# Skaipi/HNSWIndex.Net

Hardware: AMD Instinct MI355X
Metric: knn_queries_per_sec (higher is better)
Workload: dtype f32

## Files before the change

hnswindex.net_amd/bindings.py:

```python
import ctypes as ct
import os
from pathlib import Path
from typing import List, Optional, Tuple

import numpy as np
import numpy.typing as npt

_PKG = Path(__file__).resolve().parent
LIB_PATH = _PKG / "artifacts" / "native" / "linux-x64" / "HNSWIndex.Native.so"


def _load_lib():
    if os.environ.get("HNSW_MI355X_NO_TORCH", "0") != "1":
        try:
            import torch
        except Exception:
            pass
    override = os.environ.get("HNSW_MI355X_LIB")
    if override:
        return ct.CDLL(override)
    if not LIB_PATH.exists():
        raise FileNotFoundError(
            f"Native library missing {LIB_PATH}: run `python -c 'import __graft_entry__ as g; g.build()'` "
            "(hipcc --offload-arch=gfx950); there is no pure-Python or CPU fallback")
# ... 139 lines not shown


class LayerReach(ct.Structure):
    _fields_ = [(n, ct.c_int32) for n in ("layer_id", "nodes_count", "seeds", "reached", "max_hops")]

    def as_dict(self) -> dict:
        return {n: getattr(self, n) for n, _ in self._fields_}


_GRAPH_REACH_SUMMARY = ("nodes_count", "seeds", "reached", "max_hops")
lib.hnsw_mi355x_reachability.restype = ct.c_int
lib.hnsw_mi355x_reachability.argtypes = [ct.c_void_p, ct.POINTER(LayerReach), ct.c_int]
lib.hnsw_mi355x_unreachable_ids.restype = ct.c_int
lib.hnsw_mi355x_unreachable_ids.argtypes = [ct.c_void_p, ct.c_int, _I, ct.c_int]
lib.hnsw_mi355x_hop_counts.restype = ct.c_int
lib.hnsw_mi355x_hop_counts.argtypes = [ct.c_void_p, ct.c_int, _I, ct.c_int]
lib.hnswdev_graph_reach_layer.restype = ct.c_int
lib.hnswdev_graph_reach_layer.argtypes = [ct.c_void_p, ct.c_int, _U32, ct.c_longlong, _U32, ct.c_longlong, _U32, _I, ct.POINTER(ct.c_uint64)]
lib.hnswdev_graph_reach.restype = ct.c_int
lib.hnswdev_graph_reach.argtypes = [ct.c_void_p, ct.c_int, _U32, ct.c_longlong, ct.c_int, ct.POINTER(LayerReach), ct.c_int, _U32, _I]


class LayerRepair(ct.Structure):
    _fields_ = [(n, ct.c_int32) for n in ("layer_id", "unreachable_before", "linked", "evicted", "rounds", "unreachable_after")]

    def as_dict(self) -> dict:
        return {n: getattr(self, n) for n, _ in self._fields_}


lib.hnsw_mi355x_repair_reachability.restype = ct.c_int
lib.hnsw_mi355x_repair_reachability.argtypes = [ct.c_void_p, ct.c_int, ct.c_int, ct.POINTER(LayerRepair), ct.c_int]
lib.hnswdev_graph_repair_propose.restype = ct.c_int
lib.hnswdev_graph_repair_propose.argtypes = [ct.c_void_p, ct.c_int, _U32, ct.c_longlong, _U32, ct.c_longlong, ct.c_int, ct.c_int, _I, _I, _I, _I, ct.c_int]
lib.hnsw_mi355x_range_query_filtered.restype = ct.c_int
lib.hnsw_mi355x_range_query_filtered.argtypes = [ct.c_void_p, _F, ct.c_int, ct.c_int, ct.c_float, _U32, ct.c_longlong, ct.POINTER(ct.c_void_p),
                                                 ct.POINTER(ct.c_void_p), ct.POINTER(ct.c_int)]
lib.hnsw_mi355x_active_ids.restype = ct.c_int
lib.hnsw_mi355x_knn_query_at_layer.restype = ct.c_int
lib.hnsw_mi355x_knn_query_at_layer.argtypes = [ct.c_void_p, _F, ct.c_int, ct.c_int, ct.c_int, ct.c_int, _U32, ct.c_longlong, _I, _F]
lib.hnsw_mi355x_range_query_at_layer.restype = ct.c_int
lib.hnsw_mi355x_range_query_at_layer.argtypes = [ct.c_void_p, _F, ct.c_int, ct.c_int, ct.c_float, ct.c_int, _U32, ct.c_longlong, ct.POINTER(ct.c_void_p),
                                                 ct.POINTER(ct.c_void_p), ct.POINTER(ct.c_int)]
lib.hnsw_mi355x_multilayer_knn_query.restype = ct.c_int
lib.hnsw_mi355x_multilayer_knn_query.argtypes = [ct.c_void_p, _F, ct.c_int, ct.c_int, ct.c_int, ct.c_int, ct.c_int, ct.c_int, _I, _F]
lib.hnsw_mi355x_active_ids.argtypes = [ct.c_void_p, _I, ct.c_int]
lib.hnsw_mi355x_node_max_layer.restype = ct.c_int
lib.hnsw_mi355x_node_max_layer.argtypes = [ct.c_void_p, ct.c_int]
lib.hnsw_mi355x_get_out_edges.restype = ct.c_int
lib.hnsw_mi355x_get_out_edges.argtypes = [ct.c_void_p, ct.c_int, ct.c_int, _I, ct.c_int]
lib.hnsw_mi355x_export_levels.restype = ct.c_int
lib.hnsw_mi355x_export_levels.argtypes = [ct.c_void_p, _I, ct.c_int]
lib.hnsw_mi355x_export_edges.restype = ct.c_int
lib.hnsw_mi355x_export_edges.argtypes = [ct.c_void_p, ct.c_int, _I, _I, ct.c_int, ct.c_int]
lib.hnsw_mi355x_dim.restype = ct.c_int
lib.hnsw_mi355x_dim.argtypes = [ct.c_void_p]
lib.hnsw_mi355x_serialize.restype = ct.c_int
lib.hnsw_mi355x_serialize.argtypes = [ct.c_void_p, ct.c_char_p]
lib.hnsw_mi355x_deserialize.restype = ct.c_void_p
lib.hnsw_mi355x_deserialize.argtypes = [ct.c_char_p, ct.c_char_p]
lib.hnsw_mi355x_graph_hash.restype = ct.c_uint64
lib.hnsw_mi355x_graph_hash.argtypes = [ct.c_void_p]
lib.hnsw_mi355x_get_stats.restype = ct.c_int
lib.hnsw_mi355x_get_stats.argtypes = [ct.c_void_p, ct.POINTER(DeviceStats)]
lib.hnsw_mi355x_set_profiling.restype = ct.c_int
lib.hnsw_mi355x_set_profiling.argtypes = [ct.c_void_p, ct.c_int]
lib.hnsw_mi355x_index_set_insert_batch.restype = ct.c_int
lib.hnsw_mi355x_index_set_insert_batch.argtypes = [ct.c_void_p, ct.c_int]
lib.hnsw_mi355x_index_insert_batch.restype = ct.c_int
lib.hnsw_mi355x_index_insert_batch.argtypes = [ct.c_void_p]
lib.hnsw_mi355x_host_parallelism.restype = ct.c_int
lib.hnsw_mi355x_host_parallelism.argtypes = []
lib.hnsw_mi355x_device_count.restype = ct.c_int
lib.hnsw_mi355x_device_count.argtypes = [ct.c_void_p]
lib.hnsw_mi355x_get_stats_at.restype = ct.c_int
lib.hnsw_mi355x_get_stats_at.argtypes = [ct.c_void_p, ct.c_int, ct.POINTER(DeviceStats)]
lib.hnsw_mi355x_build_id.restype = ct.c_char_p
lib.hnsw_mi355x_build_id.argtypes = []
lib.hnsw_mi355x_exact_window_stats.restype = ct.c_int
lib.hnsw_mi355x_exact_window_stats.argtypes = [ct.c_void_p, ct.POINTER(ct.c_uint64)]
lib.hnsw_mi355x_row_prefilter_stats.restype = ct.c_int
lib.hnsw_mi355x_row_prefilter_stats.argtypes = [ct.c_void_p, ct.POINTER(ct.c_uint64)]
lib.hnsw_mi355x_row_prefilter_form_stats.restype = ct.c_int
lib.hnsw_mi355x_row_prefilter_form_stats.argtypes = [ct.c_void_p, ct.POINTER(ct.c_uint64)]
lib.hnsw_mi355x_row_prefilter_peek.restype = ct.c_int
lib.hnsw_mi355x_row_prefilter_peek.argtypes = [ct.c_void_p, ct.c_int, ct.c_int, ct.POINTER(ct.c_uint64), ct.POINTER(ct.c_float)]

lib.hnsw_mi355x_import_nodes.argtypes = [ct.c_void_p, _F, ct.c_int, ct.c_int, _I, ct.c_int]
lib.hnsw_mi355x_import_edges.argtypes = [ct.c_void_p, ct.c_int, _I, _I, ct.c_int]
lib.hnswdev_device_count.restype = ct.c_int
lib.hnswdev_create.restype = ct.c_int
lib.hnswdev_create.argtypes = [ct.c_int, ct.c_int, ct.c_int, ct.c_longlong, ct.POINTER(ct.c_void_p)]
lib.hnswdev_destroy.argtypes = [ct.c_void_p]
lib.hnswdev_reserve.argtypes = [ct.c_void_p, ct.c_longlong]
lib.hnswdev_upload_rows.argtypes = [ct.c_void_p, ct.c_int, ct.c_int, _F]
lib.hnswdev_download_rows.argtypes = [ct.c_void_p, ct.c_int, ct.c_int, _F]
lib.hnswdev_dist_query_batch.argtypes = [ct.c_void_p, _F, ct.c_int, _I, _I, _F]
lib.hnswdev_dist_pair_batch.argtypes = [ct.c_void_p, _I, _I, ct.c_int, _F]
lib.hnswdev_graph_begin.argtypes = [ct.c_void_p, ct.c_int, ct.c_int, _I]
lib.hnswdev_graph_set_layer.argtypes = [ct.c_void_p, ct.c_int, _I, _I, ct.c_int]
lib.hnswdev_graph_commit.argtypes = [ct.c_void_p]
lib.hnswdev_knn_search.argtypes = [ct.c_void_p, _F, ct.c_int, ct.c_int, ct.c_int, ct.c_int, _I, _F, _I]
lib.hnswdev_knn_search_filtered.restype = ct.c_int
lib.hnswdev_knn_search_filtered.argtypes = [ct.c_void_p, _F, ct.c_int, ct.c_int, ct.c_int, ct.c_int, _U32, ct.c_longlong, _I, _F, _I]
lib.hnswdev_range_search.restype = ct.c_int
lib.hnswdev_range_search.argtypes = [ct.c_void_p, _F, ct.c_int, ct.c_int, ct.c_float, _I, _I]
lib.hnswdev_exact_knn.restype = ct.c_int
lib.hnswdev_exact_knn.argtypes = [ct.c_void_p, _F, ct.c_int, ct.c_longlong, ct.c_int, _U32, ct.c_longlong, _I, _F]
lib.hnswdev_range_search_filtered.restype = ct.c_int
lib.hnswdev_range_search_filtered.argtypes = [ct.c_void_p, _F, ct.c_int, ct.c_int, ct.c_float, _U32, ct.c_longlong, _I, _I]
lib.hnswdev_exact_range.restype = ct.c_int
lib.hnswdev_exact_range.argtypes = [ct.c_void_p, _F, ct.c_int, ct.c_longlong, ct.c_float, _U32, ct.c_longlong, _I]
lib.hnswdev_exact_range_results.restype = ct.c_int
lib.hnswdev_exact_range_results.argtypes = [ct.c_void_p, _I, _F]
lib.hnswdev_exact_range_grouped.restype = ct.c_int
lib.hnswdev_exact_range_grouped.argtypes = [ct.c_void_p, _F, ct.c_int, ct.c_longlong, ct.c_float, _I, ct.c_longlong, _I, ct.c_int, _I]
lib.hnswdev_exact_knn_grouped.restype = ct.c_int
lib.hnswdev_exact_knn_grouped.argtypes = [ct.c_void_p, _F, ct.c_int, ct.c_longlong, ct.c_int, _I, ct.c_longlong, _I, ct.c_int, _I, _F]
lib.hnswdev_exact_knn_collapsed.restype = ct.c_int
lib.hnswdev_exact_knn_collapsed.argtypes = [ct.c_void_p, _F, ct.c_int, ct.c_longlong, ct.c_int, _I, ct.c_longlong, ct.c_int, _U32, ct.c_longlong, _I, _F]
lib.hnswdev_exact_grouped_list_ms.restype = ct.c_int
lib.hnswdev_exact_grouped_list_ms.argtypes = [ct.c_void_p, ct.POINTER(ct.c_double)]
lib.hnswdev_knn_search_tagged.restype = ct.c_int
lib.hnswdev_knn_search_tagged.argtypes = [ct.c_void_p, _F, ct.c_int, ct.c_int, ct.c_int, ct.c_int, ct.c_int, _U32, ct.c_longlong, _U32, ct.c_int, _I, _F, _I]
lib.hnswdev_exact_knn_tagged.restype = ct.c_int
lib.hnswdev_exact_knn_tagged.argtypes = [ct.c_void_p, _F, ct.c_int, ct.c_longlong, ct.c_int, _U32, ct.c_longlong, _U32, ct.c_int, _I, _F]
lib.hnswdev_gather_rows.restype = ct.c_int
lib.hnswdev_gather_rows.argtypes = [ct.c_void_p, _I, ct.c_int, _F]
lib.hnswdev_knn_search_by_id.restype = ct.c_int
lib.hnswdev_knn_search_by_id.argtypes = [ct.c_void_p, _I, ct.c_int, ct.c_int, ct.c_int, ct.c_int, ct.c_int, _I, _F, _I]
lib.hnswdev_exact_knn_by_id.restype = ct.c_int
lib.hnswdev_exact_knn_by_id.argtypes = [ct.c_void_p, _I, ct.c_int, ct.c_longlong, ct.c_int, _U32, ct.c_longlong, _I, _F]
lib.hnswdev_exact_range_by_id.restype = ct.c_int
lib.hnswdev_exact_range_by_id.argtypes = [ct.c_void_p, _I, ct.c_int, ct.c_longlong, ct.c_float, _U32, ct.c_longlong, _I]
lib.hnswdev_exact_range_groups.restype = ct.c_int
lib.hnswdev_exact_range_groups.argtypes = [ct.c_void_p, ct.c_longlong, ct.c_float, _U32, ct.c_longlong, _I, ct.POINTER(ct.c_uint64)]
lib.hnswdev_tag_list_ms.restype = ct.c_int
lib.hnswdev_tag_list_ms.argtypes = [ct.c_void_p, ct.POINTER(ct.c_double)]
lib.hnswdev_knn_search_grouped.restype = ct.c_int
lib.hnswdev_knn_search_grouped.argtypes = [ct.c_void_p, _F, ct.c_int, ct.c_int, ct.c_int, ct.c_int, ct.c_int, _I, ct.c_longlong, _I, ct.c_int, _I, _F, _I]
lib.hnswdev_range_search_grouped.restype = ct.c_int
lib.hnswdev_range_search_grouped.argtypes = [ct.c_void_p, _F, ct.c_int, ct.c_int, ct.c_float, ct.c_int, _I, ct.c_longlong, _I, ct.c_int, _I, _I]
lib.hnswdev_range_search_tagged.restype = ct.c_int
lib.hnswdev_range_search_tagged.argtypes = [ct.c_void_p, _F, ct.c_int, ct.c_int, ct.c_float, ct.c_int, _U32, ct.c_longlong, _U32, ct.c_int, _I, _I]
lib.hnswdev_exact_range_tagged.restype = ct.c_int
lib.hnswdev_exact_range_tagged.argtypes = [ct.c_void_p, _F, ct.c_int, ct.c_longlong, ct.c_float, _U32, ct.c_longlong, _U32, ct.c_int, _I]
lib.hnswdev_range_results.restype = ct.c_int
lib.hnswdev_range_results.argtypes = [ct.c_void_p, _I, _F]
lib.hnswdev_knn_search_at_layer.restype = ct.c_int
lib.hnswdev_knn_search_at_layer.argtypes = [ct.c_void_p, _F, ct.c_int, ct.c_int, ct.c_int, ct.c_int, ct.c_int, _U32, ct.c_longlong, _I, _F, _I]
lib.hnswdev_range_search_at_layer.restype = ct.c_int
lib.hnswdev_range_search_at_layer.argtypes = [ct.c_void_p, _F, ct.c_int, ct.c_int, ct.c_float, ct.c_int, _U32, ct.c_longlong, _I, _I]
lib.hnswdev_multilayer_search.restype = ct.c_int
lib.hnswdev_multilayer_search.argtypes = [ct.c_void_p, _F, ct.c_int, ct.c_int, ct.c_int, ct.c_int, ct.c_int, ct.c_int, _I, _F, _I]
lib.hnswdev_sync.argtypes = [ct.c_void_p]
lib.hnswdev_set_profiling.argtypes = [ct.c_void_p, ct.c_int]
lib.hnswdev_get_stats.argtypes = [ct.c_void_p, ct.POINTER(DeviceStats)]
lib.hnswdev_reset_stats.argtypes = [ct.c_void_p]
lib.hnswdev_last_error.argtypes = [ct.c_char_p, ct.c_int]
lib.hnswdev_ctx_last_error.argtypes = [ct.c_void_p, ct.c_char_p, ct.c_int]
lib.hnswdev_set_queries.argtypes = [ct.c_void_p, _F, ct.c_int]
lib.hnswdev_step_buffers.argtypes = [ct.c_void_p, ct.c_int, ct.c_int, ct.c_int, ct.POINTER(_I), ct.POINTER(_F)]
lib.hnswdev_step_submit.argtypes = [ct.c_void_p, ct.c_int, ct.c_int]
lib.hnswdev_step_wait.argtypes = [ct.c_void_p, ct.c_int]
lib.hnswdev_test_sqrt_rn.argtypes = [ct.c_int, ct.POINTER(ct.c_double), ct.POINTER(ct.c_double), ct.c_int]

COUNTER_BLOCKS = {
# ... 218 lines not shown

    @staticmethod
    def _check(status):
        if status < 0:
            raise RuntimeError(last_error())

    def set_collection_size(self, init_size: int):
        self._check(lib.hnsw_set_collection_size(init_size))

    def set_max_edges(self, max_conn: int):
        self._check(lib.hnsw_set_max_edges(max_conn))

    def set_max_candidates(self, max_candidates: int):
        self._check(lib.hnsw_set_max_candidates(max_candidates))

    def set_remove_max_candidates(self, rem_max_candidates: int):
        self._check(lib.hnsw_set_remove_max_candidates(rem_max_candidates))

    def set_distribution_rate(self, dist_rate: float):
        self._check(lib.hnsw_set_distribution_rate(dist_rate))

    def set_random_seed(self, random_seed: int):
        self._check(lib.hnsw_set_random_seed(random_seed))

    def set_min_nn(self, min_nn: int):
        self._check(lib.hnsw_set_min_nn(min_nn))

    def set_allow_removals(self, allow_removals: bool):
        self._check(lib.hnsw_set_allow_removals(allow_removals))

    def set_device(self, device: int):
        self._check(lib.hnsw_mi355x_set_device(device))

    def set_devices(self, n: int):
        self._check(lib.hnsw_mi355x_set_devices(n))

    def stats_at(self, context: int):
        st = DeviceStats()
        if not self._h or lib.hnsw_mi355x_get_stats_at(self._h, context, ct.byref(st)) != 0:
            raise RuntimeError(last_error() or "no such device context")
        return st.as_dict()

    def set_insert_batch(self, max_batch: int):
        self._check(lib.hnsw_mi355x_set_insert_batch(max_batch))

    def set_insert_batch_live(self, max_batch: int):
        if not self._h:
            return self.set_insert_batch(max_batch)
        self._check(lib.hnsw_mi355x_index_set_insert_batch(self._h, max_batch))

    @property
    def insert_batch_cap(self) -> int:
        return int(lib.hnsw_mi355x_index_insert_batch(self._h)) if self._h else host_parallelism()

    def exact_window_stats(self):
        out = (ct.c_uint64 * 4)()
        if not self._h or lib.hnsw_mi355x_exact_window_stats(self._h, out) != 0:
            return {"rounds": 0, "searches": 0, "alone": 0, "linked": 0}
        return {"rounds": int(out[0]), "searches": int(out[1]), "alone": int(out[2]), "linked": int(out[3])}

    def row_prefilter_stats(self):
        out = (ct.c_uint64 * 4)()
        if not self._h or lib.hnsw_mi355x_row_prefilter_stats(self._h, out) != 0:
            return {"launches": 0, "rows_on_shadow": 0, "rows_reread": 0, "rows_packed": 0}
        return {"launches": int(out[0]), "rows_on_shadow": int(out[1]), "rows_reread": int(out[2]), "rows_packed": int(out[3])}

    def row_prefilter_form_stats(self):
        out = (ct.c_uint64 * 2)()
        if not self._h or lib.hnsw_mi355x_row_prefilter_form_stats(self._h, out) != 0:
            return {"runtime_dim": 0, "fixed_dim": 0}
        return {"runtime_dim": int(out[0]), "fixed_dim": int(out[1])}

    def row_prefilter_peek(self, first_id: int = 0, count: int = 0):
        out = (ct.c_uint64 * 2)()
        rows = np.zeros((max(int(count), 0), self.dim), dtype=np.float32)
        if not self._h:
            if count > 0:
                raise RuntimeError("row_prefilter_peek: the index has no shadow rows")
            return {"packed": 0, "e_bits": 0, "e": np.float32(0), "rows": rows}
        self._check(lib.hnsw_mi355x_row_prefilter_peek(self._h, int(first_id), int(count), out, rows.ctypes.data_as(ct.POINTER(ct.c_float))))
        bits = int(out[1]) & 0xffffffff
        return {"packed": int(out[0]), "e_bits": bits, "e": np.array([bits], dtype=np.uint32).view(np.float32)[0], "rows": rows}

    def set_remove_batch(self, max_batch: int):
        self._check(lib.hnsw_mi355x_set_remove_batch(max_batch))

    def set_search_slots(self, slots: int):
        self._check(lib.hnsw_mi355x_set_search_slots(slots))

    def set_host_threads(self, threads: int):
        self._check(lib.hnsw_mi355x_set_host_threads(threads))

    def set_device_traversal(self, enabled: bool):
        self._check(lib.hnsw_mi355x_set_device_traversal(int(enabled)))

    def add(self, vecs: npt.ArrayLike) -> npt.NDArray[np.int32]:
        if not self._initialized:
            self._initialize()
        a = _as_2d_f32(vecs, self.dim)
        n, d = a.shape
        out_ids = np.empty(n, dtype=np.int32)
        rc = lib.hnsw_add(self._h, a.ctypes.data_as(_F), int(n), int(d), out_ids.ctypes.data_as(_I))
        if rc < 0:
            raise RuntimeError(last_error())
        return out_ids[:rc].copy()

    def remove(self, ids: npt.ArrayLike) -> None:
        arr = np.asarray(ids, dtype=np.int32).ravel()
        if arr.size == 0:
            return
        result = lib.hnsw_remove(self._h, arr.ctypes.data_as(_I), int(arr.size))
        if result < 0:
            raise RuntimeError(last_error())

    def knn_query(self, queries: npt.ArrayLike, k: int, allowed=None, layer: int = 0) -> Tuple[npt.NDArray[np.int32], npt.NDArray[np.float32]]:
        q = _as_2d_f32(queries, self.dim)
        n = int(q.shape[0])
        ids = np.empty((n, k), dtype=np.int32)
        dists = np.empty((n, k), dtype=np.float32)
        if layer != 0:
            ids.fill(-1)
            dists.fill(np.nan)
            words, nbits = allow_bits(allowed) if allowed is not None else (None, 0)
            words, wp = _words_arg(words) if allowed is not None else (None, None)
            status = lib.hnsw_mi355x_knn_query_at_layer(self._h, q.ctypes.data_as(_F), n, self.dim, k, int(layer), wp, nbits, ids.ctypes.data_as(_I),
                                                        dists.ctypes.data_as(_F))
            if status < 0:
                raise RuntimeError(last_error())
            return ids, dists
        if allowed is not None:
            words, nbits = allow_bits(allowed)
            words, wp = _words_arg(words)
            status = lib.hnsw_mi355x_knn_query_filtered(self._h, q.ctypes.data_as(_F), n, self.dim, k, wp, nbits, ids.ctypes.data_as(_I),
                                                        dists.ctypes.data_as(_F))
            if status < 0:
                raise RuntimeError(last_error())
            return ids, dists
        status = lib.hnsw_knn_query(self._h, q.ctypes.data_as(_F), n, self.dim, k, ids.ctypes.data_as(_I),
                                    dists.ctypes.data_as(_F))
        if status < 0:
            raise RuntimeError(last_error())
        return ids, dists

    def exact_knn_query(self, queries: npt.ArrayLike, k: int, allowed=None) -> Tuple[npt.NDArray[np.int32], npt.NDArray[np.float32]]:
        q = _as_2d_f32(queries, self.dim)
        n = int(q.shape[0])
        ids = np.full((n, max(k, 0)), -1, dtype=np.int32)
        dists = np.full((n, max(k, 0)), np.nan, dtype=np.float32)
        words, nbits = allow_bits(allowed) if allowed is not None else (None, 0)
        words, wp = _words_arg(words) if allowed is not None else (None, None)
        status = lib.hnsw_mi355x_exact_knn_query(self._h, q.ctypes.data_as(_F), n, self.dim, k, wp, nbits, ids.ctypes.data_as(_I),
                                                 dists.ctypes.data_as(_F))
        if status < 0:
            raise RuntimeError(last_error())
        return ids, dists

    def exact_knn_query_grouped(self, queries: npt.ArrayLike, k: int, row_group, query_group,
                                n_groups=None) -> Tuple[npt.NDArray[np.int32], npt.NDArray[np.float32]]:
        q = _as_2d_f32(queries, self.dim)
        n = int(q.shape[0])
        rg, qg, ng = _group_args(row_group, query_group, n_groups, n)
        ids = np.full((n, max(k, 0)), -1, dtype=np.int32)
        dists = np.full((n, max(k, 0)), np.nan, dtype=np.float32)
        status = lib.hnsw_mi355x_exact_knn_query_grouped(self._h, q.ctypes.data_as(_F), n, self.dim, k, rg.ctypes.data_as(_I), rg.shape[0],
                                                         qg.ctypes.data_as(_I), ng, ids.ctypes.data_as(_I), dists.ctypes.data_as(_F))
        if status < 0:
# ... 949 lines not shown
```

hnswindex.net_amd/csrc/device_backend.h:

```cpp
#pragma once
#include <cstddef>
#include <algorithm>
#include <atomic>
#include <cstdint>
#include <functional>
#include <memory>
#include <mutex>
#include <string>
#include <unordered_map>
#include <vector>
#include <thread>

#include "../../include/hnsw_mi355x.h"
#include "counter_blocks.h"
#include "dev_buf.h"

namespace hnsw {

#define HNSW_FOR_EACH_METRIC(X)      \
    X(M_SQ, sq, "sq_euclid")         \
    X(M_COS, cos, "cosine")          \
    X(M_UCOS, ucos, "ucosine")       \
    X(M_I8, i8, "sq_euclid_i8")      \
    X(M_SQH, sqh, "sq_euclid_f16")   \
// ... 210 lines not shown
    long long resident_queries() const { return n_queries_; }
    bool dist_query_batch(const float *queries, int nq, const int *offsets, const int *ids, float *out);
    bool dist_pair_batch(const int *a, const int *b, int n, float *out);

    bool graph_begin(int n, int max_edges, const int *levels);
    bool graph_set_layer(int layer, const int *counts, const int *edges, int stride);
    bool graph_commit();
    bool knn_search(const float *queries, int nq, int entry_point, int k_beam, int k_out, int *out_ids, float *out_d, int *out_flag, int layer = 0);
    bool knn_search_filtered(const float *queries, int nq, int entry_point, int k_beam, int k_out, const uint32_t *allow_bits, long long nbits,
                             int *out_ids, float *out_d, int *out_flag, int layer = 0);
    bool knn_search_grouped(const float *queries, int nq, int entry_point, int k_beam, int k_out, const int *row_group, long long n_row_group,
                            const int *query_group, int n_groups, int *out_ids, float *out_d, int *out_flag, int layer = 0);
    bool knn_search_tagged(const float *queries, int nq, int entry_point, int k_beam, int k_out, const uint32_t *row_tags, long long n_row_tags,
                           const uint32_t *query_tags, int match, int *out_ids, float *out_d, int *out_flag, int layer = 0);
    int multilayer_search_abi(const float *queries, int nq, int entry_point, int k, int max_layer, int min_layer, int layers_cap, int *out_ids,
                              float *out_d, int *out_flag);
    struct RangeResults {
        std::vector<unsigned long long> off;
        std::vector<int> cnt, flag, entry;
        std::vector<int> state;
        SearchHit *found = nullptr;
        size_t found_n = 0;
    };
    bool range_batch(const SearchJob *jobs, int njobs, float range, RangeResults *res, const RangeFilter &f);
    bool tag_candidates(const uint32_t *row_tags, long long n, const std::vector<uint32_t> &masks, int match, std::vector<int> &cnt);
    bool range_search(const float *queries, int nq, int entry_point, float range, int *out_counts, int *out_flags);
    bool range_search_filtered(const float *queries, int nq, int entry_point, float range, const uint32_t *allow_bits, long long nbits,
                               int *out_counts, int *out_flags, int layer = 0);
    bool range_search_grouped(const float *queries, int nq, int entry_point, float range, const int *row_group, long long n_row_group,
                              const int *query_group, int n_groups, int *out_counts, int *out_flags, int layer = 0);
    bool range_search_tagged(const float *queries, int nq, int entry_point, float range, const uint32_t *row_tags, long long n_row_tags,
                             const uint32_t *query_tags, int match, int *out_counts, int *out_flags, int layer = 0);
    bool range_results(int *out_ids, float *out_d);
    bool exact_knn(const float *queries, int nq, long long n_rows, int k, const uint32_t *allow_bits, long long nbits, int *out_ids, float *out_d);
    bool exact_knn_collapsed(const float *queries, int nq, long long n_rows, int k, const int *row_group, long long n_row_group, int per_group,
                             const uint32_t *allow_bits, long long nbits, int *out_ids, float *out_d);
    bool search_collapsed(int nq, int entry, int entry_layer, int ef, int beam, int k, const int *row_group, long long n_row_group, int per_group,
                          const uint32_t *allow_bits, long long nbits, int *out_ids, float *out_d, int *out_flag, int search_layer = 0);
    bool gather_rows(const int *ids, int n, float *out);
    bool set_queries_by_id(const int *ids, int nq);
    bool search_self(int nq, int entry, int entry_layer, int k, int k_out, int *out_ids, float *out_d, int *out_flag, int search_layer = 0);
    bool knn_search_by_id(const int *ids, int nq, int entry_point, int k_beam, int k_out, int *out_ids, float *out_d, int *out_flag, int layer = 0);
    bool exact_knn_by_id(const int *ids, int nq, long long n_rows, int k, const uint32_t *allow_bits, long long nbits, int *out_ids, float *out_d);
    bool exact_range(const float *queries, int nq, long long n_rows, float range, const uint32_t *allow_bits, long long nbits, int *out_counts);
    bool exact_range_results(int *out_ids, float *out_d);
    size_t exact_range_total() const { return xr_ids_.size(); }
    bool exact_range_by_id(const int *ids, int nq, long long n_rows, float range, const uint32_t *allow_bits, long long nbits, int *out_counts);
    bool exact_range_groups(long long n_rows, float range, const uint32_t *allow_bits, long long nbits, int *out_labels, uint64_t *out_info);
    bool exact_knn_grouped(const float *queries, int nq, long long n_rows, int k, const int *row_group, long long n_row_group, const int *query_group,
                           int n_groups, int *out_ids, float *out_d);
    bool exact_knn_tagged(const float *queries, int nq, long long n_rows, int k, const uint32_t *row_tags, long long n_row_tags, const uint32_t *query_tags,
                          int match, int *out_ids, float *out_d);
    double tag_list_ms() const { return xt_list_ms_; }
    bool exact_range_grouped(const float *queries, int nq, long long n_rows, float range, const int *row_group, long long n_row_group,
                             const int *query_group, int n_groups, int *out_counts);
    bool exact_range_tagged(const float *queries, int nq, long long n_rows, float range, const uint32_t *row_tags, long long n_row_tags,
                            const uint32_t *query_tags, int match, int *out_counts);
    double exact_grouped_list_ms() const { return xg_list_ms_; }
    bool graph_info(int layer, const uint32_t *live_bits, long long nbits, bool with_in_edges, hnsw_mi355x_layer_info *out);
    bool graph_components(int layer, const uint32_t *live_bits, long long nbits, int *out_count);
    bool graph_info_layer(const char *who, int layer);
    bool graph_reach_layer(int layer, const uint32_t *live_bits, long long nbits, const uint32_t *seed_bits, long long seed_nbits,
                           uint32_t *out_reached_bits, int *out_hops, uint64_t out_summary[4]);
    int graph_reach(int entry_point, int top, const uint32_t *live_bits, long long nbits, int min_layer, hnsw_mi355x_layer_reach *out_layers, int cap,
                    uint32_t *out_reached_bits, int *out_hops);
    bool graph_reach_top(const char *who, int entry_point, int *top);

    bool graph_repair_round(int layer, const uint32_t *live_bits, long long nbits, int seed_mode, int entry_point, const uint32_t *seed_bits, long long seed_nbits,
                            int which, int cands, int max_edges, bool propose, GraphRepairRound *out);
    bool graph_repair_patch(const int *recs, int nrows, int row_stride);
    int graph_repair_propose(int layer, const uint32_t *live_bits, long long nbits, const uint32_t *seed_bits, long long seed_nbits, int cands, int max_edges,
                             int *out_n, int *out_ids, int *out_cands, int *out_codes, int cap);

    void set_profiling(bool on) { profiling_ = on; }


    void set_shadows_allowed(bool on) { shadows_allowed_ = on; }
    void get_stats(hnswdev_stats *out);
    void reset_stats();
    void counters(CounterBlock b, uint64_t *out) const { std::copy_n(counters_[(int)b], kCounterSlots[(int)b], out); }
    void row_prefilter_stats(uint64_t out[4]);
    void row_prefilter_form_stats(uint64_t out[2]);
    bool row_prefilter_peek(long long first_id, int count, uint64_t out[2], float *rows);

    std::mutex &mutex() { return mu_; }
    void set_error(const std::string &msg) { std::lock_guard<std::mutex> lk(err_mu_); err_ = msg; }
    std::string error() { std::lock_guard<std::mutex> lk(err_mu_); return err_; }

private:
    Device() = default;
    std::mutex mu_, err_mu_;
    std::string err_;
    bool bind();
    bool abi_entry(const char *who, int entry_point, int *top, bool args_ok = true);
    bool abi_begin(const char *who, const float *queries, int nq, int entry_point, int layer, int *top, bool args_ok = true);
    int device_ = 0, dim_ = 0, metric_ = 0;
    int pitch_ = 0;
    int row_pitch_ = 0;
    DevBuf<float> q_stage_;
    long long capacity_ = 0;
    long long n_rows_hw_ = 0;
    DevBuf<float> d_rows_;
    DevBuf<double> d_row_sn_;
    struct RowPrefilter {
        std::mutex mu;
        DevBuf<float> rows;
        DevBuf<unsigned long long> words;
        long long row_cap = 0, packed = 0;
        bool lost = false;
        bool no_memory = false;
        uint64_t launches = 0, on_shadow = 0, reread = 0, rows_packed = 0;
        uint64_t form_launches[2] = {0, 0};
    };
    std::shared_ptr<RowPrefilter> pf_;
    void rows_written(long long first_id);
    bool row_prefilter_ready();
    DevBuf<float> d_queries_;
    DevBuf<double> d_q_sn_;
    long long q_capacity() const { return (long long)(d_queries_.cap() / (size_t)pitch_); }
    long long n_queries_ = 0;
    DevBuf<int> g_adj0_, g_level_, g_pool_;
    DevBuf<int64_t> g_upper_;
    long long g_n_ = 0;
    long long g_cap_n() const { return (long long)g_tested0_.cap(); }
    long long g_pool_cap() const { return (long long)g_testedU_.cap(); }
    bool graph_room(long long n, long long node_cap, int stride0, long long pool_len);
    DevBuf<int> g_tested0_, g_testedU_;
    int g_stride0_ = 0, g_strideU_ = 0;
    DevBuf<unsigned> s_visited_;
    DevBuf<int> s_jobctr_;
    DevBuf<int> lp_slot_[3];
    DevBuf<int> lp_grp_[6];
    DevBuf<int> lp_counters_;
    int last_insert_jobs_ = 0, last_insert_upper_ = 0, last_insert_stride_ = 0;
    int fetch_njobs_ = 0, fetch_nupper_ = 0;
    DevBuf<int> s_vistab_;
    int s_vistab_each_ = 0;
    DevBuf<int> s_fvistab_;
    int s_fvistab_each_ = 0;
    bool visited_scratch(int k, int min_cap, bool allow_hash, VisitedScratch *out, bool filtered = false);
    bool plan_traversal(bool insert, int k, bool two_heap, size_t lds, TraversalLaunch *out, bool filtered = false);
    template <class Upload, class Launch>
    bool run_resident(size_t row, long long chunk, size_t extra, bool hashed, int nq, int *out_ids, float *out_d, int *out_flag, Upload &&upload,
                      Launch &&launch);
    template <class OwnRules> bool predicate_call_ok(const PredicateCall &c, OwnRules &&own_rules);
    template <class Of> auto plan_predicate_search(const PredicateCall &c, Of of);
    template <class K, class Upload, class JobsOf, class Predicate>
    bool run_predicate_search(const PredicateCall &c, const PredicatePlan<K> &p, size_t extra, Upload &&upload, JobsOf &&jobs_of, Predicate &&predicate);
    uint64_t count_search_overflows(const PredicateCall &c);
    bool count_launch(const LaunchFamily *family, unsigned long long evals, bool hashed, bool timed, void *t0, void *t1);
    int num_cu_ = 256;
    int max_slots() const { return num_cu_ * max_waves_per_cu(); }
    static int max_waves_per_cu();
    DevBuf<SearchJob> s_jobs_;
    DevBuf<SearchHit> s_hits_;
    DevBuf<int> s_cnt_, s_flag_;
    DevBuf<unsigned long long> s_evals_;
    DevBuf<int> s_sel_, s_lcnt_, s_selU_, s_cntU_, s_iflag_;
    PinBuf<char> h_res_;
    DevBuf<int> s_rl_;
    DevBuf<int> s_order_;
    DevBuf<int> s_rlog_;
    struct QueryTail { const float *src = nullptr; long long first = 0, n = 0; } tail_;
    PinBuf<int> h_ready_;
    int *d_ready_ = nullptr;
    DevStream copy_stream_;
    bool upload_tail();
    DevBuf<int> s_dry_;
    DevBuf<int> s_wdry_;
    DevBuf<int> s_win_;
    DevBuf<SearchHit> s_spill_;
    DevBuf<SearchHit> s_fspill_;
    DevBuf<unsigned> s_allow_;
    DevBuf<int> s_glabel_;
    DevBuf<int> s_gquery_;
    DevBuf<unsigned> s_ttags_;
    DevBuf<unsigned> s_tmask_;
    DevBuf<int> s_tcnt_;
    DevBuf<int> s_tquery_;
    double xt_list_ms_ = 0.0;
    bool tag_counts(const unsigned *row_tags, long long n, const std::vector<uint32_t> &masks, int match, std::vector<int> &cnt);
    DevBuf<int> s_self_;
    DevBuf<int> x_self_;
    bool q_by_id_ = false;
    bool query_room(int nq);
    bool upload_ids(const int *ids, int n, DevBuf<int> &d_ids);
    bool gather_launch(const int *d_ids, long long n, float *out);
    bool gather_queries(const int *ids, int n, DevBuf<int> &d_ids, float *d_q, double *d_qsn);
    DevBuf<int> x_ids_;
    DevBuf<long long> x_boff_;
    DevBuf<unsigned long long> x_lists_;
    DevBuf<int> x_out_;
    DevBuf<unsigned long long> x_evals_;
    DevBuf<float> x_queries_;
    DevBuf<double> x_q_sn_;
    bool exact_queries(const char *who, const float *queries, int nq, const float **d_q, const double **d_qsn);
    bool exact_id_list(const uint32_t *allow_bits, long long n_allow, long long *m);
    bool exact_knn_rounds(const float *d_q, const double *d_qsn, int nq, const int *d_idlist, long long m, int k, int *out_ids, float *out_d, int *d_keep_ids,
                          const int *d_self = nullptr, const ExactCollapseArgs *collapse = nullptr);
// ... 119 lines not shown
```

hnswindex.net_amd/csrc/device_backend.hip:

```cpp

#include <hip/hip_runtime.h>

#include <algorithm>
#include <cmath>
#include <cstdio>
#include <cstdlib>
#include <cstring>
#include <limits>
#include <map>
#include <mutex>
#include <type_traits>
#include <vector>

#include "device_backend.h"
#include "diag.h"
#define HNSW_HOST_TU
#include "device_kernels.h"
#include "dk_exact.h"
#include "dk_graph_info.h"
#include "dk_graph_reach.h"
#include "dk_graph_repair.h"
#include "dk_tag_lists.h"
#include "range_replay.h"

// ... 322 lines not shown
    const int pitch = f16_row_words(dim);
    for (size_t r = 0; r < n; ++r) {
        const float *x = src + r * (size_t)dim;
        unsigned *rec = dst + r * (size_t)pitch;
        for (int w = 0; w < pitch; ++w) {
            const int i0 = ((w >> 3) << 4) | (w & 7), i1 = i0 + 8;
            unsigned b0 = 0u, b1 = 0u;
            if (i0 < dim) { memcpy(&b0, x + i0, 4); b0 = f32_to_f16_bits(b0); }
            if (i1 < dim) { memcpy(&b1, x + i1, 4); b1 = f32_to_f16_bits(b1); }
            rec[w] = b0 | (b1 << 16);
        }
    }
}

bool Device::upload_rows_begin(int first_id, int n, const float *rows)
{
    if (n <= 0) return true;
    if (metric_ == M_I8 || bg_.active.load()) { set_dev_error("upload_rows_begin: not available (int8 rows, or an upload already in flight)"); return false; }
    if (first_id < 0 || (long long)first_id + n > capacity_ || !rows) { set_dev_error("upload_rows: range outside capacity"); return false; }
    if (!bind()) return false;
    rows_written(first_id);
    const size_t row_bytes = (size_t)dim_ * sizeof(float);
    const size_t chunk_rows = std::max<size_t>(1, (8u << 20) / row_bytes);
    if (!bg_.stream.create(false) || !bg_.ev[0].create(false) || !bg_.ev[1].create(false)) return false;
    const size_t pin_need = chunk_rows * std::max(row_bytes, (size_t)row_pitch_ * sizeof(float));
    if (!bg_.pin[0].grow(pin_need) || !bg_.pin[1].grow(pin_need)) return false;
    bg_.resident.store(first_id);
    bg_.failed.store(false);
    bg_.active.store(true);
    n_rows_hw_ = std::max(n_rows_hw_, (long long)first_id + n);
    const bool f16 = metric_f16(metric_);
    bg_.th = std::thread([this, first_id, n, rows, row_bytes, chunk_rows, f16] {
        auto fail = [&](const char *what, hipError_t e) { bg_.err = std::string(what) + ": " + hipGetErrorString(e); bg_.failed.store(true); };
        hipError_t e = hipSetDevice(device_);
        if (e != hipSuccess) { fail("hipSetDevice", e); return; }
        hipStream_t st = S(bg_.stream);
        size_t pending_rows[2] = {0, 0};
        bool in_flight[2] = {false, false};
        int b = 0;
        long long landed = first_id;
        for (size_t r0 = 0; r0 < (size_t)n; r0 += chunk_rows, b ^= 1) {
            const size_t nr = std::min(chunk_rows, (size_t)n - r0);
            if (in_flight[b]) {
                if ((e = hipEventSynchronize(E(bg_.ev[b]))) != hipSuccess) { fail("hipEventSynchronize", e); return; }
                landed += (long long)pending_rows[b];
                bg_.resident.store(landed, std::memory_order_release);
                in_flight[b] = false;
            }
            if (f16) pack_f16_rows_host(reinterpret_cast<unsigned *>(bg_.pin[b].get()), rows + r0 * dim_, nr, dim_);
            else memcpy(bg_.pin[b], rows + r0 * dim_, nr * row_bytes);
            if ((e = hipMemcpyAsync(d_rows_ + ((size_t)first_id + r0) * row_pitch_, bg_.pin[b], f16 ? nr * (size_t)row_pitch_ * sizeof(float) : nr * row_bytes, hipMemcpyHostToDevice, st)) != hipSuccess) { fail("hipMemcpyAsync", e); return; }
            if (metric_ == M_COS) {
                const int blocks = (int)(((long long)nr * 8 + 255) / 256);
                hipLaunchKernelGGL(row_sqrtnorm_kernel, dim3(blocks), dim3(256), 0, st, d_rows_, pitch_, (long long)first_id + (long long)r0, (int)nr, d_row_sn_);
            }
            if ((e = hipEventRecord(E(bg_.ev[b]), st)) != hipSuccess) { fail("hipEventRecord", e); return; }
            pending_rows[b] = nr;
            in_flight[b] = true;
        }
        for (int k = 0; k < 2; ++k, b ^= 1)
            if (in_flight[b]) {
                if ((e = hipEventSynchronize(E(bg_.ev[b]))) != hipSuccess) { fail("hipEventSynchronize", e); return; }
                landed += (long long)pending_rows[b];
                bg_.resident.store(landed, std::memory_order_release);
            }
    });
    return true;
}

bool Device::upload_rows_wait(long long upto)
{
    if (!bg_.active.load()) return true;
    if (upto >= 0) {
        while (bg_.resident.load(std::memory_order_acquire) < upto && !bg_.failed.load()) std::this_thread::yield();
        if (!bg_.failed.load()) return true;
    }
    if (bg_.th.joinable()) bg_.th.join();
    bg_.active.store(false);
    if (bg_.failed.load()) { set_dev_error("background row upload failed: " + bg_.err); return false; }
    return true;
}

static int row_prefilter_mode() { return diag("row_prefilter", 1); }

void Device::rows_written(long long first_id)
{
    if (!pf_) return;
    std::lock_guard<std::mutex> lk(pf_->mu);
    pf_->packed = std::min(pf_->packed, std::max(0ll, first_id));
    pf_->lost = false;
}

bool Device::row_prefilter_ready()
{
    const int mode = row_prefilter_mode();
    if (!pf_ || metric_ != M_SQ || mode == 0 || bg_.active.load() || n_rows_hw_ <= 0) return false;
    RowPrefilter &P = *pf_;
    std::lock_guard<std::mutex> lk(P.mu);
    if (P.no_memory || (P.lost && mode != 2)) return false;
    hipStream_t st = S(stream_);
    const size_t words = (size_t)f16_row_words(dim_);
    if (P.row_cap < capacity_ || !P.rows) {
        const std::string before = get_dev_error();
        const bool first = !P.words;
        if (!P.rows.grow((size_t)capacity_ * words) || !P.words.grow(4)) {
            (void)P.rows.reset();
            P.row_cap = P.packed = 0;
            P.no_memory = true;
            (void)hipGetLastError();
            set_dev_error(before);
            return false;
        }
        P.row_cap = capacity_;
        P.packed = 0;
        if (first) HIP_OK(hipMemsetAsync(P.words, 0, 4 * sizeof(unsigned long long), st));
    }
    const long long n = n_rows_hw_;
    if (P.packed < n) {
        if (P.packed == 0) HIP_OK(hipMemsetAsync(P.words, 0, sizeof(unsigned long long), st));
        const long long more = n - P.packed;
        hipLaunchKernelGGL(pack_shadow_rows_kernel, dim3((unsigned)((more + 3) / 4)), dim3(256), 0, st, d_rows_.get(), dim_, P.packed, more, P.rows.get(),
                           reinterpret_cast<unsigned *>(P.words.get()));
        HIP_OK(hipGetLastError());
        HIP_OK(hipStreamSynchronize(st));
        P.rows_packed += (uint64_t)more;
        P.packed = n;
    }
    return true;
}

void Device::row_prefilter_stats(uint64_t out[4])
{
    out[0] = out[1] = out[2] = out[3] = 0;
    if (!pf_) return;
    std::lock_guard<std::mutex> lk(pf_->mu);
    out[0] = pf_->launches; out[1] = pf_->on_shadow; out[2] = pf_->reread; out[3] = pf_->rows_packed;
}

void Device::row_prefilter_form_stats(uint64_t out[2])
{
    out[0] = out[1] = 0;
    if (!pf_) return;
    std::lock_guard<std::mutex> lk(pf_->mu);
    out[0] = pf_->form_launches[0]; out[1] = pf_->form_launches[1];
}

bool Device::row_prefilter_peek(long long first_id, int count, uint64_t out[2], float *rows)
{
    out[0] = out[1] = 0;
    if (!pf_ || !pf_->rows || !pf_->words) {
        if (count > 0) set_dev_error("row_prefilter_peek: the index has no shadow rows");
        return count <= 0;
    }
    if (!bind()) return false;
    RowPrefilter &P = *pf_;
    std::lock_guard<std::mutex> lk(P.mu);
    unsigned long long e_word = 0;
    HIP_OK(hipMemcpy(&e_word, P.words.get(), sizeof(e_word), hipMemcpyDeviceToHost));
    out[0] = (uint64_t)P.packed;
    out[1] = (uint64_t)(e_word & 0xffffffffull);
    if (count <= 0) return true;
    if (first_id < 0 || first_id + count > P.packed || !rows) {
        set_dev_error("row_prefilter_peek: range outside the packed shadow rows");
        return false;
    }
    const size_t words = (size_t)f16_row_words(dim_), total = (size_t)count * words;
    const unsigned *src = reinterpret_cast<const unsigned *>(P.rows.get()) + (size_t)first_id * words;
    unsigned buf[2048];
    for (size_t w0 = 0; w0 < total; w0 += 2048) {
        const size_t nw = std::min<size_t>(2048, total - w0);
        HIP_OK(hipMemcpy(buf, src + w0, nw * sizeof(unsigned), hipMemcpyDeviceToHost));
        for (size_t j = 0; j < nw; ++j) {
            const size_t r = (w0 + j) / words;
            const int w = (int)((w0 + j) % words), i0 = ((w >> 3) << 4) | (w & 7), i1 = i0 + 8;
            if (i0 < dim_) rows[r * (size_t)dim_ + i0] = half_lo(buf[j]);
            if (i1 < dim_) rows[r * (size_t)dim_ + i1] = half_hi(buf[j]);
        }
    }
    return true;
}

bool Device::download_rows(int first_id, int n, float *rows)
{
    if (n <= 0) return true;
    if (first_id < 0 || (long long)first_id + n > capacity_ || !rows) {
        set_dev_error("download_rows: range outside capacity");
        return false;
    }
    if (!bind()) return false;
    if (metric_ == M_I8) {
        if (!q_stage_.grow((size_t)n * (size_t)dim_)) return false;
        hipLaunchKernelGGL(dequantize_rows_kernel, dim3((unsigned)(((long long)n * dim_ + 255) / 256)), dim3(256), 0, S(stream_), d_rows_, pitch_,
                           (long long)first_id, n, dim_, q_stage_);
        HIP_OK(hipGetLastError());
        HIP_OK(hipMemcpyAsync(rows, q_stage_, (size_t)n * dim_ * sizeof(float), hipMemcpyDeviceToHost, S(stream_)));
    } else if (metric_f16(metric_)) {
        const size_t chunk_rows = std::max<size_t>(1, (64u << 20) / ((size_t)dim_ * sizeof(float)));
        if (!q_stage_.grow(std::min<size_t>((size_t)n, chunk_rows) * (size_t)dim_)) return false;
        for (size_t r0 = 0; r0 < (size_t)n; r0 += chunk_rows) {
            const size_t nr = std::min(chunk_rows, (size_t)n - r0);
            hipLaunchKernelGGL(unpack_f16_rows_kernel, dim3((unsigned)((nr * (size_t)dim_ + 255) / 256)), dim3(256), 0, S(stream_), d_rows_,
                               (long long)first_id + (long long)r0, (int)nr, dim_, q_stage_);
            HIP_OK(hipGetLastError());
            HIP_OK(hipMemcpyAsync(rows + r0 * (size_t)dim_, q_stage_, nr * (size_t)dim_ * sizeof(float), hipMemcpyDeviceToHost, S(stream_)));
            HIP_OK(hipStreamSynchronize(S(stream_)));
        }
    } else {
        HIP_OK(hipMemcpyAsync(rows, d_rows_ + (size_t)first_id * pitch_, (size_t)n * dim_ * sizeof(float), hipMemcpyDeviceToHost, S(stream_)));
    }
    HIP_OK(hipStreamSynchronize(S(stream_)));
    return true;
}

bool Device::staged_upload(float *dst, const float *src, size_t bytes)
{
    constexpr int T = 4;
    constexpr size_t kChunk = 2u << 20;
    for (int i = 0; i < 2 * T; ++i) {
        if (!up_pin_[i].grow(kChunk) || !up_ev_[i].create(false)) return false;
// ... 462 lines not shown
    const int c = diag("spill_cap", -1);
    return c < 0 ? kSpillCap : std::min(kSpillCap, c);
}
constexpr int kFilterSpillCap = 32768;
static int filter_spill_cap()
{
    const int c = diag("spill_cap", -1);
    return c < 0 ? kFilterSpillCap : std::min(kFilterSpillCap, c);
}
constexpr int kFilterVisCap = 1 << 17;


static bool shadow_mode()
{
    return diag("shadow", 1) != 0;
}
static int overlap_mode()
{
    return diag("overlap", 1);
}
static bool lean_mode() { return diag("lean", 1) != 0; }
static int novis_mode()
{
    return diag("novis", 2);
}
static constexpr size_t kTeamLds = ((sizeof(TeamMail) + 15) & ~(size_t)15) + 16;
static int lat_mode()
{
    return diag("lat", 1);
}

static bool mfma_heuristic()
{
    return diag("mfma", 1) != 0;
}

struct VisitedScratch {
    long long words = 0;
    size_t bytes_per_job = 0;
    int *tab = nullptr;
    int tab_cap = 0;
};

bool Device::visited_scratch(int k, int min_cap, bool allow_hash, VisitedScratch *v, bool filtered)
{
    *v = VisitedScratch{};
    v->words = ((g_n_ + 31) / 32 + 3) & ~3LL;
    v->bytes_per_job = sizeof(unsigned) * (size_t)v->words;
    if (!allow_hash) return true;
    const int e = diag("vis_hash", -1);
    const bool want = e >= 0 ? e != 0 : v->bytes_per_job > (512u << 10);
    if (!want) return true;
    int cap = 16384;
    while (cap < 64 * k && cap < (1 << 22)) cap <<= 1;
    if (const int c = diag("vis_hash_cap", 0)) { cap = 64; while (cap < c && cap < (1 << 22)) cap <<= 1; }
    while (cap < min_cap) cap <<= 1;
    const size_t need = (size_t)max_slots() * (size_t)cap;
    DevBuf<int> &tab = filtered ? s_fvistab_ : s_vistab_;
    int &tab_each = filtered ? s_fvistab_each_ : s_vistab_each_;
    if (need > tab.cap() || cap != tab_each) {
        HIP_OK(hipStreamSynchronize(S(stream_)));
        if (!tab.reset() || !tab.grow(need)) return false;
        HIP_OK(hipMemsetAsync(tab, 0xff, sizeof(int) * need, S(stream_)));
        tab_each = cap;
    }
    v->tab = tab;
    v->tab_cap = cap;
    v->words = 0;
    v->bytes_per_job = 16;
    return true;
}

struct TraversalLaunch {
    int metric, max_slots, num_cu;
    size_t lds;
    int ns;
    bool exact_only;
    VisitedScratch vis;
    bool novis;
    bool lat_ok;
    bool filtered;
    bool prefilter;
    bool pf_fixed;
    int form;
    int slots, grid;
    unsigned block;
    size_t lds_total;
    int flags;
};

bool Device::plan_traversal(bool insert, int k, bool two_heap, size_t lds, TraversalLaunch *t, bool filtered)
{
    const int ns = g_n_ < kSortedTopMaxNodes && !two_heap && !filtered ? sorted_top_sets(k) : 0;
    t->metric = metric_;
    t->max_slots = max_slots();
    t->num_cu = num_cu_;
    t->lds = lds;
    t->filtered = filtered;
    t->prefilter = false;
    t->pf_fixed = pitch_ == kPfFixedDim && diag("pf_fixed_dim", 1) != 0;
    t->exact_only = ns == 0;
    t->ns = t->exact_only ? 2 : ns;
    if (!visited_scratch(k, filtered ? kFilterVisCap : 512, t->ns != 8, &t->vis, filtered)) return false;
    if (filtered) {
        t->novis = false;
        t->lat_ok = false;
        return true;
    }
    const int novis = novis_mode();
    t->novis = (!insert || diag("novis_insert", 1) != 0) && g_stride0_ - 2 <= 64 && overlap_mode() != 0 && (size_t)pitch_ * sizeof(float) <= 1024 &&
               (novis == 2 || (novis == 1 && t->vis.tab != nullptr));
    t->lat_ok = !t->exact_only && g_stride0_ - 2 <= 64 && lds + kTeamLds <= 64 * 1024;
    return true;
}

template <bool Insert, int M, int NS, bool H>
static auto traversal_form(int form)
{
    if constexpr (Insert)
        return form == kFormLat ? &graph_insert_search_kernel<M, NS, H, kFormLat> : &graph_insert_search_kernel<M, NS, H, kFormPlain>;
    else if constexpr (NS <= 4)
        return form == kFormLat ? &graph_search_kernel<M, NS, H, kFormLat>
               : form == kFormLean ? &graph_search_kernel<M, NS, H, kFormLean>
               : form == kFormLeanPF ? &graph_search_kernel<M, NS, H, kFormLeanPF>
               : form == kFormLeanPFFixed ? &graph_search_kernel<M, NS, H, kFormLeanPFFixed> : &graph_search_kernel<M, NS, H, kFormPlain>;
    else
        return form == kFormLat ? &graph_search_kernel<M, NS, H, kFormLat> : &graph_search_kernel<M, NS, H, kFormPlain>;
}
template <bool Insert>
static auto traversal_kernel(const TraversalLaunch &t, int form)
{
    const bool hashed = t.vis.tab != nullptr;
    decltype(traversal_form<Insert, M_SQ, 2, false>(0)) kernel = nullptr;
    with_metric(t.metric, [&](auto m) {
        if (t.ns == 2) kernel = hashed ? traversal_form<Insert, m, 2, true>(form) : traversal_form<Insert, m, 2, false>(form);
        else if (t.ns == 4) kernel = hashed ? traversal_form<Insert, m, 4, true>(form) : traversal_form<Insert, m, 4, false>(form);
        else kernel = traversal_form<Insert, m, 8, false>(form);
    });
    return kernel;
}

template <class Of>
static auto persistent_kernel(int metric, bool hashed, Of of)
{
    decltype(of(std::integral_constant<int, M_SQ>{}, std::false_type{})) kernel = nullptr;
    with_metric(metric, [&](auto m) { kernel = hashed ? of(m, std::true_type{}) : of(m, std::false_type{}); });
    return kernel;
}
template <class K>
static void place_persistent(K kernel, TraversalLaunch &t, int nj)
{
    t.form = kFormPlain;
    t.slots = std::min(t.max_slots, resident_blocks(kernel, t.lds, t.num_cu));
    t.grid = std::min(nj, t.slots);
    t.block = 64;
    t.lds_total = t.lds;
    t.flags = 0;
}

template <bool Insert>
static auto place_traversal(TraversalLaunch &t, int nj)
{
    const bool hashed = t.vis.tab != nullptr;
    const int lat = lat_mode();
    t.form = kFormPlain;
    if (t.lat_ok && lat != 0) {
        const int slots = std::min(t.max_slots, resident_blocks(traversal_kernel<Insert>(t, kFormLat), t.lds + kTeamLds, t.num_cu, 128));
        if (slots > 0 && (lat == 2 || nj <= slots)) { t.form = kFormLat; t.slots = slots; }
    }
    if (!Insert && t.form == kFormPlain && t.novis && !t.exact_only && lean_mode() && t.ns <= 4) t.form = !t.prefilter ? kFormLean : t.pf_fixed ? kFormLeanPFFixed : kFormLeanPF;
    const auto kernel = traversal_kernel<Insert>(t, t.form);
    if (t.form != kFormLat) t.slots = std::min(t.max_slots, resident_blocks(kernel, t.lds, t.num_cu));
    t.grid = std::min(nj, t.slots);
    t.block = t.form == kFormLat ? 128 : 64;
    t.lds_total = t.lds + (t.form == kFormLat ? kTeamLds : 0);
    const int overlap = overlap_mode();
    t.flags = (t.exact_only ? 0x200 : 0) | (t.novis ? 9 : overlap == 2 || (overlap == 1 && (nj <= t.slots || hashed)) ? 1 : 0);
    return kernel;
}

bool Device::ensure_search_scratch(long long chunk, long long slots, int k, size_t vis_bytes_per_job)
{
    const size_t vis_words = vis_bytes_per_job * (size_t)slots / sizeof(unsigned);
    if (vis_words > s_visited_.cap()) {
        if (!s_visited_.grow(vis_words)) return false;
        HIP_OK(hipMemsetAsync(s_visited_, 0, sizeof(unsigned) * vis_words, S(stream_)));
    }
    const size_t jobs_cap = s_flag_.cap();
    if (!s_jobctr_.grow(4 + std::max<size_t>((size_t)chunk, jobs_cap))) return false;
    if ((size_t)chunk > jobs_cap) {
        uj_len_ = 0;
        if (!reset_all(s_jobs_, s_cnt_, s_flag_)) return false;
        if (!s_jobs_.grow((size_t)chunk) || !s_cnt_.grow((size_t)chunk) || !s_flag_.grow((size_t)chunk)) return false;
    }
    if (k > 0 && !s_hits_.grow((size_t)chunk * k + ((size_t)chunk + 1) / 2)) return false;
    if (!s_spill_.grow((size_t)slots * kSpillCap + 8)) return false;
    if (!s_evals_.grow(1)) return false;
    return ev0_.create(true) && ev1_.create(true) && ev2_.create(false);
}

static bool jobs_valid(const SearchJob *jobs, int njobs, long long g_n, long long n_queries, long long n_rows)
{
    for (int i = 0; i < njobs; ++i) {
        const SearchJob &j = jobs[i];
        bool ok = j.entry >= 0 && j.entry < g_n && j.search_layer >= 0 && j.entry_layer >= j.search_layer &&
                  (j.qref >= 0 ? j.qref < n_queries : (~j.qref) < n_rows);
        if (!ok) return false;
    }
    return true;
}

bool Device::insert_search_batch(const SearchJob *jobs, int njobs, int k, int max_edges0, int n_upper, InsertResults *res, WindowExtras *win)
{
    if (njobs <= 0) return true;
    const bool windowed = win != nullptr;
    const int read_log_cap = windowed ? win->read_log_cap : 0;
    if (windowed && (read_log_cap < 8 || njobs > (1 << 16) || (n_upper > 0 && !win->upper_owner))) { set_dev_error("insert_search_batch: bad window request"); return false; }
    if (!jobs || !res || k < 1 || n_upper < 0 || max_edges0 < 2) { set_dev_error("insert_search_batch: bad argument"); return false; }
    if (g_n_ <= 0) { set_dev_error("insert_search_batch: no graph uploaded"); return false; }
    for (int i = 0; i < njobs; ++i) {
        const SearchJob &j = jobs[i];
        if (j.qref >= 0) { set_dev_error("insert_search_batch: qref must name a stored row"); return false; }
        if (j.search_layer > 0 && (j.aux < 0 || j.aux + j.search_layer > n_upper)) { set_dev_error("insert_search_batch: upper-layer slot out of range"); return false; }
        if (j.stop_layer < 0 || j.stop_layer > j.search_layer || (!windowed && j.stop_layer != 0)) { set_dev_error("insert_search_batch: bad stop layer"); return false; }
    }
    if (!jobs_valid(jobs, njobs, g_n_, n_queries_, n_rows_hw_)) { set_dev_error("insert_search_batch: job outside the uploaded graph / rows"); return false; }
    const int cand_cap = cand_lds_cap(k, pitch_, true, nbcap());
    const size_t lds = search_lds_bytes(k, cand_cap, pitch_, true, nbcap());
    if (lds > 64 * 1024) { set_dev_error("insert_search_batch: beam width / dimension exceed the LDS budget"); return false; }
    const size_t lds_link = windowed ? link_lds_or_error("insert_search_batch", pitch_, nbcap()) : 0;
    if (windowed && !lds_link) return false;
    if (!bind()) return false;
    hipStream_t st = S(stream_);
    const int sel_stride = max_edges0;
    const long long chunk = std::min<long long>(njobs, 1 << 20);
    TraversalLaunch tl;
    if (!plan_traversal(true, k, false, lds, &tl)) return false;
    if (!ensure_search_scratch(chunk, max_slots(), 0, tl.vis.bytes_per_job)) return false;
    const size_t nU = (size_t)std::max(n_upper, 1);
    if (!s_sel_.grow((size_t)njobs * sel_stride) || !s_lcnt_.grow((size_t)njobs) || !s_selU_.grow(nU * sel_stride) || !s_cntU_.grow(nU) || !s_iflag_.grow((size_t)njobs))
        return false;
    if (windowed && !s_rlog_.grow((size_t)njobs * (size_t)read_log_cap)) return false;
    const size_t b_sel0 = 4u * (size_t)njobs * sel_stride, b_cnt0 = 4u * (size_t)njobs, b_selU = 4u * nU * sel_stride, b_cntU = 4u * nU, b_flag = 4u * (size_t)njobs;
    const size_t b_log = windowed ? 4u * (size_t)njobs * (size_t)read_log_cap : 0;
    const size_t b_dry = windowed ? b_sel0 + b_selU : 0;
    const size_t b_drop = windowed ? 3u * b_sel0 : 0;
    const size_t b_rep = windowed ? b_flag : 0;
    if (windowed && !s_wdry_.grow(nU)) return false;
    const size_t need = b_sel0 + b_cnt0 + b_selU + b_cntU + b_flag + 16 + b_log + b_dry + b_drop + b_rep;
    if (windowed && !s_win_.grow((need - b_rep + 3) / 4u + 64)) return false;
    if (!h_res_.grow(need, need + need / 2)) return false;
    char *hb = h_res_;
    int *h_sel0 = reinterpret_cast<int *>(hb), *h_cnt0 = reinterpret_cast<int *>(hb + b_sel0);
// ... 348 lines not shown
{
    if (set < 0 || set > 1 || !lset_[set].busy) { set_dev_error("link_batch_finish: nothing in flight"); return false; }
    LinkSet &ls = lset_[set];
    if (!bind()) return false;
    HIP_OK(hipEventSynchronize(E(ls.ev_done)));
    ls.busy = false;
    if (out_lists) *out_lists = ls.h_out;
    if (ls.ngroups > 0 && !count_launch(&kLinkFamily, *ls.h_ev, false, ls.timed, ls.ev_start, ls.ev_stop)) return false;
    return true;
}


void *Device::pinned_stage(size_t bytes)
{
    return h_stage_.grow(bytes, std::max<size_t>(bytes, 1u << 20)) ? h_stage_.get() : nullptr;
}

bool Device::search_batch(const SearchJob *jobs, int njobs, int k, int k_out, int *out_ids, float *out_d, int *out_flag, bool keep_repeat_flag,
                          bool two_heap)
{
    if (njobs <= 0) return true;
    if (!jobs) { set_dev_error("search_batch: bad argument"); return false; }
    return search_batch_impl(jobs, njobs, k, k_out, out_ids, out_d, out_flag, keep_repeat_flag, two_heap, -1, -1);
}

bool Device::search_queries(int nq, int entry, int entry_layer, int k, int k_out, int *out_ids, float *out_d, int *out_flag)
{
    if (nq <= 0) return true;
    if (nq > (1 << 20)) {
        std::vector<SearchJob> jobs((size_t)nq);
        for (int i = 0; i < nq; ++i) jobs[(size_t)i] = SearchJob{i, entry, entry_layer, 0, -1, 0};
        return search_batch(jobs.data(), nq, k, k_out, out_ids, out_d, out_flag);
    }
    return search_batch_impl(nullptr, nq, k, k_out, out_ids, out_d, out_flag, false, false, entry, entry_layer);
}

bool Device::search_batch_impl(const SearchJob *jobs, int njobs, int k, int k_out, int *out_ids, float *out_d, int *out_flag, bool keep_repeat_flag,
                               bool two_heap, int u_entry, int u_layer)
{
    if (!out_ids || !out_d || !out_flag || k < 1 || k_out < 1) { set_dev_error("search_batch: bad argument"); return false; }
    if (g_n_ <= 0) { set_dev_error("search_batch: no graph uploaded"); return false; }
    if (jobs ? !jobs_valid(jobs, njobs, g_n_, n_queries_, n_rows_hw_) : !(u_entry >= 0 && u_entry < g_n_ && u_layer >= 0 && njobs <= n_queries_)) {
        set_dev_error("search_batch: job outside the uploaded graph / rows / queries");
        return false;
    }
    const int cand_cap = cand_lds_cap(k, pitch_, false, nbcap());
    const size_t lds = search_lds_bytes(k, cand_cap, pitch_, false, nbcap());
    if (lds > 64 * 1024) { set_dev_error("search_batch: beam width / dimension exceed the LDS budget"); return false; }
    if (!bind()) return false;
    hipStream_t st = S(stream_);
    const long long chunk = std::min<long long>(njobs, 1 << 20);
    TraversalLaunch tl;
    if (!plan_traversal(false, k, two_heap, lds, &tl)) return false;
    if (!ensure_search_scratch(chunk, max_slots(), k_out, tl.vis.bytes_per_job)) return false;
    const size_t b_jobs = sizeof(SearchJob) * (size_t)chunk, b_res = 4u * (size_t)chunk * k_out;
    const size_t off_pf = (16 + b_jobs + 2 * b_res + 4u * (size_t)chunk + 7) & ~(size_t)7;
    char *hs = static_cast<char *>(pinned_stage(off_pf + 16));
    if (!hs) return false;
    unsigned long long *h_ev = reinterpret_cast<unsigned long long *>(hs), *h_pf = reinterpret_cast<unsigned long long *>(hs + off_pf);
    SearchJob *h_jobs = reinterpret_cast<SearchJob *>(hs + 16);
    int *h_ids = reinterpret_cast<int *>(hs + 16 + b_jobs);
    float *h_d = reinterpret_cast<float *>(hs + 16 + b_jobs + b_res);
    int *h_flag = reinterpret_cast<int *>(hs + 16 + b_jobs + 2 * b_res);
    int *d_ids = reinterpret_cast<int *>(s_hits_.get());
    float *d_d = reinterpret_cast<float *>(s_hits_.get()) + (size_t)chunk * k_out;
    const bool compact = !row_collapse_ && njobs == chunk && 2 * b_res + 4u * (size_t)chunk <= (size_t)1 << 20;
    const size_t w_out = row_collapse_ ? (size_t)row_collapse_->k : (size_t)k_out;
    int *d_flag = compact ? reinterpret_cast<int *>(d_d + (size_t)chunk * k_out) : s_flag_;
    unsigned long long *d_ev = compact ? reinterpret_cast<unsigned long long *>(s_jobctr_.get() + 2) : s_evals_;
    const int *gate = tail_.n > 0 ? d_ready_ : nullptr;
    struct TailGuard { Device *d; ~TailGuard() { if (d->tail_.n > 0) d->n_queries_ = 0; d->tail_.n = 0; } } tail_guard{this};
    for (long long off = 0; off < njobs; off += chunk) {
        const int nj = (int)std::min<long long>(chunk, njobs - off);
        if (jobs) {
            memcpy(h_jobs, jobs + off, sizeof(SearchJob) * (size_t)nj);
            HIP_OK(hipMemcpyAsync(s_jobs_, h_jobs, sizeof(SearchJob) * (size_t)nj, hipMemcpyHostToDevice, st));
            uj_len_ = 0;
        } else if (!(uj_len_ >= nj && uj_entry_ == u_entry && uj_layer_ == u_layer)) {
            for (int i = 0; i < nj; ++i) h_jobs[i] = SearchJob{i, u_entry, u_layer, 0, -1, 0};
            HIP_OK(hipMemcpyAsync(s_jobs_, h_jobs, sizeof(SearchJob) * (size_t)nj, hipMemcpyHostToDevice, st));
            uj_len_ = nj; uj_entry_ = u_entry; uj_layer_ = u_layer;
        }
        auto kernel = place_traversal<false>(tl, nj);
        if (tl.form == kFormLean && row_prefilter_ready()) {
            tl.prefilter = true;
            kernel = place_traversal<false>(tl, nj);
        }
        const bool prefiltered = form_is_pf(tl.form);
        HIP_OK(hipMemsetAsync(s_jobctr_, 0, sizeof(int) * (4 + (size_t)nj), st));
        if (!compact) HIP_OK(hipMemsetAsync(s_evals_, 0, sizeof(unsigned long long), st));
        const bool timed = profiling_;
        if (timed) HIP_OK(hipEventRecord(E(ev0_), st));
        hipLaunchKernelGGL(kernel, dim3(tl.grid), dim3(tl.block), tl.lds_total, st, d_rows_, d_row_sn_, d_queries_, d_q_sn_, pitch_, g_adj0_, g_stride0_,
                           g_upper_, g_pool_, g_strideU_, s_jobs_, k, cand_cap, reinterpret_cast<ND *>(s_spill_.get()), spill_cap_for_tests(), s_visited_,
                           tl.vis.words, tl.vis.tab, tl.vis.tab_cap, k_out, d_ids, d_d, s_cnt_, d_flag, d_ev, nbcap(), nj, s_jobctr_,
                           tl.flags | (shadow_mode() && shadows_allowed_ ? 0x100 : 0), gate, prefiltered ? pf_->rows.get() : (const float *)nullptr,
                           prefiltered ? pf_->words.get() : (unsigned long long *)nullptr);
        if (tl.form == kFormLat) stats_.lat_launches++;
        if (form_is_lean(tl.form)) stats_.lean_launches++;
        HIP_OK(hipGetLastError());
        if (timed) HIP_OK(hipEventRecord(E(ev1_), st));
        if (prefiltered) HIP_OK(hipMemcpyAsync(h_pf, pf_->words.get() + 1, 2 * sizeof(unsigned long long), hipMemcpyDeviceToHost, st));
        if (tail_.n > 0 && !upload_tail()) return false;
        if (compact) {
            HIP_OK(hipMemcpyAsync(h_ids, d_ids, 2 * b_res + sizeof(int) * (size_t)nj, hipMemcpyDeviceToHost, st));
            HIP_OK(hipMemcpyAsync(h_ev, d_ev, sizeof(unsigned long long), hipMemcpyDeviceToHost, st));
            HIP_OK(hipStreamSynchronize(st));
            memcpy(out_ids + (size_t)off * k_out, h_ids, 4u * (size_t)nj * k_out);
        } else if (row_collapse_) {
            if (!collapse_and_fetch(d_ids, d_d, nj, (size_t)k_out, h_ids, h_d)) return false;
            HIP_OK(hipMemcpyAsync(h_flag, s_flag_, sizeof(int) * (size_t)nj, hipMemcpyDeviceToHost, st));
            HIP_OK(hipMemcpyAsync(h_ev, s_evals_, sizeof(unsigned long long), hipMemcpyDeviceToHost, st));
            HIP_OK(hipStreamSynchronize(st));
            memcpy(out_ids + (size_t)off * w_out, h_ids, 4u * (size_t)nj * w_out);
        } else {
        HIP_OK(hipMemcpyAsync(h_ids, d_ids, 4u * (size_t)nj * k_out, hipMemcpyDeviceToHost, st));
        HIP_OK(hipEventRecord(E(ev2_), st));
        HIP_OK(hipMemcpyAsync(h_d, d_d, 4u * (size_t)nj * k_out, hipMemcpyDeviceToHost, st));
        HIP_OK(hipMemcpyAsync(h_flag, s_flag_, sizeof(int) * (size_t)nj, hipMemcpyDeviceToHost, st));
        HIP_OK(hipMemcpyAsync(h_ev, s_evals_, sizeof(unsigned long long), hipMemcpyDeviceToHost, st));
        HIP_OK(hipEventSynchronize(E(ev2_)));
        memcpy(out_ids + (size_t)off * k_out, h_ids, 4u * (size_t)nj * k_out);
        HIP_OK(hipStreamSynchronize(st));
        }
        memcpy(out_d + (size_t)off * w_out, h_d, 4u * (size_t)nj * w_out);
        for (int i = 0; i < nj; ++i) {
            if (h_flag[i] == 2) { stats_.search_repeats++; if (!keep_repeat_flag) h_flag[i] = 0; }
            else if (h_flag[i] == 4) { stats_.tie_windows++; h_flag[i] = 0; }
        }
        memcpy(out_flag + off, h_flag, sizeof(int) * (size_t)nj);
        if (prefiltered) {
            std::lock_guard<std::mutex> lk(pf_->mu);
            const uint64_t d_shadow = h_pf[0] > pf_->on_shadow ? h_pf[0] - pf_->on_shadow : 0, d_reread = h_pf[1] > pf_->reread ? h_pf[1] - pf_->reread : 0;
            pf_->launches++;
            pf_->form_launches[tl.form == kFormLeanPFFixed]++;
            pf_->on_shadow += d_shadow;
            pf_->reread += d_reread;
            if (2 * d_reread > d_shadow && row_prefilter_mode() != 2) pf_->lost = true;
        }
        tl.prefilter = false;
        if (!count_launch(nullptr, *h_ev, tl.vis.tab != nullptr, timed, ev0_, ev1_)) return false;
    }
    for (int i = 0; i < njobs; ++i) stats_.search_overflows += (uint64_t)(out_flag[i] == 1);
    return true;
}

bool Device::collapse_and_fetch(int *d_ids, float *d_d, int nj, size_t width, int *h_ids, float *h_d)
{
    hipStream_t st = S(stream_);
    const RowCollapse &rc = *row_collapse_;
    const size_t lds = 12 * width + 4 * (size_t)rc.k, w = (size_t)rc.k;
    if (lds > 64 * 1024) { set_dev_error("search_collapsed: the beam exceeds the LDS budget of the collapse"); return false; }
    hipLaunchKernelGGL(collapse_rows_kernel, dim3((unsigned)nj), dim3(64), lds, st, d_ids, d_d, (int)width, rc.k, rc.d_labels, rc.n_labels, rc.per_group);
    HIP_OK(hipGetLastError());
    HIP_OK(hipMemcpy2DAsync(h_ids, 4 * w, d_ids, 4 * width, 4 * w, (size_t)nj, hipMemcpyDeviceToHost, st));
    HIP_OK(hipMemcpy2DAsync(h_d, 4 * w, d_d, 4 * width, 4 * w, (size_t)nj, hipMemcpyDeviceToHost, st));
    return true;
}

template <class Upload, class Launch>
bool Device::run_resident(size_t row, long long chunk, size_t extra, bool hashed, int nq, int *out_ids, float *out_d, int *out_flag, Upload &&upload,
                          Launch &&launch)
{
    hipStream_t st = S(stream_);
    const size_t b_res = 4u * (size_t)chunk * row;
    char *hs = static_cast<char *>(pinned_stage(16 + 2 * b_res + 4u * (size_t)chunk + extra));
    if (!hs) return false;
    unsigned long long *h_ev = reinterpret_cast<unsigned long long *>(hs);
    int *h_ids = reinterpret_cast<int *>(hs + 16);
    float *h_d = reinterpret_cast<float *>(hs + 16 + b_res);
    int *h_flag = reinterpret_cast<int *>(hs + 16 + 2 * b_res);
    if (!upload(hs + 16 + 2 * b_res + 4u * (size_t)chunk)) return false;
    int *d_ids = reinterpret_cast<int *>(s_hits_.get());
    float *d_d = reinterpret_cast<float *>(s_hits_.get()) + (size_t)chunk * row;
    for (long long off = 0; off < nq; off += chunk) {
        const int nj = (int)std::min<long long>(chunk, nq - off);
        HIP_OK(hipMemsetAsync(s_jobctr_, 0, sizeof(int) * 4, st));
        HIP_OK(hipMemsetAsync(s_evals_, 0, sizeof(unsigned long long), st));
        const bool timed = profiling_;
        if (timed) HIP_OK(hipEventRecord(E(ev0_), st));
        launch(off, nj, d_ids, d_d);
        HIP_OK(hipGetLastError());
        if (timed) HIP_OK(hipEventRecord(E(ev1_), st));
        const size_t w = row_collapse_ ? (size_t)row_collapse_->k : row;
        if (row_collapse_) { if (!collapse_and_fetch(d_ids, d_d, nj, row, h_ids, h_d)) return false; }
        else {
            HIP_OK(hipMemcpyAsync(h_ids, d_ids, 4u * (size_t)nj * row, hipMemcpyDeviceToHost, st));
            HIP_OK(hipMemcpyAsync(h_d, d_d, 4u * (size_t)nj * row, hipMemcpyDeviceToHost, st));
        }
        HIP_OK(hipMemcpyAsync(h_flag, s_flag_, sizeof(int) * (size_t)nj, hipMemcpyDeviceToHost, st));
        HIP_OK(hipMemcpyAsync(h_ev, s_evals_, sizeof(unsigned long long), hipMemcpyDeviceToHost, st));
        HIP_OK(hipStreamSynchronize(st));
        memcpy(out_ids + (size_t)off * w, h_ids, 4u * (size_t)nj * w);
        memcpy(out_d + (size_t)off * w, h_d, 4u * (size_t)nj * w);
        memcpy(out_flag + off, h_flag, sizeof(int) * (size_t)nj);
        if (!count_launch(nullptr, *h_ev, hashed, timed, ev0_, ev1_)) return false;
    }
    return true;
}

struct PredicateCall {
    std::string who;
    int nq, entry, entry_layer, search_layer, k, k_out;
    int *out_ids;
    float *out_d;
    int *out_flag;
};
template <class K>
struct PredicatePlan {
    bool ok;
    K kernel;
    TraversalLaunch tl;
    int cand_cap, fspill;
    long long chunk;
};

template <class OwnRules>
bool Device::predicate_call_ok(const PredicateCall &c, OwnRules &&own_rules)
{
    const std::string &who = c.who;
    if (!c.out_ids || !c.out_d || !c.out_flag || c.k < 1 || c.k_out < 1) { set_dev_error(who + ": bad argument"); return false; }
    if (const std::string why = own_rules(); !why.empty()) { set_dev_error(why); return false; }
    if (g_n_ <= 0) { set_dev_error(who + ": no graph uploaded"); return false; }
// ... 2955 lines not shown
```

hnswindex.net_amd/csrc/device_kernels.h:

```cpp
#pragma once
#include "dk_base.h"
#include "dk_metric.h"
#include "dk_heaps.h"
#include "dk_measure.h"
#include "dk_search_common.h"
#include "dk_sorted_top.h"
#include "dk_team.h"
#include "dk_pool_top.h"
#include "dk_traverse_exact.h"
#include "dk_heuristic.h"
#include "dk_search_kernels.h"
#include "dk_range_finish.h"
#include "dk_insert_kernels.h"
#include "dk_link.h"
#include "dk_misc_kernels.h"

namespace hnsw {

#define HNSW_FOR_EACH_TRAVERSAL(X, M) \
    X(M, 2, false, kFormPlain) X(M, 4, false, kFormPlain) X(M, 8, false, kFormPlain) \
    X(M, 2, true, kFormPlain) X(M, 4, true, kFormPlain)
#define HNSW_FOR_EACH_TRAVERSAL_LAT(X, M) \
    X(M, 2, false, kFormLat) X(M, 4, false, kFormLat) X(M, 8, false, kFormLat) \
    X(M, 2, true, kFormLat) X(M, 4, true, kFormLat)
#define HNSW_FOR_EACH_TRAVERSAL_LEAN(X, M) \
    X(M, 2, false, kFormLean) X(M, 4, false, kFormLean) X(M, 2, true, kFormLean) X(M, 4, true, kFormLean) \
    X(M, 2, false, kFormLeanPF) X(M, 4, false, kFormLeanPF) X(M, 2, true, kFormLeanPF) X(M, 4, true, kFormLeanPF) \
    X(M, 2, false, kFormLeanPFFixed) X(M, 4, false, kFormLeanPFFixed) X(M, 2, true, kFormLeanPFFixed) X(M, 4, true, kFormLeanPFFixed)

#define HNSW_FOR_EACH_KIND(X, ...) \
    X(insert, __VA_ARGS__) X(insert_lat, __VA_ARGS__) X(search, __VA_ARGS__) X(search_lat, __VA_ARGS__) X(search_lean, __VA_ARGS__) \
    X(filtered, __VA_ARGS__) X(multilayer, __VA_ARGS__)
#define HNSW_UNIT_insert(DO, M) HNSW_FOR_EACH_TRAVERSAL(HNSW_##DO##_INSERT, M)
#define HNSW_UNIT_insert_lat(DO, M) HNSW_FOR_EACH_TRAVERSAL_LAT(HNSW_##DO##_INSERT, M)
#define HNSW_UNIT_search(DO, M) HNSW_FOR_EACH_TRAVERSAL(HNSW_##DO##_SEARCH, M)
#define HNSW_UNIT_search_lat(DO, M) HNSW_FOR_EACH_TRAVERSAL_LAT(HNSW_##DO##_SEARCH, M)
#define HNSW_UNIT_search_lean(DO, M) HNSW_FOR_EACH_TRAVERSAL_LEAN(HNSW_##DO##_SEARCH, M)
#define HNSW_UNIT_filtered(DO, M) HNSW_FOR_EACH_FILTERED(HNSW_##DO##_FILTERED, M) HNSW_FOR_EACH_FILTERED(HNSW_##DO##_GROUPED, M) HNSW_FOR_EACH_FILTERED(HNSW_##DO##_TAGGED, M) HNSW_FOR_EACH_FILTERED(HNSW_##DO##_SELF, M)
#define HNSW_UNIT_multilayer(DO, M) HNSW_FOR_EACH_MULTILAYER(HNSW_##DO##_MULTILAYER, M)

}
```

hnswindex.net_amd/csrc/dk_base.h:

```cpp
#pragma once
#include <hip/hip_runtime.h>

#include <cstddef>
#include <cstdint>

#include "device_backend.h"

#ifdef EXP_LAT_REGS
#define HNSW_WAVES(x) 1
#else
#define HNSW_WAVES(x) (x)
#endif

#ifndef HNSW_I8_WAVES
#define HNSW_I8_WAVES 5
#endif

#ifndef HNSW_PF_WAVES
#define HNSW_PF_WAVES 3
#endif
#ifndef HNSW_PF_FIXED_WAVES
#define HNSW_PF_FIXED_WAVES 4
#endif

namespace hnsw {

__device__ __forceinline__ void wave_sync()
{
    __builtin_amdgcn_fence(__ATOMIC_SEQ_CST, "workgroup");
    __builtin_amdgcn_s_waitcnt(0);
    __builtin_amdgcn_wave_barrier();
    __builtin_amdgcn_fence(__ATOMIC_SEQ_CST, "workgroup");
}

__device__ __forceinline__ void wave_lds_sync()
{
    __builtin_amdgcn_fence(__ATOMIC_RELEASE, "wavefront");
    __builtin_amdgcn_wave_barrier();
    __builtin_amdgcn_fence(__ATOMIC_ACQUIRE, "wavefront");
}
constexpr int kFormPlain = 0, kFormLat = 1, kFormLean = 2, kFormLeanPF = 3, kFormLeanPFFixed = 4;
constexpr int kPfFixedDim = 128;
constexpr __host__ __device__ bool form_is_pf(int f) { return f == kFormLeanPF || f == kFormLeanPFFixed; }
constexpr __host__ __device__ bool form_is_lean(int f) { return f == kFormLean || form_is_pf(f); }

template <class T>
__device__ __forceinline__ T kernarg_load(unsigned byte_offset)
{
    typedef const char __attribute__((address_space(4))) *cptr;
    typedef const volatile T __attribute__((address_space(4))) *tptr;
    return *(tptr)((cptr)__builtin_amdgcn_kernarg_segment_ptr() + byte_offset);
}

constexpr __host__ __device__ bool metric_f16(int m) { return m == M_SQH || m == M_UCOSH; }
constexpr __host__ __device__ bool metric_is_sq(int m) { return m == M_SQ || m == M_SQH; }
constexpr __host__ __device__ bool metric_is_ucos(int m) { return m == M_UCOS || m == M_UCOSH; }
constexpr __host__ __device__ int metric_arith(int m) { return m == M_SQH ? (int)M_SQ : m == M_UCOSH ? (int)M_UCOS : m; }
constexpr __host__ __device__ int f16_row_words(int dim) { return ((dim + 15) >> 4) << 3; }
template <int METRIC>
__host__ __device__ __forceinline__ int row_words(int dim)
{
    if constexpr (metric_f16(METRIC)) return f16_row_words(dim);
    else return dim;
}
template <int METRIC>
__device__ __forceinline__ const float *row_at(const float *__restrict__ rows, size_t id, int dim)
{
    if constexpr (metric_f16(METRIC)) return rows + id * (size_t)f16_row_words(dim);
    else return rows + id * dim;
}
__host__ __device__ __forceinline__ float half_lo(unsigned w) { return (float)__builtin_bit_cast(_Float16, (unsigned short)(w & 0xffffu)); }
__host__ __device__ __forceinline__ float half_hi(unsigned w) { return (float)__builtin_bit_cast(_Float16, (unsigned short)(w >> 16)); }
template <int METRIC>
__device__ __forceinline__ float row_elem(const float *__restrict__ rec, int i)
{
    if constexpr (metric_f16(METRIC)) {
        const unsigned w = reinterpret_cast<const unsigned *>(rec)[((i >> 4) << 3) | (i & 7)];
        return (i & 8) ? half_hi(w) : half_lo(w);
    } else return rec[i];
}
__host__ __device__ inline unsigned short f32_to_f16_bits(unsigned x)
{
    const unsigned sign = (x >> 16) & 0x8000u, a = x & 0x7fffffffu;
    if (a >= 0x7f800000u) return (unsigned short)(sign | (a > 0x7f800000u ? 0x7e00u | ((a >> 13) & 0x3ffu) : 0x7c00u));
    if (a >= 0x477ff000u) return (unsigned short)(sign | 0x7c00u);
    if (a >= 0x38800000u) {
        const unsigned r = a - 0x38000000u;
        return (unsigned short)(sign | ((r + 0xfffu + ((r >> 13) & 1u)) >> 13));
    }
    if (a < 0x33000000u) return (unsigned short)sign;
    const unsigned e = a >> 23, m = (a & 0x7fffffu) | 0x800000u;
    const unsigned sh = 126u - e;
    const unsigned q = m >> sh, rem = m & ((1u << sh) - 1u), halfway = 1u << (sh - 1u);
    return (unsigned short)(sign | (q + ((rem > halfway || (rem == halfway && (q & 1u))) ? 1u : 0u)));
}

}
```

hnswindex.net_amd/csrc/dk_misc_kernels.h:

```cpp
#pragma once
#include "dk_metric.h"

namespace hnsw {

template <int METRIC>
__global__ void __launch_bounds__(256)
pair_distance_kernel(const float *__restrict__ rows, const double *__restrict__ row_sn, int dim,
                     const int *__restrict__ a_ids, const int *__restrict__ b_ids, float *__restrict__ out, int n,
                     long long n_rows, int *__restrict__ guard)
{
    const int g = (blockIdx.x * 256 + threadIdx.x) >> 3;
    const int j = threadIdx.x & 7;
    const bool act = g < n;
    int a = a_ids[act ? g : 0], b = b_ids[act ? g : 0];
    const bool bad = (unsigned long long)(long long)a >= (unsigned long long)n_rows || (unsigned long long)(long long)b >= (unsigned long long)n_rows;
    if (bad) { a = 0; b = 0; }
    double sa = 0.0, sb = 0.0;
    if (METRIC == M_COS) { sa = row_sn[a]; sb = row_sn[b]; }
    float r = group_metric<METRIC>(row_at<METRIC>(rows, (size_t)a, dim), row_at<METRIC>(rows, (size_t)b, dim), dim, j, sa, sb);
    if (act && j == 0) {
        out[g] = bad ? __uint_as_float(0x7fc00000u) : r;
        if (bad) atomicOr(guard, 1);
    }
}
// ... 28 lines not shown
    for (int o = 32; o > 0; o >>= 1) m = fmaxf(m, __shfl_xor(m, o, 64));
    const float scale = m / 127.0f;
    int sumsq = 0;
    const int nwords = pitch - 2;
    for (int w = lane; w < nwords; w += 64) {
        unsigned packed = 0u;
#pragma unroll
        for (int t = 0; t < 4; ++t) {
            const int i = 4 * w + t;
            int q = 0;
            if (i < dim && scale > 0.0f) {
                const float v = __builtin_rintf(x[i] / scale);
                q = (int)fminf(fmaxf(v, -127.0f), 127.0f);
            }
            sumsq += q * q;
            packed |= (unsigned)(q & 0xff) << (8 * t);
        }
        rec[w] = (int)packed;
    }
#pragma unroll
    for (int o = 32; o > 0; o >>= 1) sumsq += __shfl_xor(sumsq, o, 64);
    if (lane == 0) { rec[pitch - 2] = __float_as_int(scale); rec[pitch - 1] = sumsq; }
}
__global__ void __launch_bounds__(256)
dequantize_rows_kernel(const float *__restrict__ recs, int pitch, long long first, int n, int dim, float *__restrict__ out)
{
    const long long t = (long long)blockIdx.x * 256 + threadIdx.x;
    if (t >= (long long)n * dim) return;
    const int r = (int)(t / dim), i = (int)(t % dim);
    const int *rec = reinterpret_cast<const int *>(recs + (size_t)(first + r) * pitch);
    const int q = (int)(signed char)((rec[i >> 2] >> (8 * (i & 3))) & 0xff);
    out[t] = (float)q * __int_as_float(rec[pitch - 2]);
}
#endif
#ifdef HNSW_HOST_TU
__global__ void __launch_bounds__(256)
pack_f16_rows_kernel(const float *__restrict__ src, int dim, int n, float *__restrict__ dst, long long first)
{
    const int pitch = f16_row_words(dim);
    const long long t = (long long)blockIdx.x * 256 + threadIdx.x;
    if (t >= (long long)n * pitch) return;
    const int r = (int)(t / pitch), w = (int)(t % pitch);
    const int i0 = ((w >> 3) << 4) | (w & 7), i1 = i0 + 8;
    const float *x = src + (size_t)r * dim;
    const unsigned lo = i0 < dim ? f32_to_f16_bits(__float_as_uint(x[i0])) : 0u, hi = i1 < dim ? f32_to_f16_bits(__float_as_uint(x[i1])) : 0u;
    reinterpret_cast<unsigned *>(dst)[(size_t)(first + r) * pitch + w] = lo | (hi << 16);
}
__global__ void __launch_bounds__(256)
pack_shadow_rows_kernel(const float *__restrict__ src, int dim, long long first, long long n, float *__restrict__ dst, unsigned *__restrict__ e_bits)
{
    const int pitch = f16_row_words(dim), lane = threadIdx.x & 63;
    const long long r = (long long)blockIdx.x * 4 + (threadIdx.x >> 6);
    if (r >= n) return;
    const float *x = src + (size_t)(first + r) * dim;
    unsigned *rec = reinterpret_cast<unsigned *>(dst) + (size_t)(first + r) * pitch;
    double ss = 0.0;
    bool finite = true;
    for (int w = lane; w < pitch; w += 64) {
        const int i0 = ((w >> 3) << 4) | (w & 7), i1 = i0 + 8;
        const float x0 = i0 < dim ? x[i0] : 0.0f, x1 = i1 < dim ? x[i1] : 0.0f;
        const unsigned word = (unsigned)f32_to_f16_bits(__float_as_uint(x0)) | ((unsigned)f32_to_f16_bits(__float_as_uint(x1)) << 16);
        rec[w] = word;
        const float h0 = half_lo(word), h1 = half_hi(word);
        finite = finite && (h0 - h0 == 0.0f) && (h1 - h1 == 0.0f) && (x0 - x0 == 0.0f) && (x1 - x1 == 0.0f);
        const double d0 = (double)x0 - (double)h0, d1 = (double)x1 - (double)h1;
        ss += d0 * d0 + d1 * d1;
    }
#pragma unroll
    for (int o = 32; o > 0; o >>= 1) ss += __shfl_xor(ss, o, 64);
    const bool all_finite = __ballot(!finite) == 0ull;
    if (lane == 0) {
        unsigned bits = 0x7f800000u;
        if (all_finite && ss < 1e300) {
            const double e = sqrt(ss);
            float f = (float)e;
            if ((double)f < e) f = __uint_as_float(__float_as_uint(f) + 1u);
            f = f * 1.00000095367431640625f + 1e-37f;
            bits = __float_as_uint(f);
        }
        atomicMax(e_bits, bits);
    }
}
__global__ void __launch_bounds__(256)
unpack_f16_rows_kernel(const float *__restrict__ recs, long long first, int n, int dim, float *__restrict__ out)
{
    const long long t = (long long)blockIdx.x * 256 + threadIdx.x;
    if (t >= (long long)n * dim) return;
    const int r = (int)(t / dim), i = (int)(t % dim);
    out[t] = row_elem<M_SQH>(recs + (size_t)(first + r) * f16_row_words(dim), i);
}
#endif
#ifdef HNSW_HOST_TU
constexpr int kGatherBlock = 256;
__global__ void __launch_bounds__(kGatherBlock)
gather_rows_kernel(const float *__restrict__ rows, int pitch, long long n_rows, int kind, const int *__restrict__ ids, long long n_ids, int dim,
                           float *__restrict__ out)
{
    const long long total = n_ids * dim, step = (long long)gridDim.x * kGatherBlock;
    for (long long t = (long long)blockIdx.x * kGatherBlock + threadIdx.x; t < total; t += step) {
        const long long i = t / dim;
        const int e = (int)(t - i * dim);
        const long long id = ids[i];
        float x = 0.0f;
        if ((unsigned long long)id < (unsigned long long)n_rows) {
            const float *rec = rows + (size_t)id * pitch;
            if (kind == 1) x = row_elem<M_SQH>(rec, e);
            else if (kind == 2) {
                const int *r = reinterpret_cast<const int *>(rec);
                x = (float)(int)(signed char)((r[e >> 2] >> (8 * (e & 3))) & 0xff) * __int_as_float(r[pitch - 2]);
            } else x = rec[e];
        }
        out[t] = x;
    }
}
#endif
#ifdef HNSW_HOST_TU
__global__ void __launch_bounds__(64) collapse_rows_kernel(int *__restrict__ ids, float *__restrict__ d, int width, int k, const int *__restrict__ labels,
                                                           long long n_labels, int m)
{
    extern __shared__ int collapse_lds[];
    int *r_id = collapse_lds, *r_lab = r_id + width, *kept_lab = r_lab + width;
    float *r_d = reinterpret_cast<float *>(kept_lab + k);
    const int lane = threadIdx.x;
    int *row_ids = ids + (size_t)blockIdx.x * width;
    float *row_d = d + (size_t)blockIdx.x * width;
    for (int i = lane; i < width; i += 64) {
        const int id = row_ids[i];
        const bool real = id >= 0 && id < n_labels;
        r_id[i] = real ? id : -1;
        r_d[i] = row_d[i];
        r_lab[i] = real ? labels[id] : 0;
    }
    wave_lds_sync();
    int kept = 0;
    for (int e = 0; e < width && kept < k; ++e) {
        const int id = r_id[e], g = r_lab[e];
        int same = 0;
        for (int base = 0; base < kept; base += 64) same += __popcll(__ballot(base + lane < kept && kept_lab[base + lane] == g));
        const bool keep = id >= 0 && same < m;
        if (keep && lane == 0) { row_ids[kept] = id; row_d[kept] = r_d[e]; kept_lab[kept] = g; }
        wave_lds_sync();
        kept += keep ? 1 : 0;
    }
    for (int i = kept + lane; i < k; i += 64) { row_ids[i] = -1; row_d[i] = __uint_as_float(0x7fc00000u); }
}
#endif
#ifdef HNSW_HOST_TU
__global__ void sqrt_rn_kernel(const double *in, double *out, int n)
{
    int i = blockIdx.x * blockDim.x + threadIdx.x;
    if (i < n) out[i] = sqrt_rn(in[i]);
}
#endif

}
```

hnswindex.net_amd/csrc/dk_search_kernels.h:

```cpp
#pragma once
#include "dk_sorted_top.h"
#include "dk_pool_top.h"
#include "dk_traverse_exact.h"

namespace hnsw {

constexpr int kJobAnswered = 1, kJobTied = 2, kJobShadowed = 4;

struct SearchKernArgs {
    const float *rows; const double *row_sn; const float *queries; const double *q_sn; int dim; const int *adj0; int stride0;
    const int64_t *upper; const int *pool; int strideU; const SearchJob *jobs; int k, cand_cap; ND *spill; int spill_cap;
    unsigned *visited; long long vis_words; int *vis_tab; int vis_tab_cap, k_out; int *out_ids; float *out_d; int *out_cnt, *out_flag;
    unsigned long long *eval_counter; int nbcap, njobs; int *job_counter; int overlap; const int *ready;
    const float *pf_rows; unsigned long long *pf_words;
};
static_assert(offsetof(SearchKernArgs, jobs) == 80 && offsetof(SearchKernArgs, out_ids) == 144 && offsetof(SearchKernArgs, ready) == 208 &&
              offsetof(SearchKernArgs, pf_rows) == 216 && offsetof(SearchKernArgs, pf_words) == 224 && sizeof(SearchKernArgs) == 232,
              "SearchKernArgs must mirror graph_search_kernel's parameter list (the explicit arguments start the kernarg segment, each at its natural alignment)");
#define HNSW_KA(field) kernarg_load<decltype(SearchKernArgs::field)>((unsigned)offsetof(SearchKernArgs, field))

struct ChainEntry { int node, layer; };
template <bool CHAIN = false>
__device__ __forceinline__ void take_stable(const SearchLds &L, int lane, int top_n, int k_out, int *__restrict__ out_ids, float *__restrict__ out_d, int row,
                                            ChainEntry *next = nullptr, int per = 0)
// ... 18 lines not shown
        }
#pragma unroll
        for (int off = 32; off > 0; off >>= 1) {
            unsigned long long o = __shfl_xor(best, off, 64);
            best = o < best ? o : best;
        }
        if constexpr (CHAIN) {
            const bool have = best != ~0ull;
            const int wi = have ? (int)(best & 0xffffffffu) : 0;
            if (have && (wi & 63) == lane) used |= 1ull << (wi >> 6);
            ND w{-1, __uint_as_float(0x7fc00000u)};
            if (have) w = L.top[wi];
            if (r == 0) {
                if (have) { next->node = __builtin_amdgcn_readfirstlane(w.id); next->layer = row - 1; }
            } else if (lane == 0) {
                out_ids[(size_t)row * per + (r - 1)] = w.id;
                out_d[(size_t)row * per + (r - 1)] = w.dist;
            }
        } else {
            if (best == ~0ull) {
                if (lane == 0) { out_ids[(size_t)row * k_out + r] = -1; out_d[(size_t)row * k_out + r] = __uint_as_float(0x7fc00000u); }
                continue;
            }
            const int wi = (int)(best & 0xffffffffu);
            if ((wi & 63) == lane) used |= 1ull << (wi >> 6);
            if (lane == 0) { ND w = L.top[wi]; out_ids[(size_t)row * k_out + r] = w.id; out_d[(size_t)row * k_out + r] = w.dist; }
        }
    }
}

template <int METRIC, int NS, bool HASHED, int FORM = kFormPlain>
__device__ __forceinline__ void search_job(const float *__restrict__ rows, const double *__restrict__ row_sn, const float *__restrict__ queries,
                    const double *__restrict__ q_sn, int dim, const int *__restrict__ adj0, int stride0,
                    const int64_t *__restrict__ upper, const int *__restrict__ pool, int strideU,
                    const SearchJob *__restrict__ jobs, int k, int cand_cap, ND *__restrict__ spill,
                    int spill_cap, VisitedSet<HASHED> &V, int k_out, int *__restrict__ out_ids,
                    float *__restrict__ out_d, int *__restrict__ out_cnt, int *__restrict__ out_flag,
                    unsigned long long *__restrict__ eval_counter, int nbcap, unsigned char *smem, int job, int overlap,
                    int *__restrict__ job_word = nullptr, bool shadow = false, TeamPort *port = nullptr, bool *v_untouched = nullptr)
{
    constexpr bool LAT = FORM == kFormLat, LEAN = form_is_lean(FORM), PF = form_is_pf(FORM);
    if constexpr (LEAN) {
        cand_cap = HNSW_KA(cand_cap); nbcap = HNSW_KA(nbcap); jobs = HNSW_KA(jobs); queries = HNSW_KA(queries); q_sn = HNSW_KA(q_sn);
    }
    const SearchLds L = carve_lds(smem, k, cand_cap, dim, nbcap);
    const int lane = threadIdx.x & 63;
    if (v_untouched) *v_untouched = false;
    const SearchJob jb = jobs[job];
    const GraphView G{adj0, stride0, upper, pool, strideU};

    const float *q;
    double sb = 0.0;
    if (jb.qref >= 0) {
        q = queries + (size_t)jb.qref * dim;
        if (METRIC == M_COS) sb = q_sn[jb.qref];
    } else {
        q = row_at<METRIC>(rows, (size_t)(~jb.qref), dim);
        if (METRIC == M_COS) sb = row_sn[~jb.qref];
    }
    if constexpr (metric_f16(METRIC)) {
        if (jb.qref >= 0) for (int i = lane; i < dim; i += 64) L.qs[i] = q[i];
        else for (int i = lane; i < dim; i += 64) L.qs[i] = row_elem<METRIC>(q, i);
    } else
    for (int i = lane; i < dim; i += 64) L.qs[i] = q[i];
    if constexpr (LAT) { if (lane == 0) port->m->sb = sb; }
    unsigned long long evals = 0;
    int top_n = 0;
    bool repeated = shadow;
    ReadLog RL{nullptr, 0, 0};
    auto claim_answer = [&]() -> bool {
        if (!job_word) return true;
        int old = 0;
        if (lane == 0) old = atomicOr(job_word, kJobAnswered);
        return (__builtin_amdgcn_readfirstlane(old) & kJobAnswered) == 0;
    };
    if constexpr (NS > 0) {
        if (jb.aux != -2 && !shadow && !(overlap & 0x200)) {
        bool tie = false;
        bool window = false;
        bool ok1;
        if constexpr (LAT) ok1 = traverse_pool<METRIC, NS, HASHED>(rows, row_sn, dim, sb, G, jb, k, k_out + 1, V, L, lane, top_n, tie, evals, RL, nullptr, &window, port);
        else if constexpr (PF) {
            unsigned long long *const words = HNSW_KA(pf_words);
            RowPrefilterIo pf{HNSW_KA(pf_rows), __uint_as_float(*reinterpret_cast<const unsigned *>(words)), row_prefilter_c(dim), 0u, 0u};
            ok1 = traverse_sorted<METRIC, NS, HASHED, true, true>(rows, row_sn, dim, sb, G, jb, k, k_out + 1, V, L, lane, top_n, tie, evals, overlap, RL, nullptr, &window, &pf);
            if (lane == 0) { atomicAdd(words + 1, (unsigned long long)pf.n_shadow); atomicAdd(words + 2, (unsigned long long)pf.n_reread); }
        }
        else ok1 = traverse_sorted<METRIC, NS, HASHED, LEAN>(rows, row_sn, dim, sb, G, jb, k, k_out + 1, V, L, lane, top_n, tie, evals, overlap, RL, nullptr, &window);
        if (!(ok1 && tie)) {
            if (v_untouched) *v_untouched = LEAN || (!LAT && (overlap & 8) != 0);
            if (!claim_answer()) return;
            if constexpr (LEAN) {
                k_out = HNSW_KA(k_out); out_ids = HNSW_KA(out_ids); out_d = HNSW_KA(out_d); out_cnt = HNSW_KA(out_cnt); out_flag = HNSW_KA(out_flag);
                eval_counter = HNSW_KA(eval_counter);
            }
            for (int r = lane; r < k_out; r += 64) {
                const bool have = r < top_n;
                out_ids[(size_t)job * k_out + r] = have ? L.top[r].id : -1;
                out_d[(size_t)job * k_out + r] = have ? L.top[r].dist : __uint_as_float(0x7fc00000u);
            }
            if (lane == 0) {
                out_cnt[job] = ok1 ? top_n : 0;
                out_flag[job] = ok1 ? (window ? 4 : 0) : 1;
                atomicAdd(eval_counter, evals);
            }
            return;
        }
        if (job_word) {
            int old = 0;
            if (lane == 0) old = atomicOr(job_word, kJobTied);
            if (__builtin_amdgcn_readfirstlane(old) & (kJobShadowed | kJobAnswered)) return;
        }
        if constexpr (!LEAN) V.clear(lane);
        evals = 0;
        top_n = 0;
        repeated = true;
        }
    }
    bool aborted = false;
    bool ok;
    if constexpr (LEAN) {
        cand_cap = HNSW_KA(cand_cap);
        const int spill_cap_ = HNSW_KA(spill_cap);
        const long long vis_words = HNSW_KA(vis_words);
        int *const vis_tab = HNSW_KA(vis_tab);
        const int vis_tab_cap = HNSW_KA(vis_tab_cap);
        VisitedSet<HASHED> VE{HNSW_KA(visited) + (size_t)blockIdx.x * (size_t)vis_words, vis_words,
                              vis_tab ? vis_tab + (size_t)blockIdx.x * (size_t)vis_tab_cap : nullptr, (unsigned)(vis_tab_cap - 1), 0, vis_tab_cap / 4 * 3};
        ok = traverse<METRIC, HASHED>(rows, row_sn, dim, sb, G, jb, k, cand_cap, HNSW_KA(spill) + (size_t)blockIdx.x * spill_cap_, spill_cap_, VE, L, lane, top_n, evals, RL,
                                      shadow ? job_word : nullptr, &aborted, true);
        VE.clear(lane);
        if (v_untouched) *v_untouched = true;
        if (!aborted) {
            k_out = HNSW_KA(k_out); out_ids = HNSW_KA(out_ids); out_d = HNSW_KA(out_d); out_cnt = HNSW_KA(out_cnt); out_flag = HNSW_KA(out_flag);
            eval_counter = HNSW_KA(eval_counter);
        }
    } else
    ok = traverse<METRIC, HASHED>(rows, row_sn, dim, sb, G, jb, k, cand_cap, spill, spill_cap, V, L, lane, top_n, evals, RL,
                                             shadow ? job_word : nullptr, &aborted, LAT || (overlap & 1) != 0 || repeated);
    if (aborted || !claim_answer()) return;
    if (jb.aux == -2) {
        wave_sync();
        for (int r = lane; r < k_out; r += 64) {
            const bool have = ok && r < top_n;
            out_ids[(size_t)job * k_out + r] = have ? L.top[r].id : -1;
            out_d[(size_t)job * k_out + r] = have ? L.top[r].dist : __uint_as_float(0x7fc00000u);
        }
        if (lane == 0) {
            out_cnt[job] = ok ? top_n : 0;
            out_flag[job] = ok ? 0 : 1;
            atomicAdd(eval_counter, evals);
        }
        return;
    }
    take_stable(L, lane, top_n, k_out, out_ids, out_d, job);
    if (lane == 0) {
        out_cnt[job] = ok ? top_n : 0;
        out_flag[job] = ok ? (repeated ? 2 : 0) : 1;
        atomicAdd(eval_counter, evals);
    }
}

template <int METRIC, int NS, bool HASHED, int FORM = kFormPlain>
__global__ void __launch_bounds__(FORM == kFormLat ? 128 : 64) __attribute__((amdgpu_waves_per_eu(HNSW_WAVES(FORM == kFormLat ? (NS <= 4 ? 2 : 1) : FORM == kFormLeanPF ? HNSW_PF_WAVES : FORM == kFormLeanPFFixed ? HNSW_PF_FIXED_WAVES : METRIC == M_I8 ? (NS <= 2 ? HNSW_I8_WAVES : 4) : (NS <= 4 ? 3 : 2)))))
graph_search_kernel(const float *__restrict__ rows, const double *__restrict__ row_sn, const float *__restrict__ queries,
                    const double *__restrict__ q_sn, int dim, const int *__restrict__ adj0, int stride0,
                    const int64_t *__restrict__ upper, const int *__restrict__ pool, int strideU,
                    const SearchJob *__restrict__ jobs, int k, int cand_cap, ND *__restrict__ spill,
                    int spill_cap, unsigned *__restrict__ visited, long long vis_words, int *__restrict__ vis_tab, int vis_tab_cap, int k_out,
                    int *__restrict__ out_ids, float *__restrict__ out_d, int *__restrict__ out_cnt, int *__restrict__ out_flag,
                    unsigned long long *__restrict__ eval_counter, int nbcap, int njobs, int *__restrict__ job_counter, int overlap,
                    const int *__restrict__ ready, const float *__restrict__ pf_rows, unsigned long long *__restrict__ pf_words)
{
    constexpr bool LAT = FORM == kFormLat, LEAN = form_is_lean(FORM);
    if constexpr (form_is_pf(FORM) && METRIC != M_SQ) return;
    else {
    if constexpr (FORM == kFormLeanPFFixed) dim = kPfFixedDim;
    extern __shared__ __attribute__((aligned(16))) unsigned char smem[];
    const int lane = threadIdx.x & 63;
    VisitedSet<HASHED> V{LEAN ? nullptr : visited + (size_t)blockIdx.x * (size_t)vis_words, LEAN ? 0 : vis_words,
                 !LEAN && vis_tab ? vis_tab + (size_t)blockIdx.x * (size_t)vis_tab_cap : nullptr, LEAN ? 0u : (unsigned)(vis_tab_cap - 1), 0, LEAN ? 0 : vis_tab_cap / 4 * 3};
    ND *my_spill = LEAN ? nullptr : spill + (size_t)blockIdx.x * spill_cap;

    TeamPort port{nullptr, 0, 0};
    if constexpr (LAT) {
        TeamMail *mail = reinterpret_cast<TeamMail *>(smem + ((search_lds_bytes(k, cand_cap, dim, false, nbcap) + 15) & ~(size_t)15));
        if (threadIdx.x == 0) { mail->req_seq = 0; mail->rsp_seq = 0; mail->hint_node = -1; }
        __syncthreads();
        if (threadIdx.x >= 64) {
            const GraphView G{adj0, stride0, upper, pool, strideU};
            const SearchLds L = carve_lds(smem, k, cand_cap, dim, nbcap);
            memory_wave<METRIC, HASHED>(rows, row_sn, dim, G, V, L.qs, mail, lane);
            return;
        }
        port.m = mail;
    }
    bool shadows = (overlap & 0x100) != 0 && NS > 0 && !(overlap & 0x200);
    int *job_words = job_counter + 4;
    int known_ready = 0;
    bool v_clean = false;
    for (;;) {
        if constexpr (LEAN) {
            job_counter = HNSW_KA(job_counter); njobs = HNSW_KA(njobs); ready = HNSW_KA(ready); jobs = HNSW_KA(jobs); overlap = HNSW_KA(overlap);
            out_cnt = HNSW_KA(out_cnt); out_flag = HNSW_KA(out_flag);
            job_words = job_counter + 4;
            shadows = (overlap & 0x100) != 0 && !(overlap & 0x200);
        }
        int job = 0;
        bool shadow = false;
        if (lane == 0) job = atomicAdd(job_counter, 1);
        job = __builtin_amdgcn_readfirstlane(job);
        if (job >= njobs) {
            if (!shadows) break;
            int t = 0;
            if (lane == 0) t = atomicAdd(job_counter + 1, 1);
            t = __builtin_amdgcn_readfirstlane(t);
            if (t >= njobs || t >= (int)gridDim.x) break;
            job = njobs - 1 - t;
            if (ready) {
                const int need = __builtin_amdgcn_readfirstlane(jobs[job].qref);
                if (need >= known_ready) {
                    int r = 0;
                    if (lane == 0) r = __hip_atomic_load(ready, __ATOMIC_RELAXED, __HIP_MEMORY_SCOPE_SYSTEM);
                    known_ready = __builtin_amdgcn_readfirstlane(r);
                    __builtin_amdgcn_fence(__ATOMIC_ACQUIRE, "agent");
                    if (need >= known_ready) continue;
                }
            }
            int old = 0;
            if (lane == 0) old = atomicOr(job_words + job, kJobShadowed);
            old = __builtin_amdgcn_readfirstlane(old);
            if (old & (kJobAnswered | kJobTied)) continue;
            shadow = true;
        } else if (ready) {
            const int need = __builtin_amdgcn_readfirstlane(jobs[job].qref);
            if (need >= known_ready) {
                for (int spin = 0; spin < 512; ++spin) {
                    int r = 0;
                    if (lane == 0) r = __hip_atomic_load(ready, __ATOMIC_RELAXED, __HIP_MEMORY_SCOPE_SYSTEM);
                    known_ready = __builtin_amdgcn_readfirstlane(r);
                    if (need < known_ready) break;
                    for (int z = 0; z < 48; ++z) __builtin_amdgcn_s_sleep(127);
                }
                __builtin_amdgcn_fence(__ATOMIC_ACQUIRE, "agent");
                if (need >= known_ready) {
                    int old = 0;
                    if (shadows && lane == 0) {
                        old = atomicOr(job_words + job, kJobTied);
                        if (!(old & (kJobShadowed | kJobAnswered))) old = atomicOr(job_words + job, kJobAnswered) & kJobAnswered;
                    }
                    old = __builtin_amdgcn_readfirstlane(old);
                    if (old == 0 && lane == 0) {
                        out_cnt[job] = 0;
                        out_flag[job] = 1;
                    }
                    continue;
                }
            }
        }
        search_job<METRIC, NS, HASHED, FORM>(rows, row_sn, queries, q_sn, dim, adj0, stride0, upper, pool, strideU, jobs, k, cand_cap, my_spill, spill_cap,
// ... 343 lines not shown
```

hnswindex.net_amd/csrc/dk_sorted_top.h:

```cpp
#pragma once
#include "dk_search_common.h"

namespace hnsw {

__device__ __forceinline__ int dpp_wave_shr1(int carry_in, int v)
{
    return __builtin_amdgcn_update_dpp(carry_in, v, 0x138 , 0xf, 0xf, false);
}
template <int NS>
struct SortedTop {
    unsigned key[NS];
    int id[NS];
    __device__ __forceinline__ HEnt at(int p) const
    {
        HEnt e{__builtin_amdgcn_readlane(id[0], p & 63), (unsigned)__builtin_amdgcn_readlane((int)key[0], p & 63)};
#pragma unroll
        for (int t = 1; t < NS; ++t) {
            const int wi = __builtin_amdgcn_readlane(id[t], p & 63);
            const unsigned wk = (unsigned)__builtin_amdgcn_readlane((int)key[t], p & 63);
            if ((p >> 6) == t) { e.id = wi; e.key = wk; }
        }
        return e;
    }
    __device__ __forceinline__ unsigned key_at(int p) const
// ... 78 lines not shown
            if (lane == src) rank_old = r;
            rank_new += (xk < my_key || (xk == my_key && src > lane)) ? 1 : 0;
        }
        wave_lds_sync();
#pragma unroll
        for (int t = 0; t < NS; ++t) {
            const int p = lane + 64 * t;
            if (p < count && p + shift[t] <= k) lds[p + shift[t]] = make_uint2((unsigned)id[t], key[t]);
        }
        if ((pass >> lane) & 1ull) {
            const int np = rank_old + rank_new;
            if (np <= k) lds[np] = make_uint2((unsigned)my_id, my_key);
        }
        wave_lds_sync();
        const int total = count + (int)__popcll(pass);
        count = min(k, total);
#pragma unroll
        for (int t = 0; t < NS; ++t) {
            const int p = lane + 64 * t;
            if (p < count) { const uint2 e = lds[p]; id[t] = (int)e.x; key[t] = e.y; }
        }
        last_key = lds[count - 1].y;
        boundary_tie = total > k && lds[k].y == last_key;
        dropped_expanded = boundary_tie && (int)lds[k].x < 0;
        wave_lds_sync();
    }
    __device__ __forceinline__ bool contains_id(int node, int count, int lane) const
    {
        unsigned long long m = 0ull;
#pragma unroll
        for (int t = 0; t < NS; ++t) {
            if (64 * t >= count) break;
            m |= __ballot(lane + 64 * t < count && (id[t] & 0x3fffffff) == node);
        }
        return m != 0ull;
    }
    __device__ __forceinline__ bool any_open_key(unsigned k0, int count, int lane) const
    {
        bool o = false;
#pragma unroll
        for (int t = 0; t < NS; ++t) o |= lane + 64 * t < count && key[t] == k0 && id[t] >= 0;
        return __ballot(o) != 0ull;
    }
    __device__ __forceinline__ int first_flagged(int count, int lane, int bit) const
    {
#pragma unroll
        for (int t = 0; t < NS; ++t) {
            if (64 * t >= count) break;
            const unsigned long long m = __ballot(lane + 64 * t < count && (id[t] & bit) != 0);
            if (m) return 64 * t + (int)__builtin_ctzll(m);
        }
        return count;
    }
    __device__ __forceinline__ int count_key(unsigned k0, int count, int lane) const
    {
        int c = 0;
#pragma unroll
        for (int t = 0; t < NS; ++t) {
            if (64 * t >= count) break;
            c += (int)__popcll(__ballot(lane + 64 * t < count && key[t] == k0));
        }
        return c;
    }
    __device__ __forceinline__ bool adjacent_equal(int upto, int lane) const
    {
        bool eq = false;
#pragma unroll
        for (int t = 0; t < NS; ++t) {
            if (64 * t >= upto) break;
            int ck = 0;
            if (t > 0) ck = __builtin_amdgcn_readlane((int)key[t - 1], 63);
            const unsigned prev = (unsigned)dpp_wave_shr1(ck, (int)key[t]);
            const int p = lane + 64 * t;
            eq |= p >= 1 && p < upto && key[t] == prev;
        }
        return __ballot(eq) != 0ull;
    }
};

struct RowPrefilterIo {
    const float *rows;
    float e, c;
    unsigned n_shadow, n_reread;
};
__device__ __forceinline__ float row_prefilter_c(int dim) { return 1.0f + 1.5f * (1.001f * (float)((dim >> 3) + 16) * 5.9604644775390625e-8f); }
__device__ __forceinline__ float row_prefilter_threshold(float far, float e, float c)
{
    const float s = __builtin_sqrtf(fmaxf(far, 1e-30f) * c) + e;
    const float t = s * c;
    return t * t * 1.000003814697265625f;
}
__device__ __forceinline__ void measure_shadow(const float *shadow, int dim, const float *qs, const int *nbuf, float *dbuf, int m, int lane)
{
    for (int p0 = 0; p0 < m; p0 += 32) {
        const int left = m - p0;
        if (left > 24) measure_pass_h<M_SQH, 4>(shadow, dim, qs, nbuf, dbuf, p0, m, lane);
        else if (left > 16) measure_pass_h<M_SQH, 3>(shadow, dim, qs, nbuf, dbuf, p0, m, lane);
        else if (left > 8) measure_pass_h<M_SQH, 2>(shadow, dim, qs, nbuf, dbuf, p0, m, lane);
        else measure_pass_h<M_SQH, 1>(shadow, dim, qs, nbuf, dbuf, p0, m, lane);
    }
}

template <int METRIC, int NS, bool HASHED, bool LEAN = false, bool PF = false>
__device__ __forceinline__ bool traverse_sorted(const float *__restrict__ rows, const double *__restrict__ row_sn, int dim, double sb,
                                                const GraphView &G, const SearchJob jb, int k, int ordered_prefix, VisitedSet<HASHED> &V,
                                                const SearchLds &L, int lane, int &top_n_out, bool &tie_out, unsigned long long &evals,
                                                int oflags, ReadLog &RL, bool *order_tie_out = nullptr, bool *window_out = nullptr,
                                                RowPrefilterIo *pf = nullptr)
{
    int *nbuf = L.nbuf;
    float *dbuf = L.dbuf;
    const float *qs = L.qs;
    PH_DECL();
    int best;
    float cur;
    descend<METRIC>(rows, row_sn, dim, sb, G, jb, L, lane, best, cur, evals, RL);
    const int layer = jb.search_layer;
    RL.layer(layer, lane);
    SortedTop<NS> T;
#pragma unroll
    for (int t = 0; t < NS; ++t) { T.key[t] = 0u; T.id[t] = 0; }
    int top_n = 0;
    bool unsafe = key_unsafe(cur);
    bool tie = false, hash_full = false;
    T.insert(f2key(cur), best, top_n, k, lane);
    const bool novis = LEAN || (oflags & 8) != 0;
    if (!novis) {
        if (lane == 0) (void)V.first_visit(best);
        V.seen += 1;
    }
    unsigned far_key = f2key(cur);
    int pre_id = -1, pre_a = 0, pre_b = 0;
    const int lstride = layer == 0 ? G.stride0 : G.strideU;
    PH(0);
    constexpr int kDoubt = 0x40000000, kIdMask = 0x3fffffff;
    const bool ids_matter_everywhere = order_tie_out != nullptr;
    bool doubt_hard = false;
    unsigned nxt_key = 0xffffffffu;
    unsigned grp_key = 0u;
    int grp_cnt = 0;
    while (!unsafe && !tie) {
        const int pos = T.first_open(top_n, lane);
        if (pos < 0) break;
        const HEnt c = T.at(pos);
        if (c.id & kDoubt) { tie = true; break; }
        if (grp_cnt > 0 && c.key > grp_key) {
            if (T.count_key(grp_key, top_n, lane) != grp_cnt) { tie = true; break; }
            grp_cnt = 0;
            if (window_out) *window_out = true;
        }
        T.mark(pos, lane);
        RL.put(c.id & kIdMask, lane, top_n >= k && grp_cnt == 0 ? far_key : 0xffffffffu);
        PH(1);
        int n, nb_a = 0, nb_b = 0;
        if (c.id == pre_id) {
            n = __builtin_amdgcn_readlane(pre_a, 0);
            nb_a = __shfl(pre_a, (lane + 1) & 63, 64);
            const int w64 = __builtin_amdgcn_readlane(pre_b, 0);
            if (lane == 63) nb_a = w64;
            nb_b = __shfl(pre_b, (lane + 1) & 63, 64);
        } else {
            const int *l = G.list(c.id, layer);
            n = __builtin_amdgcn_readfirstlane(l[0]);
            if (lane < n) nb_a = l[1 + lane];
            if (lane + 64 < n) nb_b = l[65 + lane];
        }
        PH_COUNT(6, c.id == pre_id);
        PH_COUNT(7, 1);
        int m = 0;
        wave_sync();
        PH(2);
        bool have = false;
        float lane_d = 0.0f;
        int lane_id = 0;
        if (LEAN && n > 64) { hash_full = true; break; }
        const bool overlapped = LEAN || ((oflags & 1) != 0 && n <= 64);
        if (overlapped) {
            const bool in = lane < n;
            if (in) nbuf[lane] = nb_a;
            wave_sync();
            unsigned old = 0u;
            const unsigned bit = 1u << (nb_a & 31);
            unsigned hpos = 0u;
            if constexpr (HASHED) {
                hpos = ((unsigned)nb_a * 2654435761u) & V.tab_mask;
                if (in && !novis) old = (unsigned)atomicCAS(&V.tab[hpos], -1, nb_a);
            } else if (in && !novis) old = atomicOr(&V.bits[nb_a >> 5], bit);
            pre_id = -1;
            {
                const int nxt = T.first_open(top_n, lane);
                nxt_key = 0xffffffffu;
                if (nxt >= 0) {
                    const HEnt e = T.at(nxt);
                    nxt_key = e.key;
                    if (e.key == c.key) {
                        if (grp_cnt == 0) { grp_key = c.key; grp_cnt = T.count_key(c.key, top_n, lane); }
                        else if (c.key != grp_key) tie = true;
                    }
                    pre_id = e.id & kIdMask;
                    const int *pl = G.list(pre_id, layer);
                    pre_a = lane < lstride ? pl[lane] : 0;
                    pre_b = lane + 64 < lstride ? pl[lane + 64] : 0;
                }
            }
            PHX(0);
            bool pf_keep = false;
            int pf_pos = 0;
            if constexpr (PF) {
                if (n > 0) {
                    measure_shadow(pf->rows, dim, qs, nbuf, dbuf, n, lane);
                    wave_sync();
                    const float dh = in ? dbuf[lane] : 0.0f;
                    const float thr = top_n >= k ? row_prefilter_threshold(key2f(far_key), pf->e, pf->c) : __uint_as_float(0x7f800000u);
                    pf_keep = in && !(dh > thr);
                    const unsigned long long km = __ballot(pf_keep);
                    pf_pos = __builtin_amdgcn_mbcnt_hi((unsigned)(km >> 32), __builtin_amdgcn_mbcnt_lo((unsigned)km, 0));
                    const int kn = (int)__popcll(km);
                    if (pf_keep) nbuf[pf_pos] = nb_a;
                    wave_sync();
                    if (kn > 0) measure_all<METRIC>(rows, row_sn, dim, qs, sb, nbuf, dbuf, kn, lane);
                    pf->n_shadow += (unsigned)n;
                    pf->n_reread += (unsigned)kn;
                }
            } else
            if (n > 0) measure_all<METRIC>(rows, row_sn, dim, qs, sb, nbuf, dbuf, n, lane);
            wave_sync();
            PHX(1);
            if constexpr (PF) lane_d = pf_keep ? dbuf[pf_pos] : __uint_as_float(0x7f800000u);
            else
            lane_d = in ? dbuf[lane] : 0.0f;
            lane_id = nb_a;
            if (novis) {
                {
                    have = in;
                    const unsigned kq = f2key(lane_d);
                    unsigned long long look = __ballot(in && (top_n < k || kq <= far_key));
                    PHX_COUNT(3, __popcll(look));
                    unsigned long long listed = 0ull;
                    for (unsigned long long mm = look; mm; mm &= mm - 1) {
                        const int sl = (int)__builtin_ctzll(mm);
                        if (T.contains_id(__builtin_amdgcn_readlane(nb_a, sl), top_n, lane)) listed |= 1ull << sl;
                    }
                    if ((listed >> lane) & 1ull) have = false;
                }
            } else if constexpr (HASHED) {
                {
                have = in && (int)old == -1;
                if (in && (int)old != -1 && (int)old != nb_a) {
                    for (unsigned probes = 0; probes <= V.tab_mask; ++probes) {
                        hpos = (hpos + 1) & V.tab_mask;
                        const int o2 = atomicCAS(&V.tab[hpos], -1, nb_a);
                        if (o2 == -1) { have = true; break; }
                        if (o2 == nb_a) break;
                    }
                }
                }
            } else have = in && (old & bit) == 0u;
            const unsigned long long mask = __ballot(have);
            m = __popcll(mask);
            if (!novis) {
                V.seen += m;
                if (V.crowded()) { hash_full = true; break; }
            }
            PHX(2);
            PHX_COUNT(4, m);
            if (m == 0) continue;
            evals += (unsigned long long)m;
        } else {
        if (novis) { hash_full = true; break; }
        for (int base = 0; base < n; base += 64) {
            const int i = base + lane;
            bool fresh = false;
            const int nb = base == 0 ? nb_a : nb_b;
            if (i < n) fresh = V.first_visit(nb);
            const unsigned long long mask = __ballot(fresh);
            const int posn = __builtin_amdgcn_mbcnt_hi((unsigned)(mask >> 32), __builtin_amdgcn_mbcnt_lo((unsigned)mask, 0));
            if (fresh) nbuf[m + posn] = nb;
            m += __popcll(mask);
        }
        PH(3);
        pre_id = -1;
        {
            const int nxt = T.first_open(top_n, lane);
            nxt_key = 0xffffffffu;
            if (nxt >= 0) {
                const HEnt e = T.at(nxt);
                nxt_key = e.key;
                if (e.key == c.key) {
                    if (grp_cnt == 0) { grp_key = c.key; grp_cnt = T.count_key(c.key, top_n, lane); }
                    else if (c.key != grp_key) tie = true;
                }
                pre_id = e.id & kIdMask;
                const int *pl = G.list(pre_id, layer);
                pre_a = lane < lstride ? pl[lane] : 0;
                pre_b = lane + 64 < lstride ? pl[lane + 64] : 0;
            }
// ... 104 lines not shown
```

hnswindex.net_amd/csrc/exports.cpp:

```cpp
#include <algorithm>
#include <thread>
#include <atomic>
#include <chrono>
#include <cstddef>
#include <cstdio>
#include <cstdlib>
#include <cstring>
#include <mutex>
#include <shared_mutex>
#include <string>
#include <vector>

#include "../../include/hnsw_mi355x.h"
#include "hnsw_index.h"
#include "diag.h"
#include "range_replay.h"
#include "snapshot_io.h"

using hnsw::HnswIndex;
using hnsw::Params;

namespace {
std::mutex g_mu;
std::string g_last_error;
// ... 603 lines not shown
{
    std::lock_guard<std::mutex> lk(g_mu);
    g_pending.distribution_rate = (double)dist_rate;
    return 0;
}

#ifndef HNSW_MI355X_BUILD_ID_STR
#define HNSW_MI355X_BUILD_ID_STR "unidentified"
#endif
extern "C" __attribute__((visibility("default"), used)) const char hnsw_mi355x_build_id_tag[] = "HNSW_MI355X_BUILD_ID=" HNSW_MI355X_BUILD_ID_STR;
API const char *hnsw_mi355x_build_id(void) { return hnsw_mi355x_build_id_tag + sizeof("HNSW_MI355X_BUILD_ID=") - 1; }

API int hnsw_mi355x_count(void *h)
{
    if (!h) return 0;
    LOCK_INDEX(h);
    return static_cast<HnswIndex *>(h)->count();
}
API int hnsw_mi355x_set_queries(void *h, const float *queries, int count, int dim)
{
    if (!h || !queries || count <= 0 || dim <= 0) return -1;
    LOCK_INDEX(h);
    std::string err;
    if (static_cast<HnswIndex *>(h)->set_resident_queries(queries, count, dim, err) < 0) { set_error(err); return -1; }
    return 0;
}
API int hnsw_mi355x_resident_count(void *h)
{
    if (!h) return 0;
    LOCK_INDEX(h);
    return static_cast<HnswIndex *>(h)->resident_count();
}
API int hnsw_mi355x_knn_query_resident(void *h, int k, int *out_ids, float *out_dists)
{
    if (!h || !out_ids || !out_dists) return -1;
    LOCK_INDEX(h);
    std::string err;
    if (static_cast<HnswIndex *>(h)->knn_query_resident(k, out_ids, out_dists, err) < 0) { set_error(err); return -1; }
    return 0;
}
API int hnsw_mi355x_index_set_insert_batch(void *h, int max_batch)
{
    if (!h || max_batch == -1) { set_error("insert batch must be >= 1, 0 (the host's hardware threads), or -W with W >= 2"); return -1; }
    LOCK_INDEX(h);
    static_cast<HnswIndex *>(h)->set_insert_batch(max_batch);
    return 0;
}
API int hnsw_mi355x_host_parallelism(void) { return HnswIndex::host_parallelism(); }
API int hnsw_mi355x_index_insert_batch(void *h)
{
    if (!h) return 0;
    LOCK_INDEX(h);
    return static_cast<HnswIndex *>(h)->insert_batch_cap();
}
API int hnsw_mi355x_exact_window_stats(void *h, uint64_t out[4])
{
    if (!h || !out) return -1;
    LOCK_INDEX(h);
    static_cast<HnswIndex *>(h)->exact_window_stats(out);
    return 0;
}
API int hnsw_mi355x_row_prefilter_stats(void *h, uint64_t out[4])
{
    if (!h || !out) return -1;
    LOCK_INDEX(h);
    static_cast<HnswIndex *>(h)->row_prefilter_stats(out);
    return 0;
}
API int hnsw_mi355x_row_prefilter_form_stats(void *h, uint64_t out[2])
{
    if (!h || !out) return -1;
    LOCK_INDEX(h);
    static_cast<HnswIndex *>(h)->row_prefilter_form_stats(out);
    return 0;
}
API int hnsw_mi355x_row_prefilter_peek(void *h, int first_id, int count, uint64_t out[2], float *rows)
{
    if (!h || !out) return -1;
    LOCK_INDEX(h);
    std::string err;
    if (!static_cast<HnswIndex *>(h)->row_prefilter_peek(first_id, count, out, rows, err)) { set_error(err); return -1; }
    return 0;
}
API int hnsw_mi355x_get_info(void *h, hnsw_mi355x_layer_info *out, int cap)
{
    if (!h) return 0;
    if (cap < 0 || (cap > 0 && !out)) { set_error("System.ArgumentNullException: hnsw_mi355x_get_info"); return -1; }
    std::string err;
    LOCK_INDEX(h);
    const int n = static_cast<HnswIndex *>(h)->get_info(out, cap, err);
    if (n < 0) set_error(err);
    return n;
}
API int hnsw_mi355x_connected_component_counts(void *h, int *out, int cap)
{
    if (!h) return 0;
    if (cap < 0 || (cap > 0 && !out)) { set_error("System.ArgumentNullException: hnsw_mi355x_connected_component_counts"); return -1; }
    std::string err;
    LOCK_INDEX(h);
    const int n = static_cast<HnswIndex *>(h)->connected_component_counts(out, cap, err);
    if (n < 0) set_error(err);
    return n;
}
API int hnsw_mi355x_reachability(void *h, hnsw_mi355x_layer_reach *out, int cap)
{
    if (!h) return 0;
    if (cap < 0 || (cap > 0 && !out)) { set_error("System.ArgumentNullException: hnsw_mi355x_reachability"); return -1; }
    std::string err;
    LOCK_INDEX(h);
    const int n = static_cast<HnswIndex *>(h)->reachability(out, cap, err);
    if (n < 0) set_error(err);
    return n;
}
API int hnsw_mi355x_unreachable_ids(void *h, int layer, int *out, int cap)
{
    if (!h) return 0;
    if (cap < 0 || (cap > 0 && !out)) { set_error("System.ArgumentNullException: hnsw_mi355x_unreachable_ids"); return -1; }
    std::string err;
    std::vector<int> ids;
    LOCK_INDEX(h);
    if (static_cast<HnswIndex *>(h)->unreachable_ids(layer, ids, err) < 0) { set_error(err); return -1; }
    std::copy(ids.begin(), ids.begin() + std::min<size_t>(ids.size(), (size_t)cap), out);
    return (int)ids.size();
}
API int hnsw_mi355x_hop_counts(void *h, int layer, int *out, int cap)
{
    if (!h) return 0;
    if (cap < 0 || (cap > 0 && !out)) { set_error("System.ArgumentNullException: hnsw_mi355x_hop_counts"); return -1; }
    std::string err;
    LOCK_INDEX(h);
    const int n = static_cast<HnswIndex *>(h)->hop_counts(layer, out, cap, err);
    if (n < 0) set_error(err);
    return n;
}
API int hnsw_mi355x_repair_reachability(void *h, int cands, int max_rounds, hnsw_mi355x_layer_repair *out, int cap)
{
    if (!h) return 0;
    if (cap < 0 || (cap > 0 && !out)) { set_error("System.ArgumentNullException: hnsw_mi355x_repair_reachability"); return -1; }
    if (cands < 1 || cands > 64 || max_rounds < 1 || max_rounds > 64) {
        set_error("System.ArgumentOutOfRangeException: hnsw_mi355x_repair_reachability: cands = " + std::to_string(cands) + " and max_rounds = " +
                  std::to_string(max_rounds) + " must both be in 1 .. 64");
        return -1;
    }
    std::string err;
    LOCK_INDEX(h);
    const int n = static_cast<HnswIndex *>(h)->repair_reachability(cands, max_rounds, out, cap, err);
    if (n < 0) set_error(err);
    return n;
}
API int hnsw_mi355x_dim(void *h)
{
    if (!h) return 0;
    LOCK_INDEX(h);
    return static_cast<HnswIndex *>(h)->dim();
}
API int hnsw_mi355x_length(void *h)
{
    if (!h) return 0;
    LOCK_INDEX(h);
    return static_cast<HnswIndex *>(h)->graph().length;
}
API int hnsw_mi355x_active_ids(void *h, int *out, int cap)
{
    if (!h || !out) return -1;
    LOCK_INDEX(h);
    const hnsw::Graph &g = static_cast<HnswIndex *>(h)->graph();
// ... 251 lines not shown
```

hnswindex.net_amd/csrc/hnsw_index.cpp:

```cpp
#include "hnsw_index.h"
#include "diag.h"

#include <algorithm>
#include <array>
#include <atomic>
#include <chrono>
#include <cmath>
#include <cstdio>
#include <cstdlib>
#include <functional>
#include <limits>
#include <thread>
#include <unordered_map>

#include <fcntl.h>
#include <sys/mman.h>
#include <sys/stat.h>
#include <unistd.h>

#include "range_replay.h"
#include "snapshot_io.h"

namespace hnsw {

// ... 2202 lines not shown
    int lane = -1;
    bool shares_chip = false;
    {
        std::unique_lock<std::mutex> lk(lane_mu_);
        lane_cv_.wait(lk, [&] { return !lane_busy_[0] || !lane_busy_[1]; });
        lane = lane_busy_[0] ? 1 : 0;
        shares_chip = lane_busy_[1 - lane];
        lane_busy_[lane] = true;
        if (lane > 0 && !lanes_[lane]) {
            lanes_[lane].reset(Device::create_view(dev_.get()));
            if (lanes_[lane]) lanes_[lane]->set_profiling(profiling_);
        }
    }
    struct Release { HnswIndex *ix; int lane; ~Release() { { std::lock_guard<std::mutex> lk(ix->lane_mu_); ix->lane_busy_[lane] = false; } ix->lane_cv_.notify_one(); } } release{this, lane};
    Device *d = lane == 0 ? dev_.get() : lanes_[lane].get();
    if (!d) return 0;
    if (lane > 0) d->rebind(dev_.get());
    rc = -1;
    if (lane == 0) { resident_queries_ = 0; sharded_resident_ = false; }
    if (!d->set_queries(queries, count)) { err = get_dev_error(); return 1; }
    if (lane == 0) resident_queries_ = count;
    const int ep = graph_.entry, top = graph_.top_layer();
    std::vector<int> flag((size_t)count);
    d->set_shadows_allowed(!shares_chip);
    const bool ok = d->search_queries(count, ep, top, ef, k, out_ids, out_dists, flag.data());
    d->set_shadows_allowed(true);
    if (!ok) { err = get_dev_error(); return 1; }
    for (int i = 0; i < count; ++i) if (flag[(size_t)i]) return 0;
    rc = 0;
    return 1;
}

void HnswIndex::collect_stats(hnswdev_stats *out)
{
    std::memset(out, 0, sizeof(*out));
    if (!dev_) return;
    dev_->get_stats(out);
    for (auto &l : lanes_) {
        if (!l) continue;
        hnswdev_stats s;
        l->get_stats(&s);
        out->launches += s.launches; out->evals += s.evals; out->timed_launches += s.timed_launches; out->timed_evals += s.timed_evals; out->kernel_ms += s.kernel_ms;
        out->search_launches += s.search_launches; out->search_evals += s.search_evals; out->search_timed_launches += s.search_timed_launches;
        out->search_timed_evals += s.search_timed_evals; out->search_kernel_ms += s.search_kernel_ms; out->search_overflows += s.search_overflows;
        out->search_repeats += s.search_repeats; out->visited_hash_launches += s.visited_hash_launches;
        out->tie_windows += s.tie_windows; out->lat_launches += s.lat_launches; out->lean_launches += s.lean_launches; out->peer_direct_copies += s.peer_direct_copies; out->peer_staged_copies += s.peer_staged_copies; out->insert_tie_reruns += s.insert_tie_reruns; out->range_device_ordered += s.range_device_ordered; out->range_host_ordered += s.range_host_ordered;
    }
}

void HnswIndex::row_prefilter_stats(uint64_t out[4])
{
    out[0] = out[1] = out[2] = out[3] = 0;
    if (dev_) dev_->row_prefilter_stats(out);
    for (auto &r : replicas_) {
        uint64_t v[4];
        r->row_prefilter_stats(v);
        for (int i = 0; i < 4; ++i) out[i] += v[i];
    }
}

void HnswIndex::row_prefilter_form_stats(uint64_t out[2])
{
    out[0] = out[1] = 0;
    if (dev_) dev_->row_prefilter_form_stats(out);
    for (auto &r : replicas_) {
        uint64_t v[2];
        r->row_prefilter_form_stats(v);
        for (int i = 0; i < 2; ++i) out[i] += v[i];
    }
}

bool HnswIndex::row_prefilter_peek(long long first_id, int count, uint64_t out[2], float *rows, std::string &err)
{
    out[0] = out[1] = 0;
    if (!dev_) {
        if (count > 0) err = "row_prefilter_peek: the index has no shadow rows";
        return count <= 0;
    }
    if (dev_->row_prefilter_peek(first_id, count, out, rows)) return true;
    err = get_dev_error();
    return false;
}

void HnswIndex::reset_all_stats()
{
    if (dev_) dev_->reset_stats();
    for (auto &r : replicas_) r->reset_stats();
    for (auto &l : lanes_) if (l) l->reset_stats();
}

int HnswIndex::set_resident_queries(const float *queries, int count, int dim, std::string &err, bool streamed)
{
    const bool stream_on = diag("stream_queries", 1) != 0;
    streamed = streamed && stream_on;
    if (!ensure_dim(dim, err)) return -1;
    Tick t(g_pt.set_queries);
    sharded_resident_ = false;
    const int n = p_.devices;
    if (n > 1 && p_.device_traversal && count >= n) {
        if (!ensure_replicas(false, err)) return -1;
        shard_lo_.assign((size_t)n + 1, 0);
        for (int g = 0; g <= n; ++g) shard_lo_[(size_t)g] = (long long)count * g / n;
        const bool ok = fan_out(n, "set_queries failed", err, [&](int g) {
            const long long lo = shard_lo_[(size_t)g], hi = shard_lo_[(size_t)g + 1];
            const float *qs = queries + (size_t)lo * (size_t)dim;
            const int cnt = (int)(hi - lo);
            return streamed && cnt >= kStreamMin ? context(g)->set_queries_streamed(qs, cnt, kStreamHead) : context(g)->set_queries(qs, cnt);
        });
        if (!ok) { resident_queries_ = 0; return -1; }
        sharded_resident_ = true;
        resident_queries_ = count;
        return 0;
    }
    if (!(streamed && count >= kStreamMin ? dev_->set_queries_streamed(queries, count, kStreamHead) : dev_->set_queries(queries, count))) { err = get_dev_error(); return -1; }
    resident_queries_ = count;
    return 0;
}

int HnswIndex::knn_query_resident(int k, int *out_ids, float *out_dists, std::string &err)
{
    const int count = resident_queries_;
    if (count <= 0) return 0;
    if (failed(err)) return -1;
    if (k < 1 || graph_.entry < 0 || graph_.count <= 0) {
        pad_results(out_ids, out_dists, (size_t)count * (size_t)std::max(k, 0));
        return 0;
    }
    const int ef = std::max(p_.min_nn, k);
    const int ep = graph_.entry, top = graph_.top_layer();
    return answer_resident(count, ef,
        [&](Device *ctx, int cnt, long long lo, int *flag) { return ctx->search_queries(cnt, ep, top, ef, k, out_ids + (size_t)lo * k, out_dists + (size_t)lo * k, flag); },
        [&](const int *which, int n) { return knn_query_lockstep(which, n, k, out_ids, out_dists, err); },
        "search_batch failed", err);
}

int HnswIndex::range_query_lockstep(const int *which, int count, float range, std::vector<std::vector<NodeDist>> &out, std::string &err,
                                    const RangeFilter &f, int layer)
{
    if (!refresh_host_lists(err)) return -1;
    RangeSource src;
    src.jobs.resize((size_t)count);
    for (int i = 0; i < count; ++i) {
        const int qi = which ? which[i] : i;
        RangeJob &j = src.jobs[(size_t)i];
        j.g = &graph_;
        j.capacity = (int)capacity_;
        j.qi = qi;
        j.range = range;
        j.out = &out[(size_t)qi];
        j.allow = f.of(qi);
        j.layer = layer;
    }
    if (!engine()->run(src, count)) { err = get_dev_error(); return -1; }
    for (const RangeJob &j : src.jobs)
        if (j.heap_empty) { err = kHeapEmptyError; return -1; }
    return 0;
}

int HnswIndex::range_query_device(const int *which, int count, float range, std::vector<std::vector<NodeDist>> &out, std::string &err, const RangeFilter &f,
                                  int layer)
{
    if (!sync_graph(err)) return -1;
    std::vector<SearchJob> jobs((size_t)count);
    const int ep = graph_.entry, top = graph_.top_layer();
    for (int i = 0; i < count; ++i) jobs[(size_t)i] = SearchJob{which ? which[i] : i, ep, top, layer, -1};
    const auto qi = [&](size_t job) { return jobs[job].qref; };
// ... 571 lines not shown
```

hnswindex.net_amd/csrc/hnsw_index.h:

```cpp
#pragma once
#include <memory>
#include <atomic>
#include <condition_variable>
#include <mutex>
#include <shared_mutex>
#include <string>
#include <unordered_map>
#include <vector>

#include "device_backend.h"
#include "host_structs.h"
#include "search_engine.h"

namespace hnsw {

struct Params {
    int max_edges = 16;
    double distribution_rate = 0.36067376022224085;
    int min_nn = 5;
    int max_candidates = 100;
    int remove_max_candidates = 100;
    int collection_size = 65536;
    int random_seed = 31337;
    bool allow_removals = true;
// ... 7 lines not shown
};

class HnswIndex {
public:
    static HnswIndex *create(int metric, const Params &p, std::string &err);
    ~HnswIndex();

    int add(const float *vectors, int count, int dim, int *out_ids, std::string &err);
    int knn_query(const float *queries, int count, int dim, int k, int *out_ids, float *out_dists, std::string &err);

    int exact_knn_query(const float *queries, int count, int dim, int k, const uint32_t *allow_bits, long long nbits, int *out_ids, float *out_dists,
                        std::string &err);
    int exact_range_query(const float *queries, int count, int dim, float range, const uint32_t *allow_bits, long long nbits, int *counts,
                          std::vector<int> &ids, std::vector<float> &dists, std::string &err);
    int exact_knn_query_grouped(const float *queries, int count, int dim, int k, const int *row_group, long long n_row_group, const int *query_group,
                                int n_groups, int *out_ids, float *out_dists, std::string &err);
    int exact_knn_query_collapsed(const float *queries, int count, int dim, int k, const int *row_group, long long n_row_group, int per_group,
                                  const uint32_t *allow_bits, long long nbits, int *out_ids, float *out_dists, std::string &err);
    int knn_query_collapsed(const float *queries, int count, int dim, int k, int beam, const int *row_group, long long n_row_group, int per_group, int layer,
                            const uint32_t *allow_bits, long long nbits, int *out_ids, float *out_dists, std::string &err);
    int exact_knn_query_tagged(const float *queries, int count, int dim, int k, const uint32_t *row_tags, long long n_row_tags, const uint32_t *query_tags,
                               int match, int *out_ids, float *out_dists, std::string &err);
    int get_vectors(const int *ids, int n, float *out, std::string &err);
    int knn_query_by_id(const int *ids, int count, int k, int layer, int *out_ids, float *out_dists, std::string &err);
    int exact_knn_query_by_id(const int *ids, int count, int k, const uint32_t *allow_bits, long long nbits, int *out_ids, float *out_dists, std::string &err);
    int exact_range_query_by_id(const int *ids, int count, float range, const uint32_t *allow_bits, long long nbits, int *counts, std::vector<int> &out_ids,
                                std::vector<float> &out_dists, std::string &err);
    int duplicate_groups(float range, const uint32_t *allow_bits, long long nbits, int *out_labels, long long cap, uint64_t *out_info, std::string &err);
    int exact_range_query_grouped(const float *queries, int count, int dim, float range, const int *row_group, long long n_row_group, const int *query_group,
                                  int n_groups, int *counts, std::vector<int> &ids, std::vector<float> &dists, std::string &err);
    int exact_range_query_tagged(const float *queries, int count, int dim, float range, const uint32_t *row_tags, long long n_row_tags,
                                 const uint32_t *query_tags, int match, int *counts, std::vector<int> &ids, std::vector<float> &dists, std::string &err);
    int get_info(hnsw_mi355x_layer_info *out, int cap, std::string &err);
    int connected_component_counts(int *out, int cap, std::string &err);
    int reachability(hnsw_mi355x_layer_reach *out, int cap, std::string &err);
    int unreachable_ids(int layer, std::vector<int> &ids, std::string &err);
    int hop_counts(int layer, int *out, int cap, std::string &err);
    int repair_reachability(int cands, int max_rounds, hnsw_mi355x_layer_repair *out, int cap, std::string &err);
    int knn_query_general(const float *queries, int count, int dim, int k, int layer, const uint32_t *allow_bits, long long nbits, int *out_ids,
                          float *out_dists, std::string &err);
    int knn_query_grouped(const float *queries, int count, int dim, int k, int layer, const int *row_group, long long n_row_group, const int *query_group,
                          int n_groups, int *out_ids, float *out_dists, std::string &err);
    int knn_query_tagged(const float *queries, int count, int dim, int k, int layer, const uint32_t *row_tags, long long n_row_tags, const uint32_t *query_tags,
                         int match, int *out_ids, float *out_dists, std::string &err);
    int multilayer_knn_query(const float *queries, int count, int dim, int k, int max_layer, int min_layer, int layers_cap, int *out_ids,
                             float *out_dists, std::string &err);
    int top_layer() const { return graph_.entry < 0 ? -1 : graph_.top_layer(); }

    int set_resident_queries(const float *queries, int count, int dim, std::string &err, bool streamed = false);
    int knn_query_resident(int k, int *out_ids, float *out_dists, std::string &err);

    int range_query(const float *queries, int count, int dim, float range, std::vector<std::vector<NodeDist>> &out, std::string &err,
                    AllowBits allow = AllowBits{}, int layer = 0);

    int range_query_grouped(const float *queries, int count, int dim, float range, int layer, const int *row_group, long long n_row_group,
                            const int *query_group, int n_groups, std::vector<std::vector<NodeDist>> &out, std::string &err);
    int range_query_tagged(const float *queries, int count, int dim, float range, int layer, const uint32_t *row_tags, long long n_row_tags,
                           const uint32_t *query_tags, int match, std::vector<std::vector<NodeDist>> &out, std::string &err);

    int remove(const int *ids, int count, std::string &err);

    int serialize(const char *path, std::string &err);
    static HnswIndex *deserialize(int metric, const Params &backend, const char *path, std::string &err);

    int import_nodes(const float *rows, int n, int dim, const int *levels, int entry_point, std::string &err);
    int import_edges(int layer, const int *counts, const int *edges, int stride, std::string &err);

    int count() const { return graph_.count; }
    int resident_count() const { return resident_queries_; }
    int device_count() const { return p_.devices; }
    Device *device_at(int g) { return g == 0 ? dev_.get() : (g - 1 < (int)replicas_.size() ? replicas_[(size_t)g - 1].get() : nullptr); }
    int dim() const { return dim_; }
    const Graph &graph() { std::string e; (void)refresh_host_lists(e); return graph_; }
    Device *device() { return dev_.get(); }
    uint64_t graph_hash();
    void set_insert_batch(int v) { p_.insert_batch = v; }
    static int host_parallelism();
    int insert_batch_cap() const { return p_.insert_batch == 0 ? host_parallelism() : p_.insert_batch; }
    void counters(CounterBlock b, uint64_t *out) const;
    void exact_window_stats(uint64_t out[4]) const { out[0] = xw_rounds_; out[1] = xw_searches_; out[2] = xw_alone_; out[3] = xw_linked_; }
    void row_prefilter_stats(uint64_t out[4]);
    void row_prefilter_form_stats(uint64_t out[2]);
    bool row_prefilter_peek(long long first_id, int count, uint64_t out[2], float *rows, std::string &err);
    void set_profiling(bool on)
    {
        profiling_ = on;
        if (dev_) dev_->set_profiling(on);
        for (auto &r : replicas_) r->set_profiling(on);
        for (auto &l : lanes_) if (l) l->set_profiling(on);
    }

    std::shared_mutex &mutex() { return mu_; }
    int knn_query_concurrent(const float *queries, int count, int dim, int k, int *out_ids, float *out_dists, int &rc, std::string &err);
    void collect_stats(hnswdev_stats *out);
    void reset_all_stats();

private:
    std::shared_mutex mu_;
    static constexpr int kLanes = 2;
    std::unique_ptr<Device> lanes_[kLanes];
    bool lane_busy_[kLanes] = {false, false};
    std::mutex lane_mu_;
    std::condition_variable lane_cv_;
    HnswIndex() = default;
    std::string failed_msg_;
    bool failed(std::string &err) const { if (failed_msg_.empty()) return false; err = failed_msg_; return true; }
    int fail(const std::string &why, std::string &err)
    {
        failed_msg_ = "HNSWIndex MI355X backend: the index is unusable after a failed Add / Remove (" + why + ")";
        err = failed_msg_;
        return -1;
    }
    bool ensure_dim(int dim, std::string &err);
    bool ensure_capacity(long long need, std::string &err);
    bool insert_batch(const std::vector<int> &bid, std::string &err);
    long long exact_candidates(const uint32_t *&allow_bits, long long &nbits, std::vector<uint32_t> &live) const;
    bool live_labels(const int *&row_group, long long &n_row_group, std::vector<int> &live) const;
    bool ids_live(const char *who, const int *ids, int n, std::string &err) const;
    bool live_tags(const uint32_t *&row_tags, long long &n_row_tags, std::vector<uint32_t> &live) const;
    int reach_chain(const char *who, int min_layer, hnsw_mi355x_layer_reach *out, int cap, uint32_t *bits, int *hops, std::string &err);
    bool insert_exact_window(const std::vector<int> &fresh, int &p, int W, bool background, std::string &err);
    struct Selection {
        int n = 0, n_upper = 0;
        Device::InsertResults dev{nullptr, nullptr, nullptr, nullptr, nullptr, 0};
        std::vector<int> upper_base;
        std::vector<char> has_own;
        std::vector<std::vector<std::vector<int>>> own;
        inline void get(int i, int layer, const int *&ids, int &cnt) const
        {
            if (has_own[(size_t)i]) { const std::vector<int> &v = own[(size_t)i][(size_t)layer]; ids = v.data(); cnt = (int)v.size(); return; }
            if (layer == 0) { ids = dev.sel0 + (size_t)i * dev.sel_stride; cnt = dev.cnt0[i]; }
            else { const size_t s = (size_t)(upper_base[(size_t)i] + layer - 1); ids = dev.selU + s * dev.sel_stride; cnt = dev.cntU[s]; }
        }
    };
    bool search_half_lockstep(const std::vector<int> &bid, const std::vector<int> &items, Selection &sel, std::string &err);
    bool search_half_device(const std::vector<int> &bid, Selection &sel, std::string &err);
    bool link_half_lockstep(const std::vector<int> &bid, const Selection &sel, std::string &err);
    bool link_half_device(const std::vector<int> &bid, const Selection &sel, std::string &err);
    bool link_prefix_begin(const std::vector<int> &bid, const Selection &sel, int set, std::string &err);
    bool sync_graph(std::string &err);
    std::vector<std::unique_ptr<Device>> replicas_;
    std::vector<uint64_t> replica_epoch_;
    uint64_t graph_epoch_ = 1;
    std::vector<long long> shard_lo_;
    bool sharded_resident_ = false;
    Device *context(int g) { return g == 0 ? dev_.get() : replicas_[(size_t)g - 1].get(); }
    bool ensure_replicas(bool clone, std::string &err);
    bool gather_queries_to_primary(int count, std::string &err);
    bool refresh_host_lists(std::string &err);
    template <class OnDevice, class OnHost>
    int answer_resident(int count, int ef, OnDevice on_device, OnHost on_host, const char *fallback, std::string &err);
    template <class ArgsOk>
    int predicate_query_begin(const char *who, int count, int k, int layer, int *out_ids, float *out_dists, std::string &err, ArgsOk args_ok);
    template <class ClassOf, class Matches>
    int lockstep_by_class(const int *which, int n, int k, int layer, long long n_lab, size_t n_classes, ClassOf class_of, Matches matches, int *out_ids,
                          float *out_dists, std::string &err);
    template <class Search, class ClassOf, class Matches>
    int answer_by_class(int count, int k, int layer, long long n_lab, size_t n_classes, ClassOf class_of, Matches matches, Search search, const char *fallback,
                        int *out_ids, float *out_dists, std::string &err);
    int knn_query_lockstep(const int *which, int count, int k, int *out_ids, float *out_dists, std::string &err, AllowBits allow = AllowBits{},
                           int layer = 0, const int *exclude = nullptr);
    int range_query_lockstep(const int *which, int count, float range, std::vector<std::vector<NodeDist>> &out, std::string &err, const RangeFilter &f, int layer);
    int range_query_device(const int *which, int count, float range, std::vector<std::vector<NodeDist>> &out, std::string &err, const RangeFilter &f, int layer);
    template <class ClassOf, class ClassesWithId>
    int range_by_class(const char *who, const float *queries, int count, int dim, float range, int layer, RangeFilter f, ClassOf class_of,
                       ClassesWithId classes_with_id, std::vector<std::vector<NodeDist>> &out, std::string &err);
// ... 44 lines not shown
```

include/hnsw_mi355x.h:

```cpp
#ifndef HNSW_MI355X_H
#define HNSW_MI355X_H

#include <stdbool.h>
#include <stdint.h>

#ifdef __cplusplus
extern "C" {
#endif


int hnsw_get_last_error_utf8(void *buf, int buf_len);

void *hnsw_create(const char *distance_metric);

void hnsw_free(void *handle);

int hnsw_add(void *handle, const float *vectors, int count, int dim, int *out_ids);

int hnsw_remove(void *handle, const int *ids, int count);

int hnsw_knn_query(void *handle, const float *vectors, int count, int dim, int k, int *out_ids, float *out_dists);

int hnsw_range_query(void *handle, const float *vectors, int count, int dim, float range, void **out_ids,
                     void **out_dists, int *counts);

void hnsw_free_results(void **ids_array, void **dists_array, int count);

int hnsw_set_collection_size(int collection_size);
int hnsw_set_max_edges(int max_edges);
int hnsw_set_max_candidates(int max_candidates);
int hnsw_set_remove_max_candidates(int max_candidates);
int hnsw_set_distribution_rate(float dist_rate);
int hnsw_set_random_seed(int seed);
int hnsw_set_min_nn(int min_nn);
int hnsw_set_allow_removals(bool allow_removals);


typedef struct hnsw_mi355x_options {
    uint32_t struct_size;
    int32_t device;
    int32_t devices;
    int32_t insert_batch;
    int32_t remove_batch;
    int32_t host_threads;
    int32_t search_slots;
    int32_t device_traversal;
    const char *diagnostics;
} hnsw_mi355x_options;
int hnsw_mi355x_default_options(hnsw_mi355x_options *out);
int hnsw_mi355x_set_options(const hnsw_mi355x_options *opt);

int hnsw_mi355x_set_device(int device);
int hnsw_mi355x_set_insert_batch(int max_batch);
int hnsw_mi355x_index_set_insert_batch(void *handle, int max_batch);
int hnsw_mi355x_host_parallelism(void);
int hnsw_mi355x_index_insert_batch(void *handle);
int hnsw_mi355x_exact_window_stats(void *handle, uint64_t out[4]);
int hnsw_mi355x_row_prefilter_stats(void *handle, uint64_t out[4]);
int hnsw_mi355x_row_prefilter_form_stats(void *handle, uint64_t out[2]);
int hnsw_mi355x_row_prefilter_peek(void *handle, int first_id, int count, uint64_t out[2], float *rows);
int hnsw_mi355x_set_remove_batch(int max_batch);
int hnsw_mi355x_set_search_slots(int slots);
int hnsw_mi355x_set_host_threads(int threads);
int hnsw_mi355x_set_device_traversal(int enabled);

int hnsw_mi355x_set_devices(int n);
const char *hnsw_mi355x_build_id(void);
int hnsw_mi355x_device_count(void *handle);
struct hnswdev_stats;
int hnsw_mi355x_get_stats_at(void *handle, int context, struct hnswdev_stats *out);

int hnsw_mi355x_knn_query_filtered(void *handle, const float *vectors, int count, int dim, int k, const uint32_t *allow_bits,
                                   long long nbits, int *out_ids, float *out_dists);

int hnsw_mi355x_range_query_filtered(void *handle, const float *vectors, int count, int dim, float range, const uint32_t *allow_bits,
                                     long long nbits, void **out_ids, void **out_dists, int *counts);

int hnsw_mi355x_knn_query_at_layer(void *handle, const float *vectors, int count, int dim, int k, int layer, const uint32_t *allow_bits,
                                   long long nbits, int *out_ids, float *out_dists);
int hnsw_mi355x_range_query_at_layer(void *handle, const float *vectors, int count, int dim, float range, int layer, const uint32_t *allow_bits,
                                     long long nbits, void **out_ids, void **out_dists, int *counts);

int hnsw_mi355x_multilayer_knn_query(void *handle, const float *vectors, int count, int dim, int k, int max_layer, int min_layer,
                                     int layers_cap, int *out_ids, float *out_dists);

int hnsw_mi355x_exact_knn_query(void *handle, const float *vectors, int count, int dim, int k, const uint32_t *allow_bits, long long nbits,
                                int *out_ids, float *out_dists);

int hnsw_mi355x_exact_range_query(void *handle, const float *vectors, int count, int dim, float range, const uint32_t *allow_bits,
                                  long long nbits, void **out_ids, void **out_dists, int *counts);
int hnsw_mi355x_exact_range_info(void *handle, uint64_t out[4]);

int hnsw_mi355x_exact_knn_query_grouped(void *handle, const float *vectors, int count, int dim, int k, const int *row_group,
                                        long long n_row_group, const int *query_group, int n_groups, int *out_ids, float *out_dists);
int hnsw_mi355x_exact_grouped_info(void *handle, uint64_t out[4]);

int hnsw_mi355x_exact_knn_query_collapsed(void *handle, const float *vectors, int count, int dim, int k, const int *row_group,
                                          long long n_row_group, int per_group, const uint32_t *allow_words, long long nbits, int *out_ids,
                                          float *out_dists);
int hnsw_mi355x_knn_query_collapsed(void *handle, const float *vectors, int count, int dim, int k, int beam, const int *row_group,
                                    long long n_row_group, int per_group, int layer, const uint32_t *allow_words, long long nbits, int *out_ids,
                                    float *out_dists);
int hnsw_mi355x_exact_collapsed_info(void *handle, uint64_t out[4]);

int hnsw_mi355x_exact_range_query_grouped(void *handle, const float *vectors, int count, int dim, float range, const int *row_group,
                                          long long n_row_group, const int *query_group, int n_groups, void **out_ids, void **out_dists,
                                          int *counts);
int hnsw_mi355x_exact_range_grouped_info(void *handle, uint64_t out[4]);

int hnsw_mi355x_knn_query_grouped(void *handle, const float *vectors, int count, int dim, int k, int layer, const int *row_group,
                                  long long n_row_group, const int *query_group, int n_groups, int *out_ids, float *out_dists);
int hnsw_mi355x_knn_grouped_info(void *handle, uint64_t out[4]);

int hnsw_mi355x_knn_query_tagged(void *handle, const float *vectors, int count, int dim, int k, int layer, const uint32_t *row_tags,
                                 long long n_row_tags, const uint32_t *query_tags, int match, int *out_ids, float *out_dists);
int hnsw_mi355x_exact_knn_query_tagged(void *handle, const float *vectors, int count, int dim, int k, const uint32_t *row_tags,
                                       long long n_row_tags, const uint32_t *query_tags, int match, int *out_ids, float *out_dists);
int hnsw_mi355x_knn_tagged_info(void *handle, uint64_t out[5]);
int hnsw_mi355x_exact_tagged_info(void *handle, uint64_t out[6]);
int hnsw_mi355x_get_vectors(void *handle, const int *ids, int n, float *out);
int hnsw_mi355x_knn_query_by_id(void *handle, const int *ids, int count, int k, int layer, int *out_ids, float *out_dists);
int hnsw_mi355x_exact_knn_query_by_id(void *handle, const int *ids, int count, int k, const uint32_t *allow_bits, long long nbits, int *out_ids,
                                      float *out_dists);
int hnsw_mi355x_exact_range_query_by_id(void *handle, const int *ids, int count, float range, const uint32_t *allow_bits, long long nbits, void **out_ids,
                                        void **out_dists, int *counts);
int hnsw_mi355x_duplicate_groups(void *handle, float range, const uint32_t *allow_bits, long long nbits, int *out_labels, long long cap, uint64_t out_info[4]);
int hnsw_mi355x_by_id_info(void *handle, uint64_t out[6]);
int hnsw_mi355x_range_query_grouped(void *handle, const float *vectors, int count, int dim, float range, int layer, const int *row_group,
                                    long long n_row_group, const int *query_group, int n_groups, void **out_ids, void **out_dists, int *counts);
int hnsw_mi355x_range_grouped_info(void *handle, uint64_t out[4]);
int hnsw_mi355x_range_query_tagged(void *handle, const float *vectors, int count, int dim, float range, int layer, const uint32_t *row_tags,
                                   long long n_row_tags, const uint32_t *query_tags, int match, void **out_ids, void **out_dists, int *counts);
int hnsw_mi355x_exact_range_query_tagged(void *handle, const float *vectors, int count, int dim, float range, const uint32_t *row_tags,
                                         long long n_row_tags, const uint32_t *query_tags, int match, void **out_ids, void **out_dists, int *counts);
int hnsw_mi355x_range_tagged_info(void *handle, uint64_t out[6]);
int hnsw_mi355x_exact_range_tagged_info(void *handle, uint64_t out[9]);

int hnsw_mi355x_set_queries(void *handle, const float *queries, int count, int dim);
int hnsw_mi355x_knn_query_resident(void *handle, int k, int *out_ids, float *out_dists);
int hnsw_mi355x_resident_count(void *handle);

int hnsw_mi355x_count(void *handle);
int hnsw_mi355x_length(void *handle);
// ... 190 lines not shown
```

Measured before the change: 4.346 million.

## Add 8-bit quantized shadow rows for the search prefilter at fixed dim

Adds an 8-bit scalar-quantized copy of the dataset rows (global lo/step grid plus an error bound) that the lean traversal kernel uses to prefilter neighbor candidates, in place of the f16 shadow when dim equals the fixed prefilter dim. The byte rows halve the prefilter's gather traffic compared with f16. In exchange there is a bigger error bound, which can cause more rereads of full-precision rows, and an auto-fallback that disables it when rereads get too frequent. It also adds stats and peek APIs plus pack/range kernels.

```diff
diff --git a/hnswindex.net_amd/bindings.py b/hnswindex.net_amd/bindings.py
--- a/hnswindex.net_amd/bindings.py
+++ b/hnswindex.net_amd/bindings.py
@@ -245,6 +245,10 @@
 lib.hnsw_mi355x_row_prefilter_stats.argtypes = [ct.c_void_p, ct.POINTER(ct.c_uint64)]
 lib.hnsw_mi355x_row_prefilter_form_stats.restype = ct.c_int
 lib.hnsw_mi355x_row_prefilter_form_stats.argtypes = [ct.c_void_p, ct.POINTER(ct.c_uint64)]
+lib.hnsw_mi355x_row_prefilter8_stats.restype = ct.c_int
+lib.hnsw_mi355x_row_prefilter8_stats.argtypes = [ct.c_void_p, ct.POINTER(ct.c_uint64)]
+lib.hnsw_mi355x_row_prefilter8_peek.restype = ct.c_int
+lib.hnsw_mi355x_row_prefilter8_peek.argtypes = [ct.c_void_p, ct.c_int, ct.c_int, ct.POINTER(ct.c_uint64), ct.POINTER(ct.c_uint8)]
 lib.hnsw_mi355x_row_prefilter_peek.restype = ct.c_int
 lib.hnsw_mi355x_row_prefilter_peek.argtypes = [ct.c_void_p, ct.c_int, ct.c_int, ct.POINTER(ct.c_uint64), ct.POINTER(ct.c_float)]
 
@@ -629,6 +633,24 @@
         bits = int(out[1]) & 0xffffffff
         return {"packed": int(out[0]), "e_bits": bits, "e": np.array([bits], dtype=np.uint32).view(np.float32)[0], "rows": rows}
 
+    def row_prefilter8_stats(self):
+        names = ("launches", "rows_packed", "rows_on_shadow", "rows_reread", "full_packs", "fallbacks_to_f16")
+        out = (ct.c_uint64 * 6)()
+        if not self._h or lib.hnsw_mi355x_row_prefilter8_stats(self._h, out) != 0:
+            return dict.fromkeys(names, 0)
+        return {name: int(v) for name, v in zip(names, out)}
+
+    def row_prefilter8_peek(self, first_id: int = 0, count: int = 0):
+        out = (ct.c_uint64 * 4)()
+        codes = np.zeros((max(int(count), 0), 128), dtype=np.uint8)
+        f32 = lambda v: np.array([int(v) & 0xffffffff], dtype=np.uint32).view(np.float32)[0]
+        if not self._h:
+            if count > 0:
+                raise RuntimeError("row_prefilter8_peek: the index has no 8-bit shadow rows")
+            return {"packed": 0, "lo": np.float32(0), "step": np.float32(0), "e_bits": 0, "e": np.float32(0), "codes": codes}
+        self._check(lib.hnsw_mi355x_row_prefilter8_peek(self._h, int(first_id), int(count), out, codes.ctypes.data_as(ct.POINTER(ct.c_uint8))))
+        return {"packed": int(out[0]), "lo": f32(out[1]), "step": f32(out[2]), "e_bits": int(out[3]) & 0xffffffff, "e": f32(out[3]), "codes": codes}
+
     def set_remove_batch(self, max_batch: int):
         self._check(lib.hnsw_mi355x_set_remove_batch(max_batch))
 
diff --git a/hnswindex.net_amd/csrc/device_backend.h b/hnswindex.net_amd/csrc/device_backend.h
--- a/hnswindex.net_amd/csrc/device_backend.h
+++ b/hnswindex.net_amd/csrc/device_backend.h
@@ -316,6 +316,8 @@
     void row_prefilter_stats(uint64_t out[4]);
     void row_prefilter_form_stats(uint64_t out[2]);
     bool row_prefilter_peek(long long first_id, int count, uint64_t out[2], float *rows);
+    void row_prefilter8_stats(uint64_t out[6]);
+    bool row_prefilter8_peek(long long first_id, int count, uint64_t out[4], unsigned char *codes);
 
     std::mutex &mutex() { return mu_; }
     void set_error(const std::string &msg) { std::lock_guard<std::mutex> lk(err_mu_); err_ = msg; }
@@ -345,10 +347,19 @@
         bool no_memory = false;
         uint64_t launches = 0, on_shadow = 0, reread = 0, rows_packed = 0;
         uint64_t form_launches[2] = {0, 0};
+        struct Codes {
+            DevBuf<unsigned char> bytes;
+            DevBuf<unsigned long long> words;
+            long long row_cap = 0, packed = 0;
+            bool lost = false;
+            bool no_memory = false;
+            uint64_t launches = 0, on_shadow = 0, reread = 0, rows_packed = 0, full_packs = 0, fallbacks = 0;
+        } c8;
     };
     std::shared_ptr<RowPrefilter> pf_;
     void rows_written(long long first_id);
-    bool row_prefilter_ready();
+    int row_prefilter_ready();
+    bool row_prefilter8_ready();
     DevBuf<float> d_queries_;
     DevBuf<double> d_q_sn_;
     long long q_capacity() const { return (long long)(d_queries_.cap() / (size_t)pitch_); }
diff --git a/hnswindex.net_amd/csrc/device_backend.hip b/hnswindex.net_amd/csrc/device_backend.hip
--- a/hnswindex.net_amd/csrc/device_backend.hip
+++ b/hnswindex.net_amd/csrc/device_backend.hip
@@ -428,6 +428,7 @@
 }
 
 static int row_prefilter_mode() { return diag("row_prefilter", 1); }
+constexpr bool kRowPrefilter8ByDefault = true;
 
 void Device::rows_written(long long first_id)
 {
@@ -435,15 +436,63 @@
     std::lock_guard<std::mutex> lk(pf_->mu);
     pf_->packed = std::min(pf_->packed, std::max(0ll, first_id));
     pf_->lost = false;
-}
-
-bool Device::row_prefilter_ready()
+    pf_->c8.packed = std::min(pf_->c8.packed, std::max(0ll, first_id));
+    pf_->c8.lost = false;
+}
+
+bool Device::row_prefilter8_ready()
+{
+    RowPrefilter::Codes &C = pf_->c8;
+    hipStream_t st = S(stream_);
+    if (C.row_cap < capacity_ || !C.bytes) {
+        const std::string before = get_dev_error();
+        const bool first = !C.words;
+        if (!C.bytes.grow((size_t)capacity_ * kPfFixedDim) || !C.words.grow(kPf8GridWord + 1)) {
+            (void)C.bytes.reset();
+            C.row_cap = C.packed = 0;
+            C.no_memory = true;
+            (void)hipGetLastError();
+            set_dev_error(before);
+            return false;
+        }
+        C.row_cap = capacity_;
+        C.packed = 0;
+        if (first) HIP_OK(hipMemsetAsync(C.words, 0, (kPf8GridWord + 1) * sizeof(unsigned long long), st));
+    }
+    const long long n = n_rows_hw_;
+    if (C.packed < n) {
+        if (C.packed == 0) {
+            static const unsigned key_start[2] = {0xffffffffu, 0u};
+            HIP_OK(hipMemcpyAsync(C.words.get() + 3, key_start, sizeof(key_start), hipMemcpyHostToDevice, st));
+            const long long elems = n * kPfFixedDim;
+            const unsigned blocks = (unsigned)std::min<long long>((elems + 255) / 256, 8192);
+            hipLaunchKernelGGL(shadow8_range_kernel, dim3(blocks), dim3(256), 0, st, d_rows_.get(), elems, reinterpret_cast<unsigned *>(C.words.get() + 3));
+            HIP_OK(hipGetLastError());
+            hipLaunchKernelGGL(shadow8_grid_kernel, dim3(1), dim3(1), 0, st, C.words.get());
+            HIP_OK(hipGetLastError());
+            C.full_packs++;
+        }
+        const long long more = n - C.packed;
+        hipLaunchKernelGGL(pack_shadow8_rows_kernel, dim3((unsigned)((more + 3) / 4)), dim3(256), 0, st, d_rows_.get(), C.packed, more, C.bytes.get(), C.words.get());
+        HIP_OK(hipGetLastError());
+        HIP_OK(hipStreamSynchronize(st));
+        C.rows_packed += (uint64_t)more;
+        C.packed = n;
+    }
+    return true;
+}
+
+int Device::row_prefilter_ready()
 {
     const int mode = row_prefilter_mode();
-    if (!pf_ || metric_ != M_SQ || mode == 0 || bg_.active.load() || n_rows_hw_ <= 0) return false;
+    if (!pf_ || metric_ != M_SQ || mode == 0 || bg_.active.load() || n_rows_hw_ <= 0) return 0;
     RowPrefilter &P = *pf_;
     std::lock_guard<std::mutex> lk(P.mu);
-    if (P.no_memory || (P.lost && mode != 2)) return false;
+    if (pitch_ == kPfFixedDim && !P.c8.no_memory && (mode == 3 || (mode == 1 && kRowPrefilter8ByDefault && diag("pf_fixed_dim", 1) != 0 && !P.c8.lost))) {
+        if (row_prefilter8_ready()) return 2;
+        if (!P.c8.no_memory) return 0;
+    }
+    if (P.no_memory || (P.lost && mode != 2 && mode != 3)) return 0;
     hipStream_t st = S(stream_);
     const size_t words = (size_t)f16_row_words(dim_);
     if (P.row_cap < capacity_ || !P.rows) {
@@ -455,7 +504,7 @@
             P.no_memory = true;
             (void)hipGetLastError();
             set_dev_error(before);
-            return false;
+            return 0;
         }
         P.row_cap = capacity_;
         P.packed = 0;
@@ -472,7 +521,7 @@
         P.rows_packed += (uint64_t)more;
         P.packed = n;
     }
-    return true;
+    return 1;
 }
 
 void Device::row_prefilter_stats(uint64_t out[4])
@@ -480,7 +529,42 @@
     out[0] = out[1] = out[2] = out[3] = 0;
     if (!pf_) return;
     std::lock_guard<std::mutex> lk(pf_->mu);
-    out[0] = pf_->launches; out[1] = pf_->on_shadow; out[2] = pf_->reread; out[3] = pf_->rows_packed;
+    const RowPrefilter::Codes &C = pf_->c8;
+    out[0] = pf_->launches + C.launches; out[1] = pf_->on_shadow + C.on_shadow; out[2] = pf_->reread + C.reread; out[3] = pf_->rows_packed + C.rows_packed;
+}
+
+void Device::row_prefilter8_stats(uint64_t out[6])
+{
+    std::fill_n(out, 6, (uint64_t)0);
+    if (!pf_) return;
+    std::lock_guard<std::mutex> lk(pf_->mu);
+    const RowPrefilter::Codes &C = pf_->c8;
+    out[0] = C.launches; out[1] = C.rows_packed; out[2] = C.on_shadow; out[3] = C.reread; out[4] = C.full_packs; out[5] = C.fallbacks;
+}
+
+bool Device::row_prefilter8_peek(long long first_id, int count, uint64_t out[4], unsigned char *codes)
+{
+    out[0] = out[1] = out[2] = out[3] = 0;
+    if (!pf_ || !pf_->c8.bytes || !pf_->c8.words) {
+        if (count > 0) set_dev_error("row_prefilter8_peek: the index has no 8-bit shadow rows");
+        return count <= 0;
+    }
+    if (!bind()) return false;
+    std::lock_guard<std::mutex> lk(pf_->mu);
+    RowPrefilter::Codes &C = pf_->c8;
+    unsigned long long w[kPf8GridWord + 1] = {};
+    HIP_OK(hipMemcpy(w, C.words.get(), sizeof(w), hipMemcpyDeviceToHost));
+    out[0] = (uint64_t)C.packed;
+    out[1] = (uint64_t)(w[kPf8GridWord] & 0xffffffffull);
+    out[2] = (uint64_t)(w[kPf8GridWord] >> 32);
+    out[3] = (uint64_t)(w[0] & 0xffffffffull);
+    if (count <= 0) return true;
+    if (first_id < 0 || first_id + count > C.packed || !codes) {
+        set_dev_error("row_prefilter8_peek: range outside the packed shadow rows");
+        return false;
+    }
+    HIP_OK(hipMemcpy(codes, C.bytes.get() + (size_t)first_id * kPfFixedDim, (size_t)count * kPfFixedDim, hipMemcpyDeviceToHost));
+    return true;
 }
 
 void Device::row_prefilter_form_stats(uint64_t out[2])
@@ -1109,6 +1193,7 @@
     bool filtered;
     bool prefilter;
     bool pf_fixed;
+    bool pf8;
     int form;
     int slots, grid;
     unsigned block;
@@ -1124,7 +1209,7 @@
     t->num_cu = num_cu_;
     t->lds = lds;
     t->filtered = filtered;
-    t->prefilter = false;
+    t->prefilter = t->pf8 = false;
     t->pf_fixed = pitch_ == kPfFixedDim && diag("pf_fixed_dim", 1) != 0;
     t->exact_only = ns == 0;
     t->ns = t->exact_only ? 2 : ns;
@@ -1150,7 +1235,8 @@
         return form == kFormLat ? &graph_search_kernel<M, NS, H, kFormLat>
                : form == kFormLean ? &graph_search_kernel<M, NS, H, kFormLean>
                : form == kFormLeanPF ? &graph_search_kernel<M, NS, H, kFormLeanPF>
-               : form == kFormLeanPFFixed ? &graph_search_kernel<M, NS, H, kFormLeanPFFixed> : &graph_search_kernel<M, NS, H, kFormPlain>;
+               : form == kFormLeanPFFixed ? &graph_search_kernel<M, NS, H, kFormLeanPFFixed>
+               : form == kFormLeanPF8Fixed ? &graph_search_kernel<M, NS, H, kFormLeanPF8Fixed> : &graph_search_kernel<M, NS, H, kFormPlain>;
     else
         return form == kFormLat ? &graph_search_kernel<M, NS, H, kFormLat> : &graph_search_kernel<M, NS, H, kFormPlain>;
 }
@@ -1195,7 +1281,7 @@
         const int slots = std::min(t.max_slots, resident_blocks(traversal_kernel<Insert>(t, kFormLat), t.lds + kTeamLds, t.num_cu, 128));
         if (slots > 0 && (lat == 2 || nj <= slots)) { t.form = kFormLat; t.slots = slots; }
     }
-    if (!Insert && t.form == kFormPlain && t.novis && !t.exact_only && lean_mode() && t.ns <= 4) t.form = !t.prefilter ? kFormLean : t.pf_fixed ? kFormLeanPFFixed : kFormLeanPF;
+    if (!Insert && t.form == kFormPlain && t.novis && !t.exact_only && lean_mode() && t.ns <= 4) t.form = !t.prefilter ? kFormLean : t.pf8 ? kFormLeanPF8Fixed : t.pf_fixed ? kFormLeanPFFixed : kFormLeanPF;
     const auto kernel = traversal_kernel<Insert>(t, t.form);
     if (t.form != kFormLat) t.slots = std::min(t.max_slots, resident_blocks(kernel, t.lds, t.num_cu));
     t.grid = std::min(nj, t.slots);
@@ -1710,11 +1796,16 @@
             uj_len_ = nj; uj_entry_ = u_entry; uj_layer_ = u_layer;
         }
         auto kernel = place_traversal<false>(tl, nj);
-        if (tl.form == kFormLean && row_prefilter_ready()) {
-            tl.prefilter = true;
-            kernel = place_traversal<false>(tl, nj);
-        }
-        const bool prefiltered = form_is_pf(tl.form);
+        if (tl.form == kFormLean) {
+            const int shadow = row_prefilter_ready();
+            if (shadow != 0) {
+                tl.prefilter = true;
+                tl.pf8 = shadow == 2;
+                kernel = place_traversal<false>(tl, nj);
+            }
+        }
+        const bool prefiltered = form_is_pf(tl.form), pf8 = form_is_pf8(tl.form);
+        unsigned long long *const pf_words = !prefiltered ? nullptr : pf8 ? pf_->c8.words.get() : pf_->words.get();
         HIP_OK(hipMemsetAsync(s_jobctr_, 0, sizeof(int) * (4 + (size_t)nj), st));
         if (!compact) HIP_OK(hipMemsetAsync(s_evals_, 0, sizeof(unsigned long long), st));
         const bool timed = profiling_;
@@ -1722,13 +1813,13 @@
         hipLaunchKernelGGL(kernel, dim3(tl.grid), dim3(tl.block), tl.lds_total, st, d_rows_, d_row_sn_, d_queries_, d_q_sn_, pitch_, g_adj0_, g_stride0_,
                            g_upper_, g_pool_, g_strideU_, s_jobs_, k, cand_cap, reinterpret_cast<ND *>(s_spill_.get()), spill_cap_for_tests(), s_visited_,
                            tl.vis.words, tl.vis.tab, tl.vis.tab_cap, k_out, d_ids, d_d, s_cnt_, d_flag, d_ev, nbcap(), nj, s_jobctr_,
-                           tl.flags | (shadow_mode() && shadows_allowed_ ? 0x100 : 0), gate, prefiltered ? pf_->rows.get() : (const float *)nullptr,
-                           prefiltered ? pf_->words.get() : (unsigned long long *)nullptr);
+                           tl.flags | (shadow_mode() && shadows_allowed_ ? 0x100 : 0), gate,
+                           !prefiltered ? (const float *)nullptr : pf8 ? reinterpret_cast<const float *>(pf_->c8.bytes.get()) : pf_->rows.get(), pf_words);
         if (tl.form == kFormLat) stats_.lat_launches++;
         if (form_is_lean(tl.form)) stats_.lean_launches++;
         HIP_OK(hipGetLastError());
         if (timed) HIP_OK(hipEventRecord(E(ev1_), st));
-        if (prefiltered) HIP_OK(hipMemcpyAsync(h_pf, pf_->words.get() + 1, 2 * sizeof(unsigned long long), hipMemcpyDeviceToHost, st));
+        if (prefiltered) HIP_OK(hipMemcpyAsync(h_pf, pf_words + 1, 2 * sizeof(unsigned long long), hipMemcpyDeviceToHost, st));
         if (tail_.n > 0 && !upload_tail()) return false;
         if (compact) {
             HIP_OK(hipMemcpyAsync(h_ids, d_ids, 2 * b_res + sizeof(int) * (size_t)nj, hipMemcpyDeviceToHost, st));
@@ -1757,6 +1848,15 @@
             else if (h_flag[i] == 4) { stats_.tie_windows++; h_flag[i] = 0; }
         }
         memcpy(out_flag + off, h_flag, sizeof(int) * (size_t)nj);
+        if (pf8) {
+            std::lock_guard<std::mutex> lk(pf_->mu);
+            RowPrefilter::Codes &C = pf_->c8;
+            const uint64_t d_shadow = h_pf[0] > C.on_shadow ? h_pf[0] - C.on_shadow : 0, d_reread = h_pf[1] > C.reread ? h_pf[1] - C.reread : 0;
+            C.launches++;
+            C.on_shadow += d_shadow;
+            C.reread += d_reread;
+            if (4 * d_reread > d_shadow && row_prefilter_mode() == 1 && !C.lost) { C.lost = true; C.packed = 0; C.fallbacks++; }
+        } else
         if (prefiltered) {
             std::lock_guard<std::mutex> lk(pf_->mu);
             const uint64_t d_shadow = h_pf[0] > pf_->on_shadow ? h_pf[0] - pf_->on_shadow : 0, d_reread = h_pf[1] > pf_->reread ? h_pf[1] - pf_->reread : 0;
@@ -1766,7 +1866,7 @@
             pf_->reread += d_reread;
             if (2 * d_reread > d_shadow && row_prefilter_mode() != 2) pf_->lost = true;
         }
-        tl.prefilter = false;
+        tl.prefilter = tl.pf8 = false;
         if (!count_launch(nullptr, *h_ev, tl.vis.tab != nullptr, timed, ev0_, ev1_)) return false;
     }
     for (int i = 0; i < njobs; ++i) stats_.search_overflows += (uint64_t)(out_flag[i] == 1);
diff --git a/hnswindex.net_amd/csrc/device_kernels.h b/hnswindex.net_amd/csrc/device_kernels.h
--- a/hnswindex.net_amd/csrc/device_kernels.h
+++ b/hnswindex.net_amd/csrc/device_kernels.h
@@ -26,7 +26,8 @@
 #define HNSW_FOR_EACH_TRAVERSAL_LEAN(X, M) \
     X(M, 2, false, kFormLean) X(M, 4, false, kFormLean) X(M, 2, true, kFormLean) X(M, 4, true, kFormLean) \
     X(M, 2, false, kFormLeanPF) X(M, 4, false, kFormLeanPF) X(M, 2, true, kFormLeanPF) X(M, 4, true, kFormLeanPF) \
-    X(M, 2, false, kFormLeanPFFixed) X(M, 4, false, kFormLeanPFFixed) X(M, 2, true, kFormLeanPFFixed) X(M, 4, true, kFormLeanPFFixed)
+    X(M, 2, false, kFormLeanPFFixed) X(M, 4, false, kFormLeanPFFixed) X(M, 2, true, kFormLeanPFFixed) X(M, 4, true, kFormLeanPFFixed) \
+    X(M, 2, false, kFormLeanPF8Fixed) X(M, 4, false, kFormLeanPF8Fixed) X(M, 2, true, kFormLeanPF8Fixed) X(M, 4, true, kFormLeanPF8Fixed)
 
 #define HNSW_FOR_EACH_KIND(X, ...) \
     X(insert, __VA_ARGS__) X(insert_lat, __VA_ARGS__) X(search, __VA_ARGS__) X(search_lat, __VA_ARGS__) X(search_lean, __VA_ARGS__) \
diff --git a/hnswindex.net_amd/csrc/dk_base.h b/hnswindex.net_amd/csrc/dk_base.h
--- a/hnswindex.net_amd/csrc/dk_base.h
+++ b/hnswindex.net_amd/csrc/dk_base.h
@@ -22,6 +22,9 @@
 #ifndef HNSW_PF_FIXED_WAVES
 #define HNSW_PF_FIXED_WAVES 4
 #endif
+#ifndef HNSW_PF8_WAVES
+#define HNSW_PF8_WAVES 4
+#endif
 
 namespace hnsw {
 
@@ -39,9 +42,11 @@
     __builtin_amdgcn_wave_barrier();
     __builtin_amdgcn_fence(__ATOMIC_ACQUIRE, "wavefront");
 }
-constexpr int kFormPlain = 0, kFormLat = 1, kFormLean = 2, kFormLeanPF = 3, kFormLeanPFFixed = 4;
+constexpr int kFormPlain = 0, kFormLat = 1, kFormLean = 2, kFormLeanPF = 3, kFormLeanPFFixed = 4, kFormLeanPF8Fixed = 5;
 constexpr int kPfFixedDim = 128;
-constexpr __host__ __device__ bool form_is_pf(int f) { return f == kFormLeanPF || f == kFormLeanPFFixed; }
+constexpr __host__ __device__ bool form_is_pf8(int f) { return f == kFormLeanPF8Fixed; }
+constexpr __host__ __device__ bool form_is_pf_fixed(int f) { return f == kFormLeanPFFixed || f == kFormLeanPF8Fixed; }
+constexpr __host__ __device__ bool form_is_pf(int f) { return f == kFormLeanPF || form_is_pf_fixed(f); }
 constexpr __host__ __device__ bool form_is_lean(int f) { return f == kFormLean || form_is_pf(f); }
 
 template <class T>
diff --git a/hnswindex.net_amd/csrc/dk_misc_kernels.h b/hnswindex.net_amd/csrc/dk_misc_kernels.h
--- a/hnswindex.net_amd/csrc/dk_misc_kernels.h
+++ b/hnswindex.net_amd/csrc/dk_misc_kernels.h
@@ -134,6 +134,73 @@
     }
 }
 __global__ void __launch_bounds__(256)
+shadow8_range_kernel(const float *__restrict__ src, long long n_elems, unsigned *__restrict__ keys)
+{
+    unsigned kmin = 0xffffffffu, kmax = 0u;
+    for (long long t = (long long)blockIdx.x * 256 + threadIdx.x; t < n_elems; t += (long long)gridDim.x * 256) {
+        const float x = src[t];
+        if (x - x == 0.0f) { const unsigned k = f2key(x); kmin = k < kmin ? k : kmin; kmax = k > kmax ? k : kmax; }
+    }
+#pragma unroll
+    for (int o = 32; o > 0; o >>= 1) {
+        const unsigned a = (unsigned)__shfl_xor((int)kmin, o, 64), b = (unsigned)__shfl_xor((int)kmax, o, 64);
+        kmin = a < kmin ? a : kmin; kmax = b > kmax ? b : kmax;
+    }
+    if ((threadIdx.x & 63) == 0 && kmin <= kmax) { atomicMin(keys, kmin); atomicMax(keys + 1, kmax); }
+}
+__global__ void shadow8_grid_kernel(unsigned long long *__restrict__ words)
+{
+    const unsigned *keys = reinterpret_cast<const unsigned *>(words + 3);
+    float lo = 0.0f, step = 1.0f;
+    if (keys[0] <= keys[1]) {
+        lo = key2f(keys[0]);
+        const double s = ((double)key2f(keys[1]) - (double)lo) / 255.0;
+        if (s > 0.0) {
+            step = (float)s;
+            if ((double)step < s) step = __uint_as_float(__float_as_uint(step) + 1u);
+        }
+    }
+    words[kPf8GridWord] = (unsigned long long)__float_as_uint(lo) | ((unsigned long long)__float_as_uint(step) << 32);
+    words[0] = 0ull;
+}
+__global__ void __launch_bounds__(256)
+pack_shadow8_rows_kernel(const float *__restrict__ src, long long first, long long n, unsigned char *__restrict__ dst, unsigned long long *__restrict__ words)
+{
+    const int lane = threadIdx.x & 63;
+    const long long r = (long long)blockIdx.x * 4 + (threadIdx.x >> 6);
+    if (r >= n) return;
+    const unsigned long long grid = words[kPf8GridWord];
+    const float lo = __uint_as_float((unsigned)grid), step = __uint_as_float((unsigned)(grid >> 32));
+    const float *x = src + (size_t)(first + r) * kPfFixedDim;
+    unsigned char *rec = dst + (size_t)(first + r) * kPfFixedDim;
+    double ss = 0.0;
+    bool finite = true;
+    for (int i = lane; i < kPfFixedDim; i += 64) {
+        const float xi = x[i];
+        const double t = ((double)xi - (double)lo) / (double)step;
+        const int c = t > 0.0 ? (t < 255.0 ? (int)__builtin_rint(t) : 255) : 0;
+        rec[i] = (unsigned char)c;
+        const float h = __builtin_fmaf(step, (float)c, lo);
+        finite = finite && (h - h == 0.0f) && (xi - xi == 0.0f);
+        const double d = (double)xi - (double)h;
+        ss += d * d;
+    }
+#pragma unroll
+    for (int o = 32; o > 0; o >>= 1) ss += __shfl_xor(ss, o, 64);
+    const bool all_finite = __ballot(!finite) == 0ull;
+    if (lane == 0) {
+        unsigned bits = 0x7f800000u;
+        if (all_finite && ss < 1e300) {
+            const double e = sqrt(ss);
+            float f = (float)e;
+            if ((double)f < e) f = __uint_as_float(__float_as_uint(f) + 1u);
+            f = f * 1.00000095367431640625f + 1e-37f;
+            bits = __float_as_uint(f);
+        }
+        atomicMax(reinterpret_cast<unsigned *>(words), bits);
+    }
+}
+__global__ void __launch_bounds__(256)
 unpack_f16_rows_kernel(const float *__restrict__ recs, long long first, int n, int dim, float *__restrict__ out)
 {
     const long long t = (long long)blockIdx.x * 256 + threadIdx.x;
diff --git a/hnswindex.net_amd/csrc/dk_search_kernels.h b/hnswindex.net_amd/csrc/dk_search_kernels.h
--- a/hnswindex.net_amd/csrc/dk_search_kernels.h
+++ b/hnswindex.net_amd/csrc/dk_search_kernels.h
@@ -124,8 +124,9 @@
         if constexpr (LAT) ok1 = traverse_pool<METRIC, NS, HASHED>(rows, row_sn, dim, sb, G, jb, k, k_out + 1, V, L, lane, top_n, tie, evals, RL, nullptr, &window, port);
         else if constexpr (PF) {
             unsigned long long *const words = HNSW_KA(pf_words);
-            RowPrefilterIo pf{HNSW_KA(pf_rows), __uint_as_float(*reinterpret_cast<const unsigned *>(words)), row_prefilter_c(dim), 0u, 0u};
-            ok1 = traverse_sorted<METRIC, NS, HASHED, true, true>(rows, row_sn, dim, sb, G, jb, k, k_out + 1, V, L, lane, top_n, tie, evals, overlap, RL, nullptr, &window, &pf);
+            RowPrefilterIo pf{nullptr, 0.0f, row_prefilter_c(dim), 0u, 0u, (unsigned)offsetof(SearchKernArgs, pf_rows), (unsigned)offsetof(SearchKernArgs, pf_words)};
+            if constexpr (!form_is_pf8(FORM)) { pf.rows = HNSW_KA(pf_rows); pf.e = __uint_as_float(*reinterpret_cast<const unsigned *>(words)); }
+            ok1 = traverse_sorted<METRIC, NS, HASHED, true, true, form_is_pf8(FORM)>(rows, row_sn, dim, sb, G, jb, k, k_out + 1, V, L, lane, top_n, tie, evals, overlap, RL, nullptr, &window, &pf);
             if (lane == 0) { atomicAdd(words + 1, (unsigned long long)pf.n_shadow); atomicAdd(words + 2, (unsigned long long)pf.n_reread); }
         }
         else ok1 = traverse_sorted<METRIC, NS, HASHED, LEAN>(rows, row_sn, dim, sb, G, jb, k, k_out + 1, V, L, lane, top_n, tie, evals, overlap, RL, nullptr, &window);
@@ -204,7 +205,7 @@
 }
 
 template <int METRIC, int NS, bool HASHED, int FORM = kFormPlain>
-__global__ void __launch_bounds__(FORM == kFormLat ? 128 : 64) __attribute__((amdgpu_waves_per_eu(HNSW_WAVES(FORM == kFormLat ? (NS <= 4 ? 2 : 1) : FORM == kFormLeanPF ? HNSW_PF_WAVES : FORM == kFormLeanPFFixed ? HNSW_PF_FIXED_WAVES : METRIC == M_I8 ? (NS <= 2 ? HNSW_I8_WAVES : 4) : (NS <= 4 ? 3 : 2)))))
+__global__ void __launch_bounds__(FORM == kFormLat ? 128 : 64) __attribute__((amdgpu_waves_per_eu(HNSW_WAVES(FORM == kFormLat ? (NS <= 4 ? 2 : 1) : FORM == kFormLeanPF ? HNSW_PF_WAVES : FORM == kFormLeanPFFixed ? HNSW_PF_FIXED_WAVES : FORM == kFormLeanPF8Fixed ? HNSW_PF8_WAVES : METRIC == M_I8 ? (NS <= 2 ? HNSW_I8_WAVES : 4) : (NS <= 4 ? 3 : 2)))))
 graph_search_kernel(const float *__restrict__ rows, const double *__restrict__ row_sn, const float *__restrict__ queries,
                     const double *__restrict__ q_sn, int dim, const int *__restrict__ adj0, int stride0,
                     const int64_t *__restrict__ upper, const int *__restrict__ pool, int strideU,
@@ -217,7 +218,7 @@
     constexpr bool LAT = FORM == kFormLat, LEAN = form_is_lean(FORM);
     if constexpr (form_is_pf(FORM) && METRIC != M_SQ) return;
     else {
-    if constexpr (FORM == kFormLeanPFFixed) dim = kPfFixedDim;
+    if constexpr (form_is_pf_fixed(FORM)) dim = kPfFixedDim;
     extern __shared__ __attribute__((aligned(16))) unsigned char smem[];
     const int lane = threadIdx.x & 63;
     VisitedSet<HASHED> V{LEAN ? nullptr : visited + (size_t)blockIdx.x * (size_t)vis_words, LEAN ? 0 : vis_words,
diff --git a/hnswindex.net_amd/csrc/dk_sorted_top.h b/hnswindex.net_amd/csrc/dk_sorted_top.h
--- a/hnswindex.net_amd/csrc/dk_sorted_top.h
+++ b/hnswindex.net_amd/csrc/dk_sorted_top.h
@@ -184,7 +184,14 @@
     const float *rows;
     float e, c;
     unsigned n_shadow, n_reread;
+    unsigned ka_codes, ka_words;
 };
+constexpr int kPf8GridWord = 16;
+__device__ __forceinline__ unsigned long long pf8_word(unsigned ka_words, int i)
+{
+    typedef const unsigned long long __attribute__((address_space(4))) *cptr;
+    return ((cptr)(unsigned long long)kernarg_load<unsigned long long *>(ka_words))[i];
+}
 __device__ __forceinline__ float row_prefilter_c(int dim) { return 1.0f + 1.5f * (1.001f * (float)((dim >> 3) + 16) * 5.9604644775390625e-8f); }
 __device__ __forceinline__ float row_prefilter_threshold(float far, float e, float c)
 {
@@ -203,7 +210,61 @@
     }
 }
 
-template <int METRIC, int NS, bool HASHED, bool LEAN = false, bool PF = false>
+template <int NP>
+__device__ __forceinline__ void measure_pass_c8(const unsigned char *__restrict__ codes, unsigned ka_words, const float *qs, const int *nbuf,
+                                                float *dbuf, int p0, int m, int lane)
+{
+    const int grp = lane >> 3, j = lane & 7;
+    u32x4 w[NP];
+    int cidx[NP];
+#pragma unroll
+    for (int p = 0; p < NP; ++p) {
+        const int c = p0 + grp + 8 * p;
+        cidx[p] = c;
+        const int id = nbuf[c < m ? c : p0];
+        w[p] = *reinterpret_cast<const u32x4 *>(codes + (size_t)id * kPfFixedDim + 16 * j);
+    }
+    __builtin_amdgcn_sched_barrier(0);
+    const unsigned long long grid = pf8_word(ka_words, kPf8GridWord);
+    const float lo = __uint_as_float((unsigned)grid), step = __uint_as_float((unsigned)(grid >> 32));
+    const f32x2 lo2 = {lo, lo}, step2 = {step, step};
+    f32x2 acc[NP];
+#pragma unroll
+    for (int p = 0; p < NP; ++p) acc[p] = f32x2{0.0f, 0.0f};
+    const float *q = qs + 16 * j;
+#pragma unroll
+    for (int t = 0; t < 4; ++t) {
+        const f32x4 y = *reinterpret_cast<const f32x4 *>(q + 4 * t);
+        const f32x2 y01 = {y.x, y.y}, y23 = {y.z, y.w};
+#pragma unroll
+        for (int p = 0; p < NP; ++p) {
+            const unsigned ww = w[p][t];
+            const f32x2 c01 = {(float)(ww & 0xffu), (float)((ww >> 8) & 0xffu)}, c23 = {(float)((ww >> 16) & 0xffu), (float)(ww >> 24)};
+            const f32x2 h01 = __builtin_elementwise_fma(step2, c01, lo2), h23 = __builtin_elementwise_fma(step2, c23, lo2);
+            const f32x2 d01 = y01 - h01, d23 = y23 - h23;
+            acc[p] = __builtin_elementwise_fma(d01, d01, acc[p]);
+            acc[p] = __builtin_elementwise_fma(d23, d23, acc[p]);
+        }
+    }
+#pragma unroll
+    for (int p = 0; p < NP; ++p) {
+        const float lane_sum = acc[p].x + acc[p].y;
+        const float s = collapse_l2(lane_sum);
+        if (j == 0 && cidx[p] < m) dbuf[cidx[p]] = s;
+    }
+}
+__device__ __forceinline__ void measure_shadow8(const unsigned char *codes, unsigned ka_words, const float *qs, const int *nbuf, float *dbuf, int m, int lane)
+{
+    for (int p0 = 0; p0 < m; p0 += 32) {
+        const int left = m - p0;
+        if (left > 24) measure_pass_c8<4>(codes, ka_words, qs, nbuf, dbuf, p0, m, lane);
+        else if (left > 16) measure_pass_c8<3>(codes, ka_words, qs, nbuf, dbuf, p0, m, lane);
+        else if (left > 8) measure_pass_c8<2>(codes, ka_words, qs, nbuf, dbuf, p0, m, lane);
+        else measure_pass_c8<1>(codes, ka_words, qs, nbuf, dbuf, p0, m, lane);
+    }
+}
+
+template <int METRIC, int NS, bool HASHED, bool LEAN = false, bool PF = false, bool PF8 = false>
 __device__ __forceinline__ bool traverse_sorted(const float *__restrict__ rows, const double *__restrict__ row_sn, int dim, double sb,
                                                 const GraphView &G, const SearchJob jb, int k, int ordered_prefix, VisitedSet<HASHED> &V,
                                                 const SearchLds &L, int lane, int &top_n_out, bool &tie_out, unsigned long long &evals,
@@ -310,10 +371,15 @@
             int pf_pos = 0;
             if constexpr (PF) {
                 if (n > 0) {
+                    if constexpr (PF8) measure_shadow8(kernarg_load<const unsigned char *>(pf->ka_codes), pf->ka_words, qs, nbuf, dbuf, n, lane);
+                    else
                     measure_shadow(pf->rows, dim, qs, nbuf, dbuf, n, lane);
                     wave_sync();
                     const float dh = in ? dbuf[lane] : 0.0f;
-                    const float thr = top_n >= k ? row_prefilter_threshold(key2f(far_key), pf->e, pf->c) : __uint_as_float(0x7f800000u);
+                    float e_bound;
+                    if constexpr (PF8) e_bound = __uint_as_float((unsigned)pf8_word(pf->ka_words, 0));
+                    else e_bound = pf->e;
+                    const float thr = top_n >= k ? row_prefilter_threshold(key2f(far_key), e_bound, pf->c) : __uint_as_float(0x7f800000u);
                     pf_keep = in && !(dh > thr);
                     const unsigned long long km = __ballot(pf_keep);
                     pf_pos = __builtin_amdgcn_mbcnt_hi((unsigned)(km >> 32), __builtin_amdgcn_mbcnt_lo((unsigned)km, 0));
diff --git a/hnswindex.net_amd/csrc/exports.cpp b/hnswindex.net_amd/csrc/exports.cpp
--- a/hnswindex.net_amd/csrc/exports.cpp
+++ b/hnswindex.net_amd/csrc/exports.cpp
@@ -709,6 +709,21 @@
     if (!static_cast<HnswIndex *>(h)->row_prefilter_peek(first_id, count, out, rows, err)) { set_error(err); return -1; }
     return 0;
 }
+API int hnsw_mi355x_row_prefilter8_stats(void *h, uint64_t out[6])
+{
+    if (!h || !out) { set_error("System.ArgumentNullException: hnsw_mi355x_row_prefilter8_stats"); return -1; }
+    LOCK_INDEX(h);
+    static_cast<HnswIndex *>(h)->row_prefilter8_stats(out);
+    return 0;
+}
+API int hnsw_mi355x_row_prefilter8_peek(void *h, int first_id, int count, uint64_t out[4], uint8_t *codes)
+{
+    if (!h || !out || (count > 0 && !codes)) { set_error("System.ArgumentNullException: hnsw_mi355x_row_prefilter8_peek"); return -1; }
+    LOCK_INDEX(h);
+    std::string err;
+    if (!static_cast<HnswIndex *>(h)->row_prefilter8_peek(first_id, count, out, codes, err)) { set_error(err); return -1; }
+    return 0;
+}
 API int hnsw_mi355x_get_info(void *h, hnsw_mi355x_layer_info *out, int cap)
 {
     if (!h) return 0;
diff --git a/hnswindex.net_amd/csrc/hnsw_index.cpp b/hnswindex.net_amd/csrc/hnsw_index.cpp
--- a/hnswindex.net_amd/csrc/hnsw_index.cpp
+++ b/hnswindex.net_amd/csrc/hnsw_index.cpp
@@ -2308,6 +2308,29 @@
     return false;
 }
 
+void HnswIndex::row_prefilter8_stats(uint64_t out[6])
+{
+    std::fill_n(out, 6, (uint64_t)0);
+    if (dev_) dev_->row_prefilter8_stats(out);
+    for (auto &r : replicas_) {
+        uint64_t v[6];
+        r->row_prefilter8_stats(v);
+        for (int i = 0; i < 6; ++i) out[i] += v[i];
+    }
+}
+
+bool HnswIndex::row_prefilter8_peek(long long first_id, int count, uint64_t out[4], unsigned char *codes, std::string &err)
+{
+    out[0] = out[1] = out[2] = out[3] = 0;
+    if (!dev_) {
+        if (count > 0) err = "row_prefilter8_peek: the index has no 8-bit shadow rows";
+        return count <= 0;
+    }
+    if (dev_->row_prefilter8_peek(first_id, count, out, codes)) return true;
+    err = get_dev_error();
+    return false;
+}
+
 void HnswIndex::reset_all_stats()
 {
     if (dev_) dev_->reset_stats();
diff --git a/hnswindex.net_amd/csrc/hnsw_index.h b/hnswindex.net_amd/csrc/hnsw_index.h
--- a/hnswindex.net_amd/csrc/hnsw_index.h
+++ b/hnswindex.net_amd/csrc/hnsw_index.h
@@ -113,6 +113,8 @@
     void row_prefilter_stats(uint64_t out[4]);
     void row_prefilter_form_stats(uint64_t out[2]);
     bool row_prefilter_peek(long long first_id, int count, uint64_t out[2], float *rows, std::string &err);
+    void row_prefilter8_stats(uint64_t out[6]);
+    bool row_prefilter8_peek(long long first_id, int count, uint64_t out[4], unsigned char *codes, std::string &err);
     void set_profiling(bool on)
     {
         profiling_ = on;
diff --git a/include/hnsw_mi355x.h b/include/hnsw_mi355x.h
--- a/include/hnsw_mi355x.h
+++ b/include/hnsw_mi355x.h
@@ -59,6 +59,8 @@
 int hnsw_mi355x_row_prefilter_stats(void *handle, uint64_t out[4]);
 int hnsw_mi355x_row_prefilter_form_stats(void *handle, uint64_t out[2]);
 int hnsw_mi355x_row_prefilter_peek(void *handle, int first_id, int count, uint64_t out[2], float *rows);
+int hnsw_mi355x_row_prefilter8_stats(void *handle, uint64_t out[6]);
+int hnsw_mi355x_row_prefilter8_peek(void *handle, int first_id, int count, uint64_t out[4], uint8_t *codes);
 int hnsw_mi355x_set_remove_batch(int max_batch);
 int hnsw_mi355x_set_search_slots(int slots);
 int hnsw_mi355x_set_host_threads(int threads);
```

Result: faster. 4.754 million, median of 6 (+9.4%).
